# kolenyo2099/revers-o

Measured on AMD Instinct MI355X. Metric: images/sec embed+top-k (PE-L14-336, 1M x 1024 gallery), higher is better.
Workload: dtype bf16

## Files before the change

include/revo.h:

```cpp
#ifndef REVO_H
#define REVO_H
#include <stdint.h>

#ifdef __cplusplus
extern "C" {
#endif

typedef struct revo_vit revo_vit;
typedef struct revo_gallery revo_gallery;

typedef struct revo_vit_cfg {
    int32_t image_size, patch_size, width, layers, heads, mlp_dim, out_dim, pool_heads;
    int32_t use_cls;
    int32_t use_ls;
    float ln_eps, rope_theta;
    int32_t pool_mlp_dim;
} revo_vit_cfg;

typedef struct revo_tensor {
    const char* name;
    const float* data;
    int64_t numel;
} revo_tensor;

// ... 54 lines not shown
                         void* stream);
int32_t revo_search_topk_large(revo_gallery* g, const float* queries, int32_t n_queries, int32_t k, int32_t has_threshold,
                               float threshold, int64_t index_offset, float* scores, int64_t* indices, int32_t* counts,
                               void* stream);
int32_t revo_gallery_pairs(revo_gallery* g, float threshold, int64_t* n_pairs, void* stream);
int32_t revo_gallery_pairs_read(revo_gallery* g, int64_t start, int64_t n, int64_t* pairs, float* scores,
                                int32_t dst_on_device);
int32_t revo_gallery_clusters(revo_gallery* g, float threshold, int64_t* n_clusters, int64_t* n_members, void* stream);
int32_t revo_gallery_clusters_read(revo_gallery* g, int64_t* labels, int64_t* offsets, int64_t* members,
                                   int32_t dst_on_device);
int32_t revo_gallery_knn(revo_gallery* g, int32_t k, int32_t has_threshold, float threshold, int64_t* n_rows, void* stream);
int32_t revo_gallery_knn_read(revo_gallery* g, int64_t start, int64_t n, int64_t* indices, float* scores, int32_t* counts,
                              int32_t dst_on_device);
int32_t revo_gallery_kmeans(revo_gallery* g, const float* centroids, int32_t n_centroids, int32_t normalize,
                            int32_t src_on_device, int32_t max_iter, int32_t* n_iter, int32_t* converged, int64_t* n_rows,
                            void* stream);
int32_t revo_gallery_kmeans_read(revo_gallery* g, int64_t start, int64_t n, int32_t* labels, float* scores,
                                 int32_t dst_on_device);
int32_t revo_gallery_kmeans_centroids(revo_gallery* g, float* centroids, int64_t* sizes, int32_t dst_on_device);
int32_t revo_search_range(revo_gallery* g, const float* queries, int32_t n_queries, float threshold, int64_t index_offset,
                          int64_t* n_results, void* stream);
int32_t revo_search_range_read(revo_gallery* g, int64_t* offsets, int64_t start, int64_t n, int64_t* indices, float* scores,
                               int32_t dst_on_device);
int32_t revo_search_recommend(revo_gallery* g, const float* examples, int32_t n_positive, int32_t n_negative, int32_t k,
                              int32_t has_threshold, float threshold, int64_t index_offset, float* scores, int64_t* indices,
                              int32_t* counts, void* stream);
int32_t revo_search_discover(revo_gallery* g, const float* target, const float* positives, const float* negatives,
                             int32_t n_pairs, int32_t k, int32_t has_threshold, float threshold, int64_t index_offset,
                             float* scores, int64_t* indices, int32_t* counts, void* stream);
int32_t revo_search_maxsim(revo_gallery* g, const float* queries, int32_t n_vectors, int32_t k, int32_t has_threshold,
                           float threshold, int64_t index_offset, float* scores, int32_t* group_ids, int32_t* counts,
                           float* part_scores, int64_t* part_rows, void* stream);
int32_t revo_search_mmr(revo_gallery* g, const float* queries, int32_t n_queries, int32_t k, int32_t candidates,
                        float diversity, int32_t has_threshold, float threshold, int64_t index_offset, float* scores,
                        float* mmr_values, int64_t* indices, int32_t* counts, void* stream);
int32_t revo_search_fusion(revo_gallery* g, const float* queries, int32_t n_searches, int32_t n_lists, int32_t limit,
                           int32_t method, float rrf_k, const float* weights, const float* list_thresholds, int32_t k,
                           int32_t has_threshold, float threshold, int64_t index_offset, float* scores, int64_t* indices,
                           int32_t* counts, int32_t* ranks, float* list_scores, void* stream);
int32_t revo_topk_fuse(const float* scores, const int64_t* indices, const int32_t* counts, int32_t n_searches,
                       int32_t n_lists, int32_t limit, int32_t method, float rrf_k, const float* weights,
                       const float* list_thresholds, int32_t k, int32_t has_threshold, float threshold,
                       float* out_scores, int64_t* out_indices, int32_t* out_counts, int32_t* out_ranks, void* stream);
int32_t revo_search_ksel(int32_t k);
int32_t revo_search_set_total_rows(revo_gallery* g, int64_t total_rows);
int32_t revo_search_set_filter(revo_gallery* g, const uint32_t* allow_bits, int64_t rows, int32_t src_on_device,
                               void* stream);
int32_t revo_search_set_groups(revo_gallery* g, const int32_t* group_of_row, int64_t rows, int32_t src_on_device,
                               void* stream);
int32_t revo_search_groups(revo_gallery* g, const float* queries, int32_t n_queries, int32_t limit, int32_t group_size,
                           int32_t has_threshold, float threshold, int64_t index_offset, float* scores, int64_t* indices,
                           int32_t* hit_counts, int32_t* group_ids, int32_t* group_counts, void* stream);
int32_t revo_search_estimates(int32_t k);
int32_t revo_search_plan(const revo_gallery* g, int32_t n_queries, int32_t k, int64_t* out4);
int32_t revo_search_candidates(revo_gallery* g, const float* queries, int32_t n_queries, int32_t k, int32_t top_m,
                               uint32_t* bounds, void* stream);
int32_t revo_search_finish(revo_gallery* g, int32_t n_queries, int32_t k, int32_t has_threshold, float threshold,
                           int64_t index_offset, const uint32_t* all_bounds, int32_t parts, int32_t top_m, float* scores,
                           int64_t* indices, int32_t* counts, float* cert, void* stream);
int32_t revo_search_exact(revo_gallery* g, int32_t n, const int32_t* q_idx, const float* need, int32_t k,
                          int32_t has_threshold, float threshold, int64_t index_offset, float* scores, int64_t* indices,
                          int32_t* counts, void* stream);
int32_t revo_search_stats(revo_gallery* g, int32_t* out8, void* stream);
int32_t revo_topk_merge(const float* scores, const int64_t* indices, int32_t parts, int32_t n_queries, int32_t k,
                        int32_t has_threshold, float threshold, float* out_scores, int64_t* out_indices,
                        int32_t* out_counts, void* stream);

int64_t revo_topk_packed_bytes(int32_t n_queries, int32_t k);
int32_t revo_topk_merge_packed(const void* packed, int32_t parts, int32_t n_queries, int32_t k, int32_t has_threshold,
                               float threshold, float* out_scores, int64_t* out_indices, int32_t* out_counts,
                               int32_t* unc_count, int32_t* unc_q, float* unc_need, void* stream);

int32_t revo_op_gemm(int32_t epilogue, const void* a_bf16, int64_t lda, const void* b_bf16, int64_t ldb, int32_t m,
                     int32_t n, int32_t k, void* c, int64_t ldc, const float* bias, const float* gamma, void* stream);
int32_t revo_op_gemm_rope(const void* a_bf16, int64_t lda, const void* b_bf16, int64_t ldb, int32_t m, int32_t n, int32_t k,
                          void* c_bf16, int64_t ldc, const float* bias, const float* cos_sin, int32_t seq,
                          int32_t head_dim, int32_t rope_cols, void* stream);
int32_t revo_op_gemm_resid_ln(const void* a_bf16, int64_t lda, const void* b_bf16, int64_t ldb, int32_t m, int32_t n, int32_t k,
                              float* c, int64_t ldc, const float* bias, const float* gamma, void* xb_bf16, int64_t ldxb,
                              void* stats, int32_t* done, void* xlo_bf16, int32_t x_in_planes, int32_t planes_out, void* stream);
int32_t revo_op_gemm_ln_in(int32_t epilogue, const void* a_bf16, int64_t lda, const void* b_bf16, int64_t ldb, int32_t m, int32_t n,
                           int32_t k, void* c_bf16, int64_t ldc, const float* bias, const float* csum, const void* stats,
                           int32_t parts, float eps, void* tele, void* stream);
int32_t revo_op_gemm_ln_in_rope(const void* a_bf16, int64_t lda, const void* b_bf16, int64_t ldb, int32_t m, int32_t n, int32_t k,
                                void* c_bf16, int64_t ldc, const float* bias, const float* csum, const void* stats, int32_t parts,
                                float eps, const float* cos_sin, int32_t seq, int32_t head_dim, int32_t rope_cols, void* stream);
int32_t revo_op_gemm_resid_norm(const void* a_bf16, int64_t lda, const void* b_bf16, int64_t ldb, int32_t m, int32_t n, int32_t k,
                                float* c, int64_t ldc, const float* bias, const float* gamma, void* ln_out_bf16, int64_t ln_ldo,
                                float eps, int32_t* fused, void* stream);
int32_t revo_probe_mfma(const void* src_bf16, int64_t n_elems, float* sink, int32_t blocks, int32_t iters, void* stream);
int64_t revo_probe_mfma_flops(int32_t blocks, int32_t iters);
int32_t revo_probe_copy(void* dst, const void* src, int64_t bytes, void* stream);
#ifdef REVO_EXPERIMENTS
int32_t revo_vit_set_debug_layers(revo_vit* vit, int32_t n_layers);
int32_t revo_vit_read_residual(revo_vit* vit, int32_t batch, float* dst, void* stream);
int32_t revo_vit_read_tap(revo_vit* vit, int32_t which, int32_t batch, void* dst, void* stream);
int32_t revo_text_set_debug_layers(revo_text* text, int32_t n_layers);
int32_t revo_text_read_residual(revo_text* text, int32_t batch, float* dst, void* stream);
int32_t revo_search_set_mode(revo_gallery* g, int32_t mode);
int32_t revo_debug_set_remove_chunk(int64_t rows);
int32_t revo_debug_set_knn(int64_t cap_keys, int32_t level_mode);
int32_t revo_debug_set_kmeans(int64_t cap_keys);
int32_t revo_op_set_phase_groups(int32_t groups);
int32_t revo_op_set_qstores(int32_t on);
int32_t revo_debug_gemm_stamps(void* buf, int32_t items);
int32_t revo_debug_attention_clock(void* buf);
int32_t revo_debug_gemm_forms(int32_t reset);
int32_t revo_op_set_gemm_tile(int32_t tile);
int32_t revo_op_set_variant(int32_t flags);
int32_t revo_op_set_ln_fold(int32_t on);
int32_t revo_op_set_gemm_debug(int32_t flags);
int64_t revo_debug_scan_plan(int32_t Q, int64_t rows, int64_t* out, int32_t cap);
int64_t revo_debug_gemm_plan(int32_t epi, int32_t m, int32_t n, int32_t k, int64_t lda, int64_t ldb, int64_t ldc, int64_t ws_elems,
                             int32_t offers, int32_t rope_seq, int32_t rope_head_dim, int32_t rope_cols, int64_t* out, int32_t cap);
int32_t revo_debug_stream_in_planes(const revo_vit* vit, int32_t batch);
int64_t revo_debug_read_workspace(revo_gallery* g, int64_t offset, int64_t bytes, void* host_dst);
int32_t revo_debug_seed_bounds(revo_gallery* g, const uint32_t* bounds);
int32_t revo_probe_gridbar(int32_t mode, void* ctr_err, void* buf, int32_t n16, int32_t blocks, int32_t threads,
                           int32_t iters, float* sink, void* stamps, void* stream);
int32_t revo_debug_scan_stats(int64_t* out8);
#endif
int32_t revo_op_layernorm(const float* x, int64_t ldx, const float* w, const float* b, float eps, int32_t rows,
                          int32_t width, void* out, int64_t ldo, int32_t out_is_bf16, void* stream);
int32_t revo_op_layernorm_logits(const float* x, int64_t ldx, const float* w, const float* b, float eps, int32_t rows,
                                 int32_t width, float* out, int64_t ldo, const float* qk, const float* ck, int32_t heads,
                                 int32_t seq, float* logits, void* stream);
int32_t revo_op_linear_f32(int32_t epi, const float* A, int64_t lda, const float* Wt, int64_t ldw, const float* bias, int32_t M,
                           int32_t N, int32_t K, float* C, int64_t ldc, void* stream);
int32_t revo_op_linear_f32_grouped(int32_t epi, const float* A, int64_t lda, int64_t a_group_stride, int32_t group_cols,
                                   const float* Wt, int64_t ldw, const float* bias, int32_t M, int32_t N, int32_t K, float* C,
                                   int64_t ldc, void* stream);
int32_t revo_op_probe_qk(const float* q, const float* Wk, const float* bk, int32_t width, int32_t heads, float* qk, float* ck,
                         void* stream);
int32_t revo_op_l2norm_rows(const float* src, int64_t ld_src, float* dst_f32, int64_t ld_f32, uint16_t* dst_bf16, int64_t ld_bf16,
                            int64_t rows, int32_t dim, int32_t normalize, float* row_stats, float* max_stats, uint32_t* zero_a,
                            int64_t zero_a_words, uint32_t* zero_b, int64_t zero_b_words, const int64_t* dst_rows, void* stream);
int32_t revo_op_gallery_cert_stats(revo_gallery* g, float* out, void* stream);
int32_t revo_op_pool_rows(const float* x, int64_t ldx, const float* logits, int32_t batch, int32_t seq, int32_t width,
                          int32_t heads, float* u, void* stream);
int32_t revo_op_pool_rows_masked(const float* x, int64_t ldx, const float* logits, const int32_t* region_image,
                                 const uint32_t* region_bits, int32_t n_regions, int32_t batch, int32_t seq, int32_t width,
                                 int32_t heads, float* u, void* stream);
int32_t revo_op_detect_scores(const float* tokens, int64_t rows, const float* prompts, int32_t n_prompts, int32_t dim,
                              float* prompts_norm, float* scores, void* stream);
int32_t revo_op_detect_regions(const float* scores, int32_t batch, int32_t n_prompts, int32_t g, int32_t use_cls,
                               const float* thresholds, int32_t n_background, int32_t min_cells, int32_t max_regions,
                               int32_t* region_image, int32_t* region_prompt, int32_t* boxes, int32_t* cells, float* confidence,
                               uint32_t* bits, int32_t* labels, int32_t* counts, void* stream);
int32_t revo_op_rope(void* qkv_bf16, int64_t ld, const float* cos_sin, int32_t rows, int32_t seq, int32_t width,
                     int32_t heads, void* stream);
int32_t revo_op_attention(const void* qkv_bf16, int64_t ld, void* out_bf16, int64_t ldo, int32_t batch, int32_t seq,
                          int32_t heads, int32_t head_dim, void* stream);
int32_t revo_op_attention_causal(const void* qkv_bf16, int64_t ld, void* out_bf16, int64_t ldo, int32_t batch, int32_t seq,
                                 int32_t heads, int32_t head_dim, void* stream);
int32_t revo_op_embed_tokens(const int32_t* tokens_dev, const float* table, const float* pos, int32_t batch, int32_t seq,
                             int32_t vocab, int32_t width, float* x, int64_t ldx, void* stream);
int32_t revo_op_pool_eot(const int32_t* tokens_dev, const float* x, int64_t ldx, int32_t batch, int32_t seq, int32_t width,
                         float* out, void* stream);
int32_t revo_op_f32_to_bf16(const float* src, int64_t ld_src, void* dst_bf16, int64_t ld_dst, int64_t rows,
                            int32_t cols, void* stream);

int32_t revo_prof_enable(int32_t on);
int32_t revo_prof_reset(void);
int32_t revo_prof_report(char* buf, int32_t capacity);

typedef struct revo_crop_job {
// ... 12 lines not shown
```

revers-o_amd/_lib.py:

```python
import ctypes as C
import os

_HERE = os.path.dirname(os.path.abspath(__file__))
LIB_PATH = os.path.join(_HERE, "librevo.so")


class RevoError(RuntimeError):
    pass


class VitCfg(C.Structure):
    _fields_ = [(n, C.c_int32) for n in (
        "image_size", "patch_size", "width", "layers", "heads", "mlp_dim", "out_dim", "pool_heads",
        "use_cls", "use_ls")] + [("ln_eps", C.c_float), ("rope_theta", C.c_float), ("pool_mlp_dim", C.c_int32)]


class TextCfg(C.Structure):
    _fields_ = [(n, C.c_int32) for n in (
        "context_length", "vocab_size", "width", "layers", "heads", "mlp_dim", "out_dim", "use_ls")] + [("ln_eps", C.c_float)]


class Tensor(C.Structure):
    _fields_ = [("name", C.c_char_p), ("data", C.c_void_p), ("numel", C.c_int64)]


class CropJob(C.Structure):
    _fields_ = [("src", C.c_void_p), ("height", C.c_int32), ("width", C.c_int32), ("row_stride", C.c_int64),
                ("x0", C.c_int32), ("y0", C.c_int32), ("x1", C.c_int32), ("y1", C.c_int32)]


_p, _i32, _i64, _f32 = C.c_void_p, C.c_int32, C.c_int64, C.c_float

SIGNATURES = {
    "revo_last_error": (C.c_char_p, []),
    "revo_version": (_i32, []),
    "revo_sync": (_i32, [_p]),
    "revo_vit_create": (_i32, [C.POINTER(VitCfg), C.POINTER(Tensor), _i32, _i32, _i32, C.POINTER(_p)]),
    "revo_vit_destroy": (_i32, [_p]),
    "revo_vit_forward": (_i32, [_p, _p, _i32, _i32, _p, _i32, _p]),
    "revo_vit_forward_regions": (_i32, [_p, _p, _i32, _i32, _p, _p, _i32, _i32, _p, _p, _i32, _p]),
    "revo_vit_forward_tokens": (_i32, [_p, _p, _i32, _i32, _p, _p, _i32, _p]),
    "revo_vit_detect": (_i32, [_p, _p, _i32, _i32, _p, _i32, _p, _i32, _i32, _i32, _p, _i32, _i32, C.POINTER(C.c_int64), _p]),
    "revo_vit_detect_read": (_i32, [_p, _i64, _i64, _p, _p, _p, _p, _p, _p, _p, _i32]),
    "revo_vit_detect_maps": (_i32, [_p, _p, _p, _i32]),
    "revo_vit_seq_len": (_i32, [_p]),
    "revo_vit_stats": (_i32, [_p, C.POINTER(C.c_double), _i32, _p]),
    "revo_text_create": (_i32, [C.POINTER(TextCfg), C.POINTER(Tensor), _i32, _i32, _i32, C.POINTER(_p)]),
    "revo_text_destroy": (_i32, [_p]),
    "revo_text_forward": (_i32, [_p, _p, _i32, _i32, _p, _i32, _p]),
    "revo_gallery_create": (_i32, [_i32, _i64, _i32, _i32, C.POINTER(_p)]),
    "revo_gallery_destroy": (_i32, [_p]),
    "revo_gallery_append": (_i32, [_p, _p, _i64, _i32, _i32, _p]),
    "revo_gallery_size": (_i64, [_p]),
    "revo_gallery_clear": (_i32, [_p]),
    "revo_gallery_read": (_i32, [_p, _i64, _i64, _p, _i32]),
    "revo_gallery_remove": (_i32, [_p, _p, _i64, _i32, C.POINTER(C.c_int64), _p]),
    "revo_gallery_update": (_i32, [_p, _p, _p, _i64, _i32, _i32, _p]),
    "revo_gallery_append_unique": (_i32, [_p, _p, _i64, _i32, _i32, _f32, _p, _p, _i32, C.POINTER(C.c_int64), _p]),
    "revo_gallery_pairs": (_i32, [_p, _f32, C.POINTER(C.c_int64), _p]),
    "revo_gallery_pairs_read": (_i32, [_p, _i64, _i64, _p, _p, _i32]),
    "revo_gallery_clusters": (_i32, [_p, _f32, C.POINTER(C.c_int64), C.POINTER(C.c_int64), _p]),
    "revo_gallery_clusters_read": (_i32, [_p, _p, _p, _p, _i32]),
    "revo_gallery_knn": (_i32, [_p, _i32, _i32, _f32, C.POINTER(C.c_int64), _p]),
    "revo_gallery_knn_read": (_i32, [_p, _i64, _i64, _p, _p, _p, _i32]),
    "revo_gallery_kmeans": (_i32, [_p, _p, _i32, _i32, _i32, _i32, _p, _p, C.POINTER(C.c_int64), _p]),
    "revo_gallery_kmeans_read": (_i32, [_p, _i64, _i64, _p, _p, _i32]),
    "revo_gallery_kmeans_centroids": (_i32, [_p, _p, _p, _i32]),
    "revo_search_range": (_i32, [_p, _p, _i32, _f32, _i64, C.POINTER(C.c_int64), _p]),
    "revo_search_range_read": (_i32, [_p, _p, _i64, _i64, _p, _p, _i32]),
    "revo_search_recommend": (_i32, [_p, _p, _i32, _i32, _i32, _i32, _f32, _i64, _p, _p, _p, _p]),
    "revo_search_discover": (_i32, [_p, _p, _p, _p, _i32, _i32, _i32, _f32, _i64, _p, _p, _p, _p]),
    "revo_search_maxsim": (_i32, [_p, _p, _i32, _i32, _i32, _f32, _i64, _p, _p, _p, _p, _p, _p]),
    "revo_search_mmr": (_i32, [_p, _p, _i32, _i32, _i32, _f32, _i32, _f32, _i64, _p, _p, _p, _p, _p]),
    "revo_search_fusion": (_i32, [_p, _p, _i32, _i32, _i32, _i32, _f32, _p, _p, _i32, _i32, _f32, _i64, _p, _p, _p, _p, _p, _p]),
    "revo_topk_fuse": (_i32, [_p, _p, _p, _i32, _i32, _i32, _i32, _f32, _p, _p, _i32, _i32, _f32, _p, _p, _p, _p, _p]),
    "revo_search_topk": (_i32, [_p, _p, _i32, _i32, _i32, _f32, _i64, _p, _p, _p, _p]),
    "revo_search_topk_large": (_i32, [_p, _p, _i32, _i32, _i32, _f32, _i64, _p, _p, _p, _p]),
    "revo_search_ksel": (_i32, [_i32]),
    "revo_search_set_total_rows": (_i32, [_p, _i64]),
    "revo_search_set_filter": (_i32, [_p, _p, _i64, _i32, _p]),
    "revo_search_set_groups": (_i32, [_p, _p, _i64, _i32, _p]),
    "revo_search_groups": (_i32, [_p, _p, _i32, _i32, _i32, _i32, _f32, _i64, _p, _p, _p, _p, _p, _p]),
    "revo_search_estimates": (_i32, [_i32]),
    "revo_search_plan": (_i32, [_p, _i32, _i32, C.POINTER(C.c_int64)]),
    "revo_search_candidates": (_i32, [_p, _p, _i32, _i32, _i32, _p, _p]),
    "revo_search_finish": (_i32, [_p, _i32, _i32, _i32, _f32, _i64, _p, _i32, _i32, _p, _p, _p, _p, _p]),
    "revo_search_exact": (_i32, [_p, _i32, _p, _p, _i32, _i32, _f32, _i64, _p, _p, _p, _p]),
    "revo_search_stats": (_i32, [_p, C.POINTER(C.c_int32), _p]),
    "revo_topk_merge": (_i32, [_p, _p, _i32, _i32, _i32, _i32, _f32, _p, _p, _p, _p]),
    "revo_topk_packed_bytes": (_i64, [_i32, _i32]),
    "revo_topk_merge_packed": (_i32, [_p, _i32, _i32, _i32, _i32, _f32, _p, _p, _p, _p, _p, _p, _p]),
    "revo_op_gemm": (_i32, [_i32, _p, _i64, _p, _i64, _i32, _i32, _i32, _p, _i64, _p, _p, _p]),
    "revo_op_gemm_resid_ln": (_i32, [_p, _i64, _p, _i64, _i32, _i32, _i32, _p, _i64, _p, _p, _p, _i64, _p, C.POINTER(C.c_int32), _p, _i32,
                                     _i32, _p]),
    "revo_op_gemm_ln_in": (_i32, [_i32, _p, _i64, _p, _i64, _i32, _i32, _i32, _p, _i64, _p, _p, _p, _i32, _f32, _p, _p]),
    "revo_op_gemm_rope": (_i32, [_p, _i64, _p, _i64, _i32, _i32, _i32, _p, _i64, _p, _p, _i32, _i32, _i32, _p]),
    "revo_op_gemm_ln_in_rope": (_i32, [_p, _i64, _p, _i64, _i32, _i32, _i32, _p, _i64, _p, _p, _p, _i32, _f32, _p, _i32, _i32, _i32,
                                       _p]),
    "revo_op_gemm_resid_norm": (_i32, [_p, _i64, _p, _i64, _i32, _i32, _i32, _p, _i64, _p, _p, _p, _i64, _f32, C.POINTER(C.c_int32),
                                       _p]),
    "revo_op_layernorm": (_i32, [_p, _i64, _p, _p, _f32, _i32, _i32, _p, _i64, _i32, _p]),
    "revo_op_layernorm_logits": (_i32, [_p, _i64, _p, _p, _f32, _i32, _i32, _p, _i64, _p, _p, _i32, _i32, _p, _p]),
    "revo_op_linear_f32": (_i32, [_i32, _p, _i64, _p, _i64, _p, _i32, _i32, _i32, _p, _i64, _p]),
    "revo_op_linear_f32_grouped": (_i32, [_i32, _p, _i64, _i64, _i32, _p, _i64, _p, _i32, _i32, _i32, _p, _i64, _p]),
    "revo_op_probe_qk": (_i32, [_p, _p, _p, _i32, _i32, _p, _p, _p]),
    "revo_op_l2norm_rows": (_i32, [_p, _i64, _p, _i64, _p, _i64, _i64, _i32, _i32, _p, _p, _p, _i64, _p, _i64, _p, _p]),
    "revo_op_gallery_cert_stats": (_i32, [_p, C.POINTER(C.c_float), _p]),
    "revo_op_pool_rows": (_i32, [_p, _i64, _p, _i32, _i32, _i32, _i32, _p, _p]),
    "revo_op_pool_rows_masked": (_i32, [_p, _i64, _p, _p, _p, _i32, _i32, _i32, _i32, _i32, _p, _p]),
    "revo_op_detect_scores": (_i32, [_p, _i64, _p, _i32, _i32, _p, _p, _p]),
    "revo_op_detect_regions": (_i32, [_p, _i32, _i32, _i32, _i32, _p, _i32, _i32, _i32, _p, _p, _p, _p, _p, _p, _p, _p, _p]),
    "revo_op_rope": (_i32, [_p, _i64, _p, _i32, _i32, _i32, _i32, _p]),
    "revo_op_attention": (_i32, [_p, _i64, _p, _i64, _i32, _i32, _i32, _i32, _p]),
    "revo_op_attention_causal": (_i32, [_p, _i64, _p, _i64, _i32, _i32, _i32, _i32, _p]),
    "revo_op_embed_tokens": (_i32, [_p, _p, _p, _i32, _i32, _i32, _i32, _p, _i64, _p]),
    "revo_op_pool_eot": (_i32, [_p, _p, _i64, _i32, _i32, _i32, _p, _p]),
    "revo_op_f32_to_bf16": (_i32, [_p, _i64, _p, _i64, _i64, _i32, _p]),
    "revo_prof_enable": (_i32, [_i32]),
    "revo_prof_reset": (_i32, []),
    "revo_prof_report": (_i32, [C.c_char_p, _i32]),
    "revo_preprocess_crop_resize": (_i32, [C.POINTER(CropJob), _i32, _i32, _p, _p]),
    "revo_probe_mfma": (_i32, [_p, _i64, _p, _i32, _i32, _p]),
    "revo_probe_mfma_flops": (_i64, [_i32, _i32]),
    "revo_probe_copy": (_i32, [_p, _p, _i64, _p]),
}

EXPERIMENT_SIGNATURES = {
    "revo_vit_set_debug_layers": (_i32, [_p, _i32]),
    "revo_vit_read_residual": (_i32, [_p, _i32, _p, _p]),
    "revo_vit_read_tap": (_i32, [_p, _i32, _i32, _p, _p]),
    "revo_text_set_debug_layers": (_i32, [_p, _i32]),
    "revo_text_read_residual": (_i32, [_p, _i32, _p, _p]),
    "revo_search_set_mode": (_i32, [_p, _i32]),
    "revo_op_set_gemm_tile": (_i32, [_i32]),
    "revo_op_set_phase_groups": (_i32, [_i32]),
    "revo_op_set_qstores": (_i32, [_i32]),
    "revo_debug_gemm_forms": (_i32, [_i32]),
    "revo_debug_gemm_stamps": (_i32, [_p, _i32]),
    "revo_debug_attention_clock": (_i32, [_p]),
    "revo_op_set_variant": (_i32, [_i32]),
    "revo_op_set_ln_fold": (_i32, [_i32]),
    "revo_op_set_gemm_debug": (_i32, [_i32]),
    "revo_debug_scan_stats": (_i32, [C.POINTER(C.c_int64)]),
    "revo_debug_set_remove_chunk": (_i32, [_i64]),
    "revo_debug_set_knn": (_i32, [_i64, _i32]),
    "revo_debug_set_kmeans": (_i32, [_i64]),
    "revo_debug_seed_bounds": (_i32, [_p, _p]),
    "revo_debug_read_workspace": (_i64, [_p, _i64, _i64, _p]),
    "revo_debug_stream_in_planes": (_i32, [_p, _i32]),
    "revo_probe_gridbar": (_i32, [_i32, _p, _p, _i32, _i32, _i32, _i32, _p, _p, _p]),
    "revo_debug_scan_plan": (_i64, [_i32, _i64, C.POINTER(C.c_int64), _i32]),
    "revo_debug_gemm_plan": (_i64, [_i32, _i32, _i32, _i32, _i64, _i64, _i64, _i64, _i32, _i32, _i32, _i32, C.POINTER(C.c_int64), _i32]),
}
BASE_SIGNATURES = dict(SIGNATURES)
if os.environ.get("REVO_LIBRARY_PATH"):
    LIB_PATH = os.environ["REVO_LIBRARY_PATH"]
elif os.environ.get("REVO_EXPERIMENTS") == "1":
    LIB_PATH = os.path.join(_HERE, "librevo_exp.so")
if os.environ.get("REVO_EXPERIMENTS") == "1":
    SIGNATURES = dict(SIGNATURES, **EXPERIMENT_SIGNATURES)

_lib = None
_lib_exp = None


def product_is_experiment_build():
    return os.environ.get("REVO_EXPERIMENTS") == "1"


def load_exp():
    global _lib_exp
    if _lib_exp is not None:
        return _lib_exp
    import torch
    path = os.path.join(_HERE, "librevo_exp.so")
    if not os.path.exists(path):
        raise RevoError(f"{path} not found: build it with `make -C revers-o_amd/csrc exp`")
    lib = C.CDLL(path)
# ... 47 lines not shown
```

revers-o_amd/csrc/api.hip:

```cpp
#include <algorithm>
#include <cstdlib>
#include <cstring>
#include <map>
#include <mutex>
#include <string>
#include <vector>

#include "../../include/revo.h"
#include "api_internal.h"
#include "kernels.h"
#include "tower.h"

static thread_local std::string g_err;
void revo_set_error(const std::string& msg) { g_err = msg; }
extern "C" const char* revo_last_error(void) { return g_err.c_str(); }
extern "C" int32_t revo_version(void) { return 100; }

extern "C" int32_t revo_sync(void* stream) {
    REVO_HIP_CHECK(hipStreamSynchronize((hipStream_t)stream));
    return 0;
}

namespace {
struct Profiler {
// ... 4 lines not shown
    std::vector<hipEvent_t> pool;
    std::map<std::string, std::pair<long, double>> acc;
    hipEvent_t get() {
        if (!pool.empty()) { hipEvent_t e = pool.back(); pool.pop_back(); return e; }
        hipEvent_t e; (void)hipEventCreate(&e); return e;
    }
    void drain() {
        for (auto& r : recs) {
            float ms = 0.f;
            if (hipEventSynchronize(r.b) == hipSuccess && hipEventElapsedTime(&ms, r.a, r.b) == hipSuccess) {
                auto& s = acc[r.cls];
                s.first += 1; s.second += ms;
            }
            pool.push_back(r.a); pool.push_back(r.b);
        }
        recs.clear();
    }
} g_prof;
}

ProfScope::ProfScope(const char* cls, hipStream_t s) : active(g_prof.on != 0), st(s) {
    if (active && g_prof.on >= 2) {
        const int which = !strcmp(cls, "gemm_qkv") ? 0 : !strcmp(cls, "gemm_out") ? 1 : !strcmp(cls, "gemm_fc1") ? 2 :
                          !strcmp(cls, "gemm_fc2") ? 3 : -1;
        active = which >= 0;
        if (active && g_prof.on == 3) active = (g_prof.sample[which]++ & 3) == 0;
    }
    if (!active) return;
    std::lock_guard<std::mutex> lk(g_prof.mu);
    rec.cls = cls; rec.a = g_prof.get(); rec.b = g_prof.get();
    (void)hipEventRecord(rec.a, st);
}
ProfScope::~ProfScope() {
    if (!active) return;
    (void)hipEventRecord(rec.b, st);
    std::lock_guard<std::mutex> lk(g_prof.mu);
    g_prof.recs.push_back(rec);
}

extern "C" int32_t revo_prof_enable(int32_t on) {
    g_prof.on = on < 0 ? 0 : (on > 3 ? 1 : on);
    for (auto& x : g_prof.sample) x = 0;
    return 0;
}
extern "C" int32_t revo_prof_reset(void) {
    std::lock_guard<std::mutex> lk(g_prof.mu);
    g_prof.drain();
    g_prof.acc.clear();
    return 0;
}
extern "C" int32_t revo_prof_report(char* buf, int32_t capacity) {
    std::lock_guard<std::mutex> lk(g_prof.mu);
    g_prof.drain();
    std::string s = "{";
    bool first = true;
    for (auto& kv : g_prof.acc) {
        if (!first) s += ", ";
        first = false;
        s += "\"" + kv.first + "\": {\"launches\": " + std::to_string(kv.second.first) +
             ", \"ms\": " + std::to_string(kv.second.second) + "}";
    }
    s += "}";
    if ((int)s.size() + 1 > capacity) { revo_set_error("prof_report: buffer too small"); return -2; }
    memcpy(buf, s.c_str(), s.size() + 1);
    return 0;
}

namespace {
constexpr long OP_WS_ELEMS = 16l << 20;
struct OpScratch {
    float* p = nullptr; hipStream_t st; hipError_t err = hipSuccess;
    explicit OpScratch(hipStream_t s, bool wanted = true) : st(s) {
        if (wanted) err = hipMallocAsync((void**)&p, OP_WS_ELEMS * 4, st);
    }
    OpScratch(const OpScratch&) = delete;
    ~OpScratch() { if (p) (void)hipFreeAsync(p, st); }
    long elems() const { return p ? OP_WS_ELEMS : 0; }
    int status() const {
        if (err == hipSuccess) return 0;
        revo_set_error(std::string("hipMallocAsync((void**)&ws, OP_WS_ELEMS * 4, st): ") + hipGetErrorString(err));
        return -1;
    }
};
}

extern "C" int32_t revo_op_gemm(int32_t epi, const void* a, int64_t lda, const void* b, int64_t ldb, int32_t m,
                                int32_t n, int32_t k, void* c, int64_t ldc, const float* bias, const float* gamma,
                                void* stream) {
    API_BEGIN
    REVO_REQUIRE(epi >= 0 && epi <= 3, "op_gemm: epilogue must be 0..3");
    hipStream_t st = (hipStream_t)stream;
    OpScratch ws(st, epi == revo::EPI_RESID_F32);
    CHECK_RC(ws.status());
    return gemm("gemm_op", epi, (const bf16_t*)a, lda, (const bf16_t*)b, ldb, m, n, k, c, ldc, bias, gamma, st, ws.p, ws.elems());
    API_END
}
extern "C" int32_t revo_op_gemm_resid_ln(const void* a, int64_t lda, const void* b, int64_t ldb, int32_t m, int32_t n, int32_t k,
                                         float* c, int64_t ldc, const float* bias, const float* gamma, void* xb, int64_t ldxb,
                                         void* stats, int32_t* done, void* xlo, int32_t x_in_planes, int32_t planes_out,
                                         void* stream) {
    API_BEGIN
    REVO_REQUIRE(a && b && c && xb && done, "op_gemm_resid_ln: null argument");
    REVO_REQUIRE(stats || (xlo && x_in_planes && !planes_out), "op_gemm_resid_ln: stats may be NULL only for planes in, fp32 out");
    REVO_REQUIRE(xlo || (!x_in_planes && !planes_out), "op_gemm_resid_ln: planes need the low plane");
    hipStream_t st = (hipStream_t)stream;
    OpScratch ws(st);
    CHECK_RC(ws.status());
    revo::GemmArgs g = gemm_args(a, lda, b, ldb, m, n, k, c, ldc);
    g.bias = bias; g.gamma = gamma; g.ws = ws.p; g.ws_elems = OP_WS_ELEMS;
    int flag = 0;
    if (stats) { g.lnf_xb = (bf16_t*)xb; g.lnf_ldxb = ldxb; g.lnf_stats = (float2*)stats; g.lnf_done = &flag; }
    if (xlo) { g.xp_hi = (bf16_t*)xb; g.xp_lo = (bf16_t*)xlo; g.xp_ld = ldxb; g.xp_in = x_in_planes != 0; g.xp_out = planes_out != 0; }
    const int rc = revo::launch_gemm(revo::EPI_RESID_F32, g, st);
    *done = flag;
    return rc;
    API_END
}
extern "C" int32_t revo_op_gemm_ln_in(int32_t epi, const void* a, int64_t lda, const void* b, int64_t ldb, int32_t m, int32_t n,
                                      int32_t k, void* c, int64_t ldc, const float* bias, const float* csum, const void* stats,
                                      int32_t parts, float eps, void* tele, void* stream) {
    API_BEGIN
    REVO_REQUIRE(epi == revo::EPI_BF16 || epi == revo::EPI_BF16_GELU, "op_gemm_ln_in: epilogue must be 0 (bf16) or 1 (bf16 + GELU)");
    REVO_REQUIRE(a && b && c && csum && stats, "op_gemm_ln_in: null argument");
    revo::GemmArgs g = gemm_args(a, lda, b, ldb, m, n, k, c, ldc);
    g.bias = bias; g.lnc_stats = (const float2*)stats; g.lnc_parts = parts; g.lnc_c = csum; g.lnc_eps = eps;
    g.lnc_tele = (unsigned long long*)tele;
    return revo::launch_gemm(epi, g, (hipStream_t)stream);
    API_END
}
extern "C" int32_t revo_op_gemm_rope(const void* a, int64_t lda, const void* b, int64_t ldb, int32_t m, int32_t n,
                                     int32_t k, void* c, int64_t ldc, const float* bias, const float* cos_sin,
                                     int32_t seq, int32_t head_dim, int32_t rope_cols, void* stream) {
    API_BEGIN
    revo::GemmArgs g = gemm_args(a, lda, b, ldb, m, n, k, c, ldc);
    g.bias = bias; g.rope_cs = (const float2*)cos_sin; g.rope_S = seq; g.rope_hd = head_dim; g.rope_cols = rope_cols;
    return revo::launch_gemm(revo::EPI_BF16_ROPE, g, (hipStream_t)stream);
    API_END
}
extern "C" int32_t revo_op_gemm_ln_in_rope(const void* a, int64_t lda, const void* b, int64_t ldb, int32_t m, int32_t n, int32_t k,
                                           void* c, int64_t ldc, const float* bias, const float* csum, const void* stats,
                                           int32_t parts, float eps, const float* cos_sin, int32_t seq, int32_t head_dim,
                                           int32_t rope_cols, void* stream) {
    API_BEGIN
    REVO_REQUIRE(a && b && c && csum && stats && cos_sin, "op_gemm_ln_in_rope: null argument");
    revo::GemmArgs g = gemm_args(a, lda, b, ldb, m, n, k, c, ldc);
    g.bias = bias; g.rope_cs = (const float2*)cos_sin; g.rope_S = seq; g.rope_hd = head_dim; g.rope_cols = rope_cols;
    g.lnc_stats = (const float2*)stats; g.lnc_parts = parts; g.lnc_c = csum; g.lnc_eps = eps;
    return revo::launch_gemm(revo::EPI_BF16_ROPE, g, (hipStream_t)stream);
    API_END
}
extern "C" int32_t revo_op_gemm_resid_norm(const void* a, int64_t lda, const void* b, int64_t ldb, int32_t m, int32_t n, int32_t k,
                                           float* c, int64_t ldc, const float* bias, const float* gamma, void* ln_out,
                                           int64_t ln_ldo, float eps, int32_t* fused, void* stream) {
    API_BEGIN
    REVO_REQUIRE(a && b && c && ln_out && fused, "op_gemm_resid_norm: null argument");
    hipStream_t st = (hipStream_t)stream;
    OpScratch ws(st);
    CHECK_RC(ws.status());
    int flag = 0;
    const LnAfter ln{eps, (bf16_t*)ln_out, ln_ldo, &flag, nullptr, nullptr, nullptr, 0, 0};
    const int rc = gemm("gemm_op", revo::EPI_RESID_F32, (const bf16_t*)a, lda, (const bf16_t*)b, ldb, m, n, k, c, ldc, bias, gamma,
                        st, ws.p, OP_WS_ELEMS, &ln);
    *fused = flag;
    return rc;
    API_END
}
#ifdef REVO_EXPERIMENTS
extern "C" int32_t revo_op_set_variant(int32_t flags) {
    revo::gemm_force_gy((flags >> 4) & 15);
    revo::attention_force_nw((flags >> 8) & 15);
    revo::gemm_set_tail_split(((flags >> 12) & 1) ? 0 : 1);
    revo::gemm_set_persistent(((flags >> 16) & 1) ? 0 : 1);
    revo::gemm_set_splitk(((flags >> 17) & 1) ? 0 : 1);
    revo::gemm_set_min_tiles256(((flags >> 18) & 1) ? 0 : 100);
    revo::gemm_set_ring(((flags >> 19) & 1) ? 0 : 1, 0);
    revo::gemm_set_rows192(((flags >> 3) & 1) ? 0 : 1);
    revo::attention_set_shape16((flags >> 20) & 1);
    return 0;
}
extern "C" int32_t revo_op_set_ln_fold(int32_t on) {
    REVO_REQUIRE(on >= 0 && on <= 2, "set_ln_fold: 0 (LayerNorm kernels), 1 (folded, stream in planes: default) or 2 (folded, fp32 stream + bf16 copy)");
    revo::gemm_set_ln_fold(on);
    return 0;
}
extern "C" int32_t revo_op_set_qstores(int32_t on) {
    revo::gemm_set_qstores(on);
    return 0;
}
extern "C" int32_t revo_op_set_phase_groups(int32_t groups) {
    REVO_REQUIRE(groups >= 0 && groups <= 4, "set_phase_groups: 0 (heuristic), 1 (off) or 2..4");
    revo::gemm_set_phase_groups(groups);
    return 0;
}
extern "C" int32_t revo_debug_attention_clock(void* buf) {
    revo::attention_set_clock_buffer((unsigned long long*)buf);
    return 0;
}
extern "C" int32_t revo_debug_gemm_stamps(void* buf, int32_t items) {
    revo::gemm_set_stamps((unsigned long long*)buf, buf ? items : 0);
    return 0;
}
extern "C" int32_t revo_debug_gemm_forms(int32_t reset) { return (int32_t)revo::gemm_debug_forms(reset); }
extern "C" int32_t revo_op_set_gemm_tile(int32_t tile) {
    REVO_REQUIRE(tile == 0 || tile == 128 || tile == 256, "set_gemm_tile: 0, 128 or 256");
    revo::gemm_force_tile(tile);
    return 0;
}
extern "C" int32_t revo_op_set_gemm_debug(int32_t flags) {
    revo::gemm_set_debug(flags & 3);
    revo::gemm_set_stagger(((flags >> 28) & 15) * 200, 2 + ((flags >> 2) & 3));
    revo::topk_scan256_set_debug(((flags >> 13) & 7) | (((flags >> 20) & 255) << 3));
    return revo_op_set_variant(flags);
}
extern "C" int64_t revo_debug_scan_plan(int32_t Q, int64_t rows, int64_t* out, int32_t cap) {
    if (Q < 1 || rows < 1 || !out || cap < 2) return -1;
    return (int64_t)revo::topk_scan256_plan_dump(Q, (long)rows, (long*)out, cap);
}
extern "C" int64_t revo_debug_gemm_plan(int32_t epi, int32_t m, int32_t n, int32_t k, int64_t lda, int64_t ldb, int64_t ldc,
                                        int64_t ws_elems, int32_t offers, int32_t rope_seq, int32_t rope_head_dim, int32_t rope_cols,
                                        int64_t* out, int32_t cap) {
    if (epi < 0 || epi > 5 || !out) return -2;
    return (int64_t)revo::gemm_debug_plan(epi, m, n, k, (long)lda, (long)ldb, (long)ldc, (long)ws_elems, (unsigned)offers, rope_seq,
                                          rope_head_dim, rope_cols, (long*)out, cap);
}
#endif
extern "C" int32_t revo_op_layernorm(const float* x, int64_t ldx, const float* w, const float* b, float eps,
                                     int32_t rows, int32_t width, void* out, int64_t ldo, int32_t out_is_bf16,
                                     void* stream) {
    API_BEGIN
    return revo::launch_layernorm(x, ldx, w, b, eps, rows, width, out, ldo, out_is_bf16, (hipStream_t)stream);
    API_END
// ... 153 lines not shown
```

revers-o_amd/csrc/gemm.hip:

```cpp
#include <cstdlib>
#include "gemm_kernels.h"
#include "gemm_plan.h"

namespace revo {

static GemmKnobs g_knobs;
void gemm_force_tile(int t) { g_knobs.force_tile = t; }
void gemm_force_gy(int gy) { g_knobs.force_gy = gy; }
void gemm_set_min_tiles256(int n) { g_knobs.min_tiles256 = n; }
void gemm_set_persistent(int on) { g_knobs.persistent = on; }
void gemm_set_qstores(int on) { g_knobs.qstores = on & 31; g_knobs.qtail = !(on & 32); }
void gemm_set_ring(int on, int max_tiles) { g_knobs.ring = on; if (max_tiles > 0) g_knobs.ring_max_tiles = max_tiles; }
void gemm_set_tail_split(int on) { g_knobs.tail_split = on; }
void gemm_set_splitk(int on) { g_knobs.splitk = on; }
void gemm_set_rows192(int on) { g_knobs.rows192 = on; }
void gemm_set_ln_fold(int on) { g_knobs.lnf = on != 0; g_knobs.ln_planes = on != 2; }
bool gemm_ln_planes_enabled() { return g_knobs.lnf && g_knobs.ln_planes; }
#ifdef REVO_EXPERIMENTS
void gemm_set_debug(int d) { g_knobs.dbg = d; }
void gemm_set_stagger(int cycles, int groups) { g_knobs.stagger_cycles = cycles; g_knobs.stagger_groups = groups < 1 ? 1 : groups; }
void gemm_set_phase_groups(int g) { g_knobs.phase_groups = g < 0 ? 0 : (g > 4 ? 4 : g); }
static unsigned long long* g_stamps = nullptr; static int g_stamp_items = 0;
void gemm_set_stamps(unsigned long long* buf, int items) { g_stamps = buf; g_stamp_items = items; }
static unsigned g_forms = 0;
unsigned gemm_debug_forms(int reset) { const unsigned f = g_forms; if (reset) g_forms = 0; return f; }
#endif

static const char* check_args(const GemmArgs& a) {
    if (const char* e = gemm_shape_error(a.M, a.N, a.K, a.lda, a.ldb, a.ldc)) return e;
    if (((uintptr_t)a.A | (uintptr_t)a.B | (uintptr_t)a.C) & 15) return "gemm: operands must be 16-byte aligned";
    return nullptr;
}

bool gemm_resid_folds(int M, int N, int K, long lda, long ldb, long ldc) {
    GemmProblem p{};
    p.epi = EPI_RESID_F32; p.M = M; p.N = N; p.K = K; p.lda = lda; p.ldb = ldb; p.ldc = ldc;
    p.fold_offered = true;
    const GemmPlan pl = gemm_plan(p, g_knobs);
    return !pl.error && pl.step[0].fold;
}

template <int EPI, int BMR>
static int launch_256p(GemmArgs& b, const GemmStep& s, hipStream_t st) {
    int nslot = s.nslot;
#ifdef REVO_EXPERIMENTS
    b.stagger_cycles = g_knobs.stagger_cycles; b.stagger_groups = g_knobs.stagger_groups;
    b.stamps = g_stamps; b.stamp_items = g_stamp_items;
    if (const char* e = getenv("REVO_GEMM_NSLOT")) { const int v = atoi(e); if (v >= 1 && v < nslot) nslot = v; }
    {
        int groups = g_knobs.phase_groups > 1 ? g_knobs.phase_groups : 1;
        if (BMR != 256 && groups > 3) groups = 3;
        if (groups > 1 || b.stamps != nullptr) {
            REVO_FUNC_LDS((gemm256pp_kernel<EPI, BMR>), G256P_LDS);
            hipLaunchKernelGGL((gemm256pp_kernel<EPI, BMR>), dim3(8 * nslot), dim3(G256_THREADS), G256P_LDS, st, b, nslot, groups);
            return 0;
        }
    }
#endif
    if constexpr (EPI == EPI_RESID_F32) {
#define REVO_LAUNCH_XP(X)                                                                                              \
    case X:                                                                                                             \
        REVO_FUNC_LDS((gemm256p_kernel<EPI, BMR, X>), G256P_LDS);                                                       \
        hipLaunchKernelGGL((gemm256p_kernel<EPI, BMR, X>), dim3(8 * nslot), dim3(G256_THREADS), G256P_LDS, st, b, nslot); \
        return 0;
        switch (s.xp) { REVO_LAUNCH_XP(1) REVO_LAUNCH_XP(2) REVO_LAUNCH_XP(3) default: break; }
#undef REVO_LAUNCH_XP
    }
    REVO_FUNC_LDS((gemm256p_kernel<EPI, BMR>), G256P_LDS);
    hipLaunchKernelGGL((gemm256p_kernel<EPI, BMR>), dim3(8 * nslot), dim3(G256_THREADS), G256P_LDS, st, b, nslot);
    return 0;
}

template <int EPI, int DBG>
static int launch_256d(const GemmArgs& b, const GemmStep& s, hipStream_t st) {
    REVO_FUNC_LDS((gemm256_kernel<EPI, DBG>), G256_LDS_LN);
    hipLaunchKernelGGL((gemm256_kernel<EPI, DBG>), dim3(s.grid_x), dim3(G256_THREADS), G256_LDS_LN, st, b);
    return 0;
}

static int launch_splitk(const GemmArgs& b, const GemmStep& s, hipStream_t st) {
    const long plane = (long)b.M * b.N;
    GemmArgs c = b;
    c.C = b.ws; c.ldc = b.N; c.bias = nullptr; c.gamma = nullptr;
    c.ksplit = s.S; c.c_split_stride = plane;
    if (s.form == GF_SPLITK_256) {
        REVO_FUNC_LDS((gemm256_kernel<EPI_F32, 4>), G256_LDS);
        hipLaunchKernelGGL((gemm256_kernel<EPI_F32, 4>), dim3(s.grid_x, s.grid_y), dim3(G256_THREADS), G256_LDS, st, c);
    } else {
        constexpr int LDS = G128R_NST * (128 + 64) * 128;
        REVO_FUNC_LDS((gemm128r_kernel<EPI_F32>), LDS);
        hipLaunchKernelGGL((gemm128r_kernel<EPI_F32>), dim3(s.grid_x, s.grid_y), dim3(GEMM_THREADS), LDS, st, c);
    }
    REVO_HIP_CHECK(hipGetLastError());
    if (s.reduce_ln) {
        const dim3 grid((unsigned)((b.M + 3) / 4));
        const int groups = (b.N / 8 + 63) / 64;
#define RLN_LAUNCH(G) hipLaunchKernelGGL((splitk_reduce_resid_ln_kernel<G>), grid, dim3(256), 0, st, b.ws, s.S, plane, b.M, b.N, b.bias, \
                                         b.gamma, (float*)b.C, b.ldc, b.ln_w, b.ln_b, b.ln_eps, b.ln_out, b.ln_ldo)
        if (groups <= 1) RLN_LAUNCH(1);
        else if (groups <= 2) RLN_LAUNCH(2);
        else if (groups <= 3) RLN_LAUNCH(3);
        else RLN_LAUNCH(4);
#undef RLN_LAUNCH
        return 0;
    }
    const long quads = plane / 4;
    hipLaunchKernelGGL(splitk_reduce_resid_kernel, dim3((unsigned)((quads + 255) / 256)), dim3(256), 0, st, b.ws, s.S, plane,
                       b.M, b.N, b.bias, b.gamma, (float*)b.C, b.ldc);
    return 0;
}

template <int EPI>
static int run_step(const GemmArgs& a, const GemmStep& s, hipStream_t st) {
    constexpr bool BF16 = EPI == EPI_BF16 || EPI == EPI_BF16_GELU;
    GemmArgs b = a;
    b.M = s.rows;
    b.A = a.A + (long)s.row0 * a.lda;
    b.C = (char*)a.C + (long)s.row0 * a.ldc * (BF16 ? 2 : 4);
    if (b.lnc_stats) b.lnc_stats += (long)s.row0 * a.lnc_parts;
    b.gy = s.gy; b.t192_tiles = s.t192_tiles; b.t192_tall = s.t192_tall; b.qtail_rows = s.qtail_rows;
    if (!s.fold) { b.lnf_xb = nullptr; b.lnf_stats = nullptr; }
    if (!s.xp) b.xp_in = b.xp_out = 0;
    switch (s.form) {
        case GF_SKINNY_444:
        case GF_SKINNY_411:
            if (s.form == GF_SKINNY_444) hipLaunchKernelGGL((gemm_skinny_kernel<EPI, 4, 4, 4>), dim3(s.grid_x, s.grid_y), dim3(256), 0, st, b);
            else hipLaunchKernelGGL((gemm_skinny_kernel<EPI, 4, 1, 1>), dim3(s.grid_x), dim3(256), 0, st, b);
            break;
        case GF_128_128:
            REVO_FUNC_LDS((gemm128_kernel<EPI, 128>), 2 * (128 + 128) * 128);
            hipLaunchKernelGGL((gemm128_kernel<EPI, 128>), dim3(s.grid_x), dim3(GEMM_THREADS), 2 * (128 + 128) * 128, st, b);
            break;
        case GF_128_64:
            hipLaunchKernelGGL((gemm128_kernel<EPI, 64>), dim3(s.grid_x), dim3(GEMM_THREADS), 2 * (128 + 64) * 128, st, b);
            break;
        case GF_128R: {
            constexpr int LDS = G128R_NST * (128 + 64) * 128;
            REVO_FUNC_LDS((gemm128r_kernel<EPI>), LDS);
            hipLaunchKernelGGL((gemm128r_kernel<EPI>), dim3(s.grid_x), dim3(GEMM_THREADS), LDS, st, b);
            break;
        }
        case GF_256_TILE:
#ifdef REVO_EXPERIMENTS
            if constexpr (EPI == EPI_BF16) {
                if (s.dbg == 1) return launch_256d<EPI_BF16, 1>(b, s, st);
                if (s.dbg == 2) return launch_256d<EPI_BF16, 2>(b, s, st);
                if (s.dbg) return launch_256d<EPI_BF16, 3>(b, s, st);
            }
#endif
            return launch_256d<EPI, 0>(b, s, st);
        case GF_256P:
            return launch_256p<EPI, 256>(b, s, st);
        case GF_256P_192:
            if constexpr (EPI == EPI_RESID_F32) return launch_256p<EPI, 192>(b, s, st);
            return -3;
        case GF_256Q:
        case GF_256Q_QTAIL:
            if constexpr (BF16 || (EPI == EPI_BF16_ROPE && G256Q_ROPE_BUILT)) {
#ifdef REVO_EXPERIMENTS
                b.stamps = g_stamps; b.stamp_items = g_stamp_items;
                b.stagger_cycles = 0;
                b.stagger_groups = ((g_knobs.qstores & 7) == 2 ? 0x100 : 0)
                                   | ((g_knobs.qstores & 8) ? 0x200 : 0);
#endif
                REVO_FUNC_LDS((gemm256q_kernel<EPI>), G256Q_LDS);
                hipLaunchKernelGGL((gemm256q_kernel<EPI>), dim3(8 * s.nslot), dim3(G256_THREADS), G256Q_LDS, st, b, s.nslot);
                break;
            }
            return -3;
        case GF_SPLITK_RING:
        case GF_SPLITK_RING_LN:
        case GF_SPLITK_256:
            if constexpr (EPI == EPI_RESID_F32) return launch_splitk(b, s, st);
            return -3;
        default:
            return -3;
    }
    return 0;
}

template <int EPI>
static int run_plan(const GemmArgs& a, const GemmPlan& pl, hipStream_t st) {
    for (int i = 0; i < pl.nsteps; ++i) {
        const int rc = run_step<EPI>(a, pl.step[i], st);
        if (rc == -3) revo_set_error("gemm: internal: the plan names a form this epilogue does not have");
        if (rc) return rc;
        REVO_HIP_CHECK(hipGetLastError());
    }
    return 0;
}

int launch_gemm_f32_ring(const GemmArgs& a, hipStream_t st) {
    if (const char* e = check_args(a)) {
        revo_set_error(e);
        return -2;
    }
    REVO_REQUIRE(a.N % 64 == 0 && a.K % 64 == 0, "gemm ring: N and K must be multiples of 64");
    const int tiles64 = ((a.M + 127) / 128) * ((a.N + 63) / 64);
    constexpr int LDS = G128R_NST * (128 + 64) * 128;
    REVO_FUNC_LDS((gemm128r_kernel<EPI_F32>), LDS);
    GemmArgs b = a;
    b.ksplit = 1;
    hipLaunchKernelGGL((gemm128r_kernel<EPI_F32>), dim3(tiles64), dim3(GEMM_THREADS), LDS, st, b);
    REVO_HIP_CHECK(hipGetLastError());
    return 0;
}

int launch_gemm(int epi, const GemmArgs& a, hipStream_t st) {
    if (const char* e = check_args(a)) {
        revo_set_error(e);
        return -2;
    }
    if (a.lnc_stats && (!a.lnc_c || a.lnc_parts < 1 || a.lnc_parts > 6 || (epi != EPI_BF16 && epi != EPI_BF16_GELU && epi != EPI_BF16_ROPE))) {
        revo_set_error("gemm: a folded LayerNorm (lnc_*) needs a bf16 epilogue, the column sums and 1..6 statistics slots per row");
        return -2;
    }
    if (epi == EPI_BF16_ROPE && (!a.rope_cs || a.rope_S <= 0 || a.rope_hd <= 0 || a.rope_hd % 8 || a.rope_cols % a.rope_hd || a.rope_cols > a.N)) {
        revo_set_error("gemm: the RoPE epilogue needs a table, rope_hd % 8 == 0 and rope_cols a multiple of rope_hd");
        return -2;
    }
    const GemmPlan pl = gemm_plan(gemm_problem(epi, a), g_knobs);
    if (pl.error) {
        revo_set_error(pl.error);
        return -2;
    }
    int rc;
    switch (epi) {
        case EPI_BF16: rc = run_plan<EPI_BF16>(a, pl, st); break;
        case EPI_BF16_GELU: rc = run_plan<EPI_BF16_GELU>(a, pl, st); break;
        case EPI_RESID_F32: rc = run_plan<EPI_RESID_F32>(a, pl, st); break;
        case EPI_F32: rc = run_plan<EPI_F32>(a, pl, st); break;
        case EPI_PATCH: rc = run_plan<EPI_PATCH>(a, pl, st); break;
        case EPI_BF16_ROPE: rc = run_plan<EPI_BF16_ROPE>(a, pl, st); break;
        default: revo_set_error("gemm: unknown epilogue"); return -2;
    }
    if (rc) return rc;
    if (pl.step[0].fold) *a.lnf_done = 1;
    if (pl.step[0].reduce_ln) *a.ln_fused = 1;
#ifdef REVO_EXPERIMENTS
    g_forms |= pl.forms;
#endif
    return 0;
}

#ifdef REVO_EXPERIMENTS
long gemm_debug_plan(int epi, int M, int N, int K, long lda, long ldb, long ldc, long ws_elems, unsigned offers, int rope_S,
                     int rope_hd, int rope_cols, long* out, int cap) {
    GemmProblem p{};
    p.epi = epi; p.M = M; p.N = N; p.K = K; p.lda = lda; p.ldb = ldb; p.ldc = ldc; p.ws_elems = ws_elems;
    p.ln_offered = offers & 1; p.ln_ldo = ldc;
    p.fold_offered = offers & 2; p.lnf_ldxb = ldc;
    p.xp_in = (offers >> 2) & 1; p.xp_out = (offers >> 3) & 1; p.planes_valid = true;
    p.lnc = offers & 16; p.prefer256 = (offers >> 5) & 1;
    p.rope_S = rope_S; p.rope_hd = rope_hd; p.rope_cols = rope_cols;
    const GemmPlan pl = gemm_plan(p, g_knobs);
    constexpr int PER_STEP = 14;
    if (cap < 2 + 2 * PER_STEP) return -2;
    out[0] = pl.error ? -1 : (long)pl.forms;
    out[1] = pl.error ? 0 : pl.nsteps;
    for (int i = 0; i < out[1]; ++i) {
        const GemmStep& s = pl.step[i];
        const long v[PER_STEP] = {(long)s.form, s.row0, s.rows, s.gy, s.nslot, s.grid_x, s.grid_y, s.t192_tiles, s.t192_tall, s.qtail_rows,
                                  s.S, s.reduce_ln, s.xp, s.fold};
        for (int j = 0; j < PER_STEP; ++j) out[2 + i * PER_STEP + j] = v[j];
    }
    return out[0];
}
#endif

}
```

revers-o_amd/csrc/gemm_kernels.h:

```cpp
#pragma once
#include <type_traits>
#include "gemm_core.h"
#include "gemm256_core.h"
#include "kernels.h"

namespace revo {

__device__ __forceinline__ f32x2 gelu_erf2(f32x2 x) {
    const f32x2 ax = {__builtin_fabsf(x.x), __builtin_fabsf(x.y)};
    const f32x2 z = ax * 0.70710678118654752f;
    f32x2 p = z * 0.0000430638f + 0.0002765672f;
    p = p * z + 0.0001520143f;
    p = p * z + 0.0092705272f;
    p = p * z + 0.0422820123f;
    p = p * z + 0.0705230784f;
    p = p * z + 1.0f;
    p = p * p;
    p = p * p;
    p = p * p;
    p = p * p;
    const f32x2 r = {__builtin_amdgcn_rcpf(p.x), __builtin_amdgcn_rcpf(p.y)};
    return (x + ax * (1.0f - r)) * 0.5f;
}
__device__ __forceinline__ f32x4 gelu_erf4(f32x4 v) {
    const f32x2 lo = gelu_erf2((f32x2){v[0], v[1]}), hi = gelu_erf2((f32x2){v[2], v[3]});
    return (f32x4){lo.x, lo.y, hi.x, hi.y};
}
#ifndef REVO_LNC_ABLATE
#define REVO_LNC_ABLATE 0
#endif
#ifndef REVO_GELU_WIDTH
#define REVO_GELU_WIDTH 2
#endif
template <int NV>
__device__ __forceinline__ void gelu_erf4xn(f32x4 (&v)[NV]) {
    constexpr int NP = 2 * NV;
    f32x2 x[NP], ax[NP], z[NP], q[NP];
#pragma unroll
    for (int i = 0; i < NP; ++i) {
        x[i] = (f32x2){v[i >> 1][(i & 1) * 2], v[i >> 1][(i & 1) * 2 + 1]};
        ax[i] = (f32x2){__builtin_fabsf(x[i].x), __builtin_fabsf(x[i].y)};
    }
#pragma unroll
    for (int i = 0; i < NP; ++i) z[i] = ax[i] * 0.70710678118654752f;
#pragma unroll
    for (int i = 0; i < NP; ++i) q[i] = z[i] * 0.0000430638f + 0.0002765672f;
#pragma unroll
    for (int i = 0; i < NP; ++i) q[i] = q[i] * z[i] + 0.0001520143f;
#pragma unroll
    for (int i = 0; i < NP; ++i) q[i] = q[i] * z[i] + 0.0092705272f;
#pragma unroll
    for (int i = 0; i < NP; ++i) q[i] = q[i] * z[i] + 0.0422820123f;
#pragma unroll
    for (int i = 0; i < NP; ++i) q[i] = q[i] * z[i] + 0.0705230784f;
#pragma unroll
    for (int i = 0; i < NP; ++i) q[i] = q[i] * z[i] + 1.0f;
#pragma unroll
    for (int r = 0; r < 4; ++r)
#pragma unroll
        for (int i = 0; i < NP; ++i) q[i] = q[i] * q[i];
#pragma unroll
    for (int i = 0; i < NP; ++i) q[i] = (f32x2){__builtin_amdgcn_rcpf(q[i].x), __builtin_amdgcn_rcpf(q[i].y)};
#pragma unroll
    for (int i = 0; i < NP; ++i) q[i] = 1.0f - q[i];
#pragma unroll
    for (int i = 0; i < NP; ++i) x[i] = x[i] + ax[i] * q[i];
#pragma unroll
    for (int i = 0; i < NP; ++i) x[i] = x[i] * 0.5f;
#pragma unroll
    for (int i = 0; i < NV; ++i) v[i] = (f32x4){x[2 * i].x, x[2 * i].y, x[2 * i + 1].x, x[2 * i + 1].y};
}

__device__ __forceinline__ float row16_sum(float v) {
    v += __builtin_bit_cast(float, __builtin_amdgcn_update_dpp(0, __builtin_bit_cast(int, v), 0xB1, 0xf, 0xf, true));
    v += __builtin_bit_cast(float, __builtin_amdgcn_update_dpp(0, __builtin_bit_cast(int, v), 0x4E, 0xf, 0xf, true));
    v += __builtin_bit_cast(float, __builtin_amdgcn_update_dpp(0, __builtin_bit_cast(int, v), 0x141, 0xf, 0xf, true));
    v += __builtin_bit_cast(float, __builtin_amdgcn_update_dpp(0, __builtin_bit_cast(int, v), 0x140, 0xf, 0xf, true));
    return v;
}
__device__ __forceinline__ void lnf_merge(const float2* part, int P, float eps, float& rstd, float& mr) {
    float sm = 0.f, sq = 0.f;
    for (int i = 0; i < P; ++i) { const float2 t = part[i]; sm += t.x; sq += t.y; }
    const float mean = sm / (float)P;
    float dd = 0.f;
    for (int i = 0; i < P; ++i) { const float d = part[i].x - mean; dd = fmaf(d, d, dd); }
    const float var = fmaf((float)LNF_SLICE, dd, sq) / (float)(LNF_SLICE * P);
    rstd = rsqrtf(var + eps);
    mr = -mean * rstd;
}

template <int EPI, int MF, int NF>
__device__ __forceinline__ void gemm_epilogue(const GemmArgs& p, int m_base, int n_base, int lane,
                                              f32x4 (&acc)[MF][NF]) {
    const int lr = lane & 15, lq = lane >> 4;
    const bool lnc = (EPI == EPI_BF16 || EPI == EPI_BF16_GELU || EPI == EPI_BF16_ROPE) && p.lnc_stats != nullptr;
#pragma unroll
    for (int m = 0; m < MF; ++m) {
        const int row = m_base + m * 16 + lr;
        if (row >= p.M) continue;
        float ln_rstd = 1.f, ln_mr = 0.f;
        if (lnc)
            lnf_merge(p.lnc_stats + (long)row * p.lnc_parts, p.lnc_parts, p.lnc_eps, ln_rstd, ln_mr);
        long orow = row;
        int prow = 0;
        if (EPI == EPI_PATCH) {
            const int b = row / p.G2, g = row - b * p.G2;
            orow = (long)b * p.S + p.cls + g;
            prow = p.cls + g;
        }
#pragma unroll
        for (int n = 0; n < NF; ++n) {
            const int col = n_base + n * 16 + lq * 4;
            if (col >= p.N) continue;
            f32x4 v = acc[m][n];
            if (lnc) {
                const f32x4 c = *(const f32x4*)(p.lnc_c + col);
                const f32x4 b = p.bias ? *(const f32x4*)(p.bias + col) : (f32x4){0.f, 0.f, 0.f, 0.f};
                v = v * ln_rstd + (c * ln_mr + b);
            } else
            if (p.bias) {
                const f32x4 b = *(const f32x4*)(p.bias + col);
                v += b;
            }
            if (EPI == EPI_BF16_ROPE) {
                {
                    const bool rot = col < p.rope_cols;
                    const float2* t = p.rope_cs + (long)(row % p.rope_S) * (p.rope_hd >> 1) + ((col % p.rope_hd) >> 1);
                    const f32x4 tc = *(const f32x4*)t;
#pragma unroll
                    for (int h2 = 0; h2 < 2; ++h2) {
                        const float x0 = bf16_to_f32(f32_to_bf16(v[2 * h2])), x1 = bf16_to_f32(f32_to_bf16(v[2 * h2 + 1]));
                        const float cx = rot ? tc[2 * h2] : 1.0f, cy = rot ? tc[2 * h2 + 1] : 0.0f;
                        v[2 * h2] = x0 * cx - x1 * cy;
                        v[2 * h2 + 1] = x1 * cx + x0 * cy;
                    }
                }
            }
            if (EPI == EPI_BF16 || EPI == EPI_BF16_GELU || EPI == EPI_BF16_ROPE) {
                if (EPI == EPI_BF16_GELU) v = gelu_erf4(v);
                uint2 o;
                o.x = pack_bf16x2(v[0], v[1]);
                o.y = pack_bf16x2(v[2], v[3]);
                *(uint2*)((bf16_t*)p.C + orow * p.ldc + col) = o;
            } else if (EPI == EPI_RESID_F32) {
                float* dst = (float*)p.C + orow * p.ldc + col;
                f32x4 x = *(const f32x4*)dst;
                if (p.gamma) {
                    const f32x4 g = *(const f32x4*)(p.gamma + col);
                    v *= g;
                }
                x += v;
                *(f32x4*)dst = x;
            } else if (EPI == EPI_F32) {
                *(f32x4*)((float*)p.C + orow * p.ldc + col) = v;
            } else if (EPI == EPI_PATCH) {
                const f32x4 pe = *(const f32x4*)(p.pos + (long)prow * p.N + col);
                v += pe;
                *(f32x4*)((float*)p.C + orow * p.ldc + col) = v;
            }
        }
    }
}

template <int QT>
__device__ __forceinline__ void gemm256_load_resid(const GemmArgs& p, int m_base, int n_base, int lane, f32x4 (&res)[8],
                                                   bool nt = false) {
    int gcol = n_base + (lane & 15) * 4;
    gcol = gcol < p.N ? gcol : p.N - 4;
#pragma unroll
    for (int it = 0; it < 8; ++it) {
        int grow = m_base + QT * 32 + it * 4 + (lane >> 4);
        grow = grow < p.M ? grow : p.M - 1;
        const f32x4* src = (const f32x4*)((const float*)p.C + (long)grow * p.ldc + gcol);
        res[it] = nt ? __builtin_nontemporal_load(src) : *src;
    }
}
template <int EPI, int QT>
__device__ __forceinline__ void gemm256_epilogue_f32_quarter(const GemmArgs& p, char* slab, int m_base, int n_base,
                                                             int lane, f32x4 (&acc)[8][4], const f32x4 (&bias4)[4],
                                                             const f32x4 (&gamma4)[4], const f32x4 (&res)[8],
                                                             float2* lnst = nullptr) {
    constexpr int RS = 272;
    asm volatile("" : "+v"(lane) :: "memory");
    const int lr = lane & 15, lq = lane >> 4;
#pragma unroll
// ... 201 lines not shown
                                o.y = pack_bf16x2(v[n][2], v[n][3]);
                                *(uint2*)(slab + (m * 16 + lr) * RS + ((n0 + n) * 16 + lq * 4) * 2) = o;
                            }
                        }
                    } else {
#pragma unroll
                        for (int n = 0; n < 4; ++n) {
                            f32x4 v;
                            if (LNC && !(REVO_LNC_ABLATE & 2)) v = acc[half * 4 + m][n] * st.x + (c4[n] * st.y + bias4[n]);
                            else v = acc[half * 4 + m][n] + bias4[n];
                            uint2 o;
                            o.x = pack_bf16x2(v[0], v[1]);
                            o.y = pack_bf16x2(v[2], v[3]);
                            *(uint2*)(slab + (m * 16 + lr) * RS + (n * 16 + lq * 4) * 2) = o;
                        }
                    }
                }
            };
            if (lnmr) frag_phase(std::true_type{});
            else frag_phase(std::false_type{});
            if (EPI == EPI_BF16_ROPE && half == 0 && !(SKIP_DEAD && m_base + 64 >= p.M)) rope_load(1, rtab_next);
            const int gcol = n_base + (lane & 7) * 8;
#pragma unroll
            for (int it = 0; it < 8; ++it) {
                const int rl = it * 8 + (lane >> 3);
                uint4 v = *(const uint4*)(slab + rl * RS + (lane & 7) * 16);
                const int grow = m_base + half * 64 + rl;
                if (EPI == EPI_BF16_ROPE) {
                    if (gcol < p.rope_cols) {
                        uint32_t w[4] = {v.x, v.y, v.z, v.w};
#pragma unroll
                        for (int j = 0; j < 4; ++j) {
                            const float x0 = bf16_to_f32((bf16_t)(w[j] & 0xffff)), x1 = bf16_to_f32((bf16_t)(w[j] >> 16));
                            const float cx = rtab[it][j >> 1][(j & 1) * 2], cy = rtab[it][j >> 1][(j & 1) * 2 + 1];
                            w[j] = pack_bf16x2(x0 * cx - x1 * cy, x1 * cx + x0 * cy);
                        }
                        v = make_uint4(w[0], w[1], w[2], w[3]);
                    }
                }
                typedef uint32_t nt_u32x4 __attribute__((ext_vector_type(4)));
                if (EPI == EPI_BF16_ROPE || EPI == EPI_BF16_GELU) {
                    if (grow < p.M && gcol < p.N)
                        __builtin_nontemporal_store(__builtin_bit_cast(nt_u32x4, v), (nt_u32x4*)((bf16_t*)p.C + (long)grow * p.ldc + gcol));
                } else
                if (grow < p.M && gcol < p.N) *(uint4*)((bf16_t*)p.C + (long)grow * p.ldc + gcol) = v;
            }
            asm volatile("" ::: "memory");
        }
    } else {
        if (SKIP_DEAD && m_base >= p.M) return;
        if constexpr (EPI == EPI_RESID_F32 && XP != 0) {
            constexpr bool PIN = XP >= 2, POUT = XP <= 2, ST = XP <= 2;
#pragma unroll
            for (int m = 0; m < 8; ++m)
#pragma unroll
                for (int n = 0; n < 4; ++n) acc[m][n] = (acc[m][n] + bias4[n]) * gamma4[n];
            asm volatile("" ::: "memory");
            uint4 pa[4][2], pb[4][2];
            gemm256_resid8_load<0, PIN>(p, m_base, n_base, lane, pa);
            gemm256_resid8_quarter<0, PIN, POUT, ST>(p, slab, m_base, n_base, lane, acc, pa, lnst);
            gemm256_resid8_load<1, PIN>(p, m_base, n_base, lane, pa);
            gemm256_resid8_load<2, PIN>(p, m_base, n_base, lane, pb);
            gemm256_resid8_quarter<1, PIN, POUT, ST>(p, slab, m_base, n_base, lane, acc, pa, lnst);
            if (SKIP_DEAD && m_base + 64 >= p.M) return;
            gemm256_resid8_quarter<2, PIN, POUT, ST>(p, slab, m_base, n_base, lane, acc, pb, lnst);
            gemm256_resid8_load<3, PIN>(p, m_base, n_base, lane, pa);
            gemm256_resid8_quarter<3, PIN, POUT, ST>(p, slab, m_base, n_base, lane, acc, pa, lnst);
            return;
        }
        f32x4 ra[8], rb[8];
        const bool nt = lnst != nullptr;
        if (EPI == EPI_RESID_F32) gemm256_load_resid<0>(p, m_base, n_base, lane, ra, nt);
        if (EPI == EPI_RESID_F32) gemm256_load_resid<1>(p, m_base, n_base, lane, rb, nt);
        gemm256_epilogue_f32_quarter<EPI, 0>(p, slab, m_base, n_base, lane, acc, bias4, gamma4, ra, lnst);
        gemm256_epilogue_f32_quarter<EPI, 1>(p, slab, m_base, n_base, lane, acc, bias4, gamma4, rb, lnst);
        if (SKIP_DEAD && m_base + 64 >= p.M) return;
        if (EPI == EPI_RESID_F32) gemm256_load_resid<2>(p, m_base, n_base, lane, ra, nt);
        if (EPI == EPI_RESID_F32) gemm256_load_resid<3>(p, m_base, n_base, lane, rb, nt);
        gemm256_epilogue_f32_quarter<EPI, 2>(p, slab, m_base, n_base, lane, acc, bias4, gamma4, ra, lnst);
        gemm256_epilogue_f32_quarter<EPI, 3>(p, slab, m_base, n_base, lane, acc, bias4, gamma4, rb, lnst);
    }
}

constexpr int LNC_RAW_BYTES = 256 * 6 * 8 + 1024, LNC_MR_BYTES = 256 * 8;
constexpr int G256P_LN_OFF = 98304 + 5 * 9216;
static_assert(G256P_LN_OFF + LNC_RAW_BYTES + LNC_MR_BYTES <= 163840, "");
constexpr int G256_LDS_LN = G256_LDS + LNC_RAW_BYTES + LNC_MR_BYTES;
constexpr int G256Q_BC_OFF = G256_LDS_LN + LNC_MR_BYTES;
constexpr int G256Q_LDS = G256Q_BC_OFF + 2 * 2048;
static_assert(G256Q_LDS <= 163840, "");
template <class ARGS>
__device__ __forceinline__ void lnc_issue_stats(const ARGS& p, int m0, char* lds_raw, int wave, int ) {
    if (wave >= 4) return;
    int lane;
    asm volatile("v_mbcnt_lo_u32_b32 %0, -1, 0\n\tv_mbcnt_hi_u32_b32 %0, -1, %0" : "=v"(lane) :: "memory");
    const int P = p.lnc_parts;
    long left = ((long)p.M - m0) * P * 8;
    const long full = 256l * P * 8;
    left = left < 0 ? 0 : (left > full ? full : left);
    const __amdgpu_buffer_rsrc_t rs = __builtin_amdgcn_make_buffer_rsrc((void*)(p.lnc_stats + (long)m0 * P), 0, (int)left, 0x00020000);
    const int share = 512 * P, pieces = (share + 1023) >> 10;
    for (int j = 0; j < pieces; ++j) {
        const int off = wave * share + j * 1024;
        if (off + 1024 <= LNC_RAW_BYTES)
            __builtin_amdgcn_raw_ptr_buffer_load_lds(rs, (__attribute__((address_space(3))) void*)(lds_raw + off), 16,
                                                     (uint32_t)(off + lane * 16), 0, 0, 0);
    }
}
template <int VM = 4, class ARGS = GemmArgs>
__device__ __forceinline__ void lnc_merge_rows(const ARGS& p, const char* lds_raw, float2* lds_mr, int wave, int , bool one_ktile,
                                               bool tele = false, int rows_left = 0) {
    if (wave >= 4) return;
    int lane;
    asm volatile("v_mbcnt_lo_u32_b32 %0, -1, 0\n\tv_mbcnt_hi_u32_b32 %0, -1, %0" : "=v"(lane) :: "memory");
    if (one_ktile) asm volatile("s_waitcnt vmcnt(0)" ::: "memory");
    else asm volatile("s_waitcnt vmcnt(%0)" :: "n"(VM) : "memory");
    const int t = wave * 64 + lane;
    if (t < 256) {
        float r, m;
        auto merge_n = [&](auto np) {
            constexpr int NP = decltype(np)::value;
            f32x4 v[NP / 2];
#pragma unroll
            for (int i = 0; i < NP / 2; ++i) v[i] = *(const f32x4*)(lds_raw + t * (NP * 8) + i * 16);
            float sm = 0.f, sq = 0.f;
#pragma unroll
            for (int i = 0; i < NP; ++i) { sm += v[i >> 1][(i & 1) * 2]; sq += v[i >> 1][(i & 1) * 2 + 1]; }
            const float mean = sm / (float)NP;
            float dd = 0.f;
#pragma unroll
            for (int i = 0; i < NP; ++i) { const float d = v[i >> 1][(i & 1) * 2] - mean; dd = fmaf(d, d, dd); }
            const float var = fmaf((float)LNF_SLICE, dd, sq) / (float)(LNF_SLICE * NP);
            r = rsqrtf(var + p.lnc_eps);
            m = -mean * r;
        };
        if (p.lnc_parts == 4) merge_n(std::integral_constant<int, 4>{});
        else if (p.lnc_parts == 6) merge_n(std::integral_constant<int, 6>{});
        else lnf_merge((const float2*)lds_raw + t * p.lnc_parts, p.lnc_parts, p.lnc_eps, r, m);
        lds_mr[t] = make_float2(r, m);
        if (tele) {
            const int live = rows_left - wave * 64 < 0 ? 0 : (rows_left - wave * 64 > 64 ? 64 : rows_left - wave * 64);
            const float am = lane < live ? __builtin_fabsf(m) : 0.f;
            const unsigned long long big = __builtin_amdgcn_ballot_w64(am > LNC_TELE_RATIO);
            const unsigned long long huge = __builtin_amdgcn_ballot_w64(am > 4.0f * LNC_TELE_RATIO);
            if (lane == 0 && live > 0) {
                unsigned long long* tp = p.lnc_tele;
                asm volatile("" : "+v"(tp));
                atomicAdd(tp, (unsigned long long)live);
                if (big) atomicAdd(tp + 1, (unsigned long long)__builtin_popcountll(big));
                if (huge) atomicAdd(tp + 2, (unsigned long long)__builtin_popcountll(huge));
            }
        }
    }
    asm volatile("s_waitcnt lgkmcnt(0)" ::: "memory");
}
__device__ __forceinline__ void lnf_store_tile_stats(const GemmArgs& p, const float2* lds_st, int m0, int mend, int tn, int wave,
                                                     int lane) {
    asm volatile("" : "+v"(lane) :: "memory");
    const int t = wave * 64 + lane;
    if (t < 256 && m0 + t < mend) {
        const float2 a = lds_st[t * 4], b = lds_st[t * 4 + 1], c = lds_st[t * 4 + 2], d = lds_st[t * 4 + 3];
        const float mean = ((a.x + b.x) + (c.x + d.x)) * 0.25f;
        const float da = a.x - mean, db = b.x - mean, dc = c.x - mean, dd = d.x - mean;
        const float m2 = ((a.y + b.y) + (c.y + d.y)) + 64.0f * (fmaf(da, da, db * db) + fmaf(dc, dc, dd * dd));
        p.lnf_stats[(long)(m0 + t) * (p.N / LNF_SLICE) + tn] = make_float2(mean, m2);
    }
}

template <int EPI, int BN = 128>
__global__ __launch_bounds__(GEMM_THREADS) void gemm128_kernel(GemmArgs p) {
    extern __shared__ __attribute__((aligned(16))) char smem[];
    constexpr int BM = 128, MF = 4, NF = BN / 32;
    const int tiles_n = (p.N + BN - 1) / BN;
    const int tiles_m = (p.M + BM - 1) / BM;
    const int s = xcd_remap(blockIdx.x, tiles_m * tiles_n);
    const int tm = s / tiles_n, tn = s - tm * tiles_n;
    const int m0 = tm * BM, n0 = tn * BN;
    const int wave = __builtin_amdgcn_readfirstlane(threadIdx.x >> 6);
    const int lane = threadIdx.x & 63;
    const int wr = wave >> 1, wc = wave & 1;

    TileLoader<BM> la;
    TileLoader<BN> lb;
    la.init(p.A, p.lda, m0, p.M, wave, lane);
    lb.init(p.B, p.ldb, n0, p.N, wave, lane);

    f32x4 acc[MF][NF];
#pragma unroll
    for (int m = 0; m < MF; ++m)
#pragma unroll
        for (int n = 0; n < NF; ++n) acc[m][n] = (f32x4){0.f, 0.f, 0.f, 0.f};

    gemm_mainloop<BM, BN, MF, NF>(la, lb, smem, p.K, wave, lane, wr * 64, wc * (BN / 2), acc);
    gemm_epilogue<EPI, MF, NF>(p, m0 + wr * 64, n0 + wc * (BN / 2), lane, acc);
}

constexpr int G128R_NST = 6;
template <int EPI>
__global__ __launch_bounds__(GEMM_THREADS) void gemm128r_kernel(GemmArgs p) {
    extern __shared__ __attribute__((aligned(16))) char smem[];
    constexpr int BM = 128, BN = 64, MF = 4, NF = BN / 32;
    const int tiles_n = (p.N + BN - 1) / BN;
    const int tiles_m = (p.M + BM - 1) / BM;
    const int s = xcd_remap(blockIdx.x, tiles_m * tiles_n);
    const int tm = s / tiles_n, tn = s - tm * tiles_n;
    const int m0 = tm * BM, n0 = tn * BN;
    const int wave = __builtin_amdgcn_readfirstlane(threadIdx.x >> 6);
    const int lane = threadIdx.x & 63;
    const int wr = wave >> 1, wc = wave & 1;
    if (EPI == EPI_F32 && p.ksplit > 1) {
        const int nt = p.K >> 6, t0 = (int)blockIdx.y * nt / p.ksplit, t1 = ((int)blockIdx.y + 1) * nt / p.ksplit;
        p.A += t0 * 64;
        p.B += t0 * 64;
        p.K = (t1 - t0) * 64;
        p.C = (float*)p.C + (long)blockIdx.y * p.c_split_stride;
    }
    TileLoader<BM> la;
    TileLoader<BN> lb;
    la.init(p.A, p.lda, m0, p.M, wave, lane);
    lb.init(p.B, p.ldb, n0, p.N, wave, lane);
    f32x4 acc[MF][NF];
#pragma unroll
    for (int m = 0; m < MF; ++m)
#pragma unroll
        for (int n = 0; n < NF; ++n) acc[m][n] = (f32x4){0.f, 0.f, 0.f, 0.f};
    gemm_mainloop_ring<BM, BN, MF, NF, G128R_NST>(la, lb, smem, p.K, wave, lane, wr * 64, wc * (BN / 2), acc);
    gemm_epilogue<EPI, MF, NF>(p, m0 + wr * 64, n0 + wc * (BN / 2), lane, acc);
}

template <int EPI, int DBG>
__global__ __launch_bounds__(G256_THREADS, 2) void gemm256_kernel(GemmArgs p) {
    extern __shared__ __attribute__((aligned(16))) char smem[];
    const int tiles_n = (p.N + 255) / 256;
    const int tiles_m = (p.M + 255) / 256;
    const int gy = p.gy, gx = 8 / gy;
    const int xcd = blockIdx.x & 7, slot = blockIdx.x >> 3;
    const int xi = xcd / gy, xj = xcd - xi * gy;
    const int pm = (tiles_m + gx - 1) / gx, pn = (tiles_n + gy - 1) / gy;
    const int m_lo = xi * pm, n_lo = xj * pn;
    const int m_cnt = (tiles_m - m_lo) < pm ? (tiles_m - m_lo) : pm;
    const int n_cnt = (tiles_n - n_lo) < pn ? (tiles_n - n_lo) : pn;
    if (m_cnt <= 0 || n_cnt <= 0 || slot >= m_cnt * n_cnt) return;
    const int tm = m_lo + slot / n_cnt, tn = n_lo + slot % n_cnt;
    const int m0 = tm * 256, n0 = tn * 256;
    const int wave = __builtin_amdgcn_readfirstlane(threadIdx.x >> 6);
    const int lane = threadIdx.x & 63;

    if (DBG & 4) {
        const int nt = p.K >> 6, t0 = (int)blockIdx.y * nt / p.ksplit, t1 = ((int)blockIdx.y + 1) * nt / p.ksplit;
        p.A += t0 * 64;
        p.B += t0 * 64;
        p.K = (t1 - t0) * 64;
        p.C = (float*)p.C + (long)blockIdx.y * p.c_split_stride;
    }
    G256Operand A, B;
    g256_operand_init(A, p.A, p.lda, p.M, m0, wave, lane);
    g256_operand_init(B, p.B, p.ldb, p.N, n0, wave, lane);

    f32x4 acc[8][4];
#pragma unroll
    for (int m = 0; m < 8; ++m)
#pragma unroll
        for (int n = 0; n < 4; ++n) acc[m][n] = (f32x4){0.f, 0.f, 0.f, 0.f};

    const bool lnc = (EPI == EPI_BF16 || EPI == EPI_BF16_GELU || EPI == EPI_BF16_ROPE) && p.lnc_stats != nullptr;
    float2* lds_mr = (float2*)(smem + G256_LDS + LNC_RAW_BYTES);
    if (!(DBG & 2)) {
        if (lnc) lnc_issue_stats(p, m0, smem + G256_LDS, wave, lane);
        g256_issue_prologue(A, B, smem, p.K, wave);
        if (lnc) lnc_merge_rows(p, smem + G256_LDS, lds_mr, wave, lane, p.K <= 64, p.lnc_tele != nullptr && n0 == 0, p.M - m0);
        gemm256_mainloop(A, B, smem, p.K, wave, lane, acc);
    }
    if (DBG & 1) {
        if (acc[0][0][0] != 12345.678f) return;
    }
    if constexpr (EPI == EPI_PATCH) {
        gemm_epilogue<EPI, 8, 4>(p, m0 + (wave >> 2) * 128, n0 + (wave & 3) * 64, lane, acc);
    } else {
        const bool wide = (p.N & 7) == 0 && (p.ldc & 7) == 0;
        if (wide) gemm256_epilogue<EPI>(p, smem + wave * 16384, m0 + (wave >> 2) * 128, n0 + (wave & 3) * 64, lane, acc, nullptr,
                                        lnc ? lds_mr + (wave >> 2) * 128 : nullptr);
        else gemm_epilogue<EPI, 8, 4>(p, m0 + (wave >> 2) * 128, n0 + (wave & 3) * 64, lane, acc);
    }
}


constexpr int G256P_LDS = 163840;
template <int EPI, int BMR = 256, int XP = 0>
__global__ __launch_bounds__(G256_THREADS, 2) void gemm256p_kernel(GemmArgs p, int nslot) {
    static_assert(BMR == 256 || BMR == 192, "");
    extern __shared__ __attribute__((aligned(16))) char smem[];
    const int tiles_n = (p.N + 255) / 256;
    const int tiles_m = BMR == 256 ? (p.M + 255) / 256 : p.t192_tiles;
    const int tall0 = tiles_m - p.t192_tall;
    const int gy = p.gy, gx = 8 / gy;
    const int xcd = blockIdx.x & 7;
    const int xi = __builtin_amdgcn_readfirstlane(xcd / gy), xj = xcd - xi * gy;
    const int pm = __builtin_amdgcn_readfirstlane((tiles_m + gx - 1) / gx), pn = __builtin_amdgcn_readfirstlane((tiles_n + gy - 1) / gy);
    const int m_lo = xi * pm, n_lo = xj * pn;
    const int m_cnt = (tiles_m - m_lo) < pm ? (tiles_m - m_lo) : pm;
    const int n_cnt = (tiles_n - n_lo) < pn ? (tiles_n - n_lo) : pn;
    const int total = (m_cnt > 0 && n_cnt > 0) ? m_cnt * n_cnt : 0;
    int slot = blockIdx.x >> 3;
    if (slot >= total) return;
    const int wave = __builtin_amdgcn_readfirstlane(threadIdx.x >> 6);
    const int lane = threadIdx.x & 63;
    char* slab = smem + (wave < 3 ? 32768 + wave * 9216 : 98304 + (wave - 3) * 9216);
#ifdef REVO_EXPERIMENTS
    if (p.stagger_cycles > 0) {
        const int grp = (blockIdx.x >> 3) % p.stagger_groups;
        const long t0 = (long)__builtin_amdgcn_s_memrealtime();
        const long wait = (long)p.stagger_cycles * grp / p.stagger_groups;
        while ((long)__builtin_amdgcn_s_memrealtime() - t0 < wait) __builtin_amdgcn_s_sleep(8);
    }
#endif

    auto tile_row0 = [&](int mi) { return BMR == 256 ? mi * 256 : mi * 192 + (mi > tall0 ? (mi - tall0) * 16 : 0); };
    int sq = __builtin_amdgcn_readfirstlane(slot / n_cnt);
    int mi = m_lo + sq;
    int m0 = tile_row0(mi), n0 = (n_lo + (slot - sq * n_cnt)) * 256;
    bool tall = BMR != 256 && mi >= tall0;
    const bool lnc = (EPI == EPI_BF16 || EPI == EPI_BF16_GELU || EPI == EPI_BF16_ROPE) && p.lnc_stats != nullptr;
    const bool lnf = EPI == EPI_RESID_F32 && p.lnf_stats != nullptr;
    char* lds_raw = smem + G256P_LN_OFF;
    float2* lds_mr = (float2*)(smem + G256P_LN_OFF + LNC_RAW_BYTES);
    float2* lds_st = (float2*)(smem + G256P_LN_OFF);
    if (lnc) lnc_issue_stats(p, m0, lds_raw, wave, lane);
    G256Operand A, B;
    g256_operand_init(A, p.A, p.lda, p.M, m0, wave, lane, BMR == 256 ? 256 : (tall ? 208 : 192));
    g256_operand_init(B, p.B, p.ldb, p.N, n0, wave, lane);
    g256_issue_half(A, 0, 0, G256_A(smem, 0), wave);
    g256_issue_half(A, 1, 0, G256_A(smem, 0), wave);
    g256_issue_half(B, 0, 0, G256_B(smem, 0), wave);
    g256_issue_half(B, 1, 0, G256_B(smem, 0), wave);
    for (;;) {
        if (p.K > 64) {
            g256_issue_half(A, 0, 128, G256_A(smem, 1), wave);
            g256_issue_half(A, 1, 128, G256_A(smem, 1), wave);
        }
        if (lnc && !(REVO_LNC_ABLATE & 1)) lnc_merge_rows(p, lds_raw, lds_mr, wave, lane, p.K <= 64, p.lnc_tele != nullptr && n0 == 0, p.M - m0);
        f32x4 acc[8][4];
#pragma unroll
        for (int m = 0; m < 8; ++m)
#pragma unroll
            for (int n = 0; n < 4; ++n) acc[m][n] = (f32x4){0.f, 0.f, 0.f, 0.f};
        if constexpr (BMR == 256) gemm256_mainloop(A, B, smem, p.K, wave, lane, acc);
        else gemm256_mainloop<192>(A, B, smem, p.K, wave, lane, acc, tall);

        int lane_e = lane;
        if constexpr (EPI != EPI_BF16 && EPI != EPI_BF16_ROPE)
            asm volatile("v_mbcnt_lo_u32_b32 %0, -1, 0\n\tv_mbcnt_hi_u32_b32 %0, -1, %0" : "=v"(lane_e));
        const int mb = m0 + (wave >> 2) * 128, nb = n0 + (wave & 3) * 64;
        GemmArgs pe = p;
        if (BMR != 256) {
            const int mend = m0 + (tall ? 208 : 192);
            pe.M = mend < p.M ? mend : p.M;
        }
        const int m0_done = m0, tn_done = n0 >> 8;
        slot += nslot;
        const bool more = slot < total;
        if (more) {
            sq = __builtin_amdgcn_readfirstlane(slot / n_cnt);
            mi = m_lo + sq;
            m0 = tile_row0(mi);
            n0 = (n_lo + (slot - sq * n_cnt)) * 256;
            tall = BMR != 256 && mi >= tall0;
            if (lnc && !(REVO_LNC_ABLATE & 4)) lnc_issue_stats(p, m0, lds_raw, wave, lane);
            g256_operand_init(A, p.A, p.lda, p.M, m0, wave, lane, BMR == 256 ? 256 : (tall ? 208 : 192));
            g256_operand_init(B, p.B, p.ldb, p.N, n0, wave, lane);
            g256_issue_half(A, 0, 0, G256_A(smem, 0), wave);
            g256_issue_half(A, 1, 0, G256_A(smem, 0), wave);
            g256_issue_half(B, 0, 0, G256_B(smem, 0), wave);
            g256_issue_half(B, 1, 0, G256_B(smem, 0), wave);
        }
        if constexpr (EPI == EPI_PATCH) {
            gemm_epilogue<EPI, 8, 4>(pe, mb, nb, lane_e, acc);
        } else {
            const bool wide = (p.N & 7) == 0 && (p.ldc & 7) == 0;
            if (wide) gemm256_epilogue<EPI, BMR != 256, XP>(pe, slab, mb, nb, lane_e, acc,
                                                            lnf ? lds_st + (wave >> 2) * 128 * 4 + (wave & 3) : nullptr,
                                                            lnc ? lds_mr + (wave >> 2) * 128 : nullptr);
            else gemm_epilogue<EPI, 8, 4>(pe, mb, nb, lane_e, acc);
        }
        if (lnf) {
            asm volatile("s_waitcnt lgkmcnt(0)" ::: "memory");
            __builtin_amdgcn_s_barrier();
            lnf_store_tile_stats(pe, lds_st, m0_done, pe.M, tn_done, wave, lane_e);
            if (!more) break;
            continue;
        }
        if (!more) break;
        __builtin_amdgcn_s_barrier();
    }
}


template <int EPI>
__device__ __forceinline__ void gemm256q_tail(char* smem, int wave) {
    const __attribute__((address_space(4))) GemmArgs* pk0 = (const __attribute__((address_space(4))) GemmArgs*)__builtin_amdgcn_kernarg_segment_ptr();
    if (pk0->qtail_rows <= 0) return;
    const bool lnc = pk0->lnc_stats != nullptr;
    {
        const __attribute__((address_space(4))) GemmArgs& q = *pk0;
        int lane_t;
        asm volatile("v_mbcnt_lo_u32_b32 %0, -1, 0\n\tv_mbcnt_hi_u32_b32 %0, -1, %0" : "=v"(lane_t));
        const int li = lane_t & 15, lq = lane_t >> 4;
        const int tail = q.qtail_rows, Kw = q.K >> 3;
        const __amdgpu_buffer_rsrc_t ars = __builtin_amdgcn_make_buffer_rsrc((void*)(q.A + (long)q.M * q.lda), 0, (int)(tail * q.lda * 2), 0x00020000);
        float* part = (float*)smem;
        for (int strip = blockIdx.x; strip * 16 < q.N; strip += gridDim.x) {
            __builtin_amdgcn_s_barrier();
            f32x4 acc4[4];
#pragma unroll
            for (int m = 0; m < 4; ++m) acc4[m] = (f32x4){0.f, 0.f, 0.f, 0.f};
            const bf16_t* wrow = q.B + (long)(strip * 16 + li) * q.ldb + wave * Kw + lq * 8;
            const int aoff = (li * (int)q.lda + wave * Kw + lq * 8) * 2;
            for (int k0 = 0; k0 < Kw; k0 += 128) {
                bf16x8 wf[4], af[4][4];
#pragma unroll
                for (int s4 = 0; s4 < 4; ++s4) {
                    if (k0 + s4 * 32 < Kw) {
                        wf[s4] = *(const bf16x8*)(wrow + k0 + s4 * 32);
#pragma unroll
                        for (int m = 0; m < 4; ++m)
                            af[s4][m] = __builtin_bit_cast(bf16x8, __builtin_amdgcn_raw_buffer_load_b128(ars, aoff + (m * 16 * (int)q.lda + k0 + s4 * 32) * 2, 0, 0));
                    }
                }
#pragma unroll
                for (int s4 = 0; s4 < 4; ++s4)
                    if (k0 + s4 * 32 < Kw) {
#pragma unroll
                        for (int m = 0; m < 4; ++m) acc4[m] = __builtin_amdgcn_mfma_f32_16x16x32_bf16(wf[s4], af[s4][m], acc4[m], 0, 0, 0);
                    }
            }
#pragma unroll
            for (int m = 0; m < 4; ++m) *(f32x4*)(part + (wave * 64 + m * 16 + li) * 16 + lq * 4) = acc4[m];
            __builtin_amdgcn_s_barrier();
            if (wave < 4) {
                const int tt = wave * 64 + lane_t;
                const int row = tt >> 2, cq = tt & 3;
                f32x4 v = *(const f32x4*)(part + row * 16 + cq * 4);
#pragma unroll
                for (int w = 1; w < 8; ++w) v += *(const f32x4*)(part + (w * 64 + row) * 16 + cq * 4);
                if (row < tail) {
                    const int col = strip * 16 + cq * 4;
                    const long grow = (long)q.M + row;
                    const f32x4 b4 = q.bias ? *(const f32x4*)(q.bias + col) : (f32x4){0.f, 0.f, 0.f, 0.f};
                    if (lnc) {
                        float rstd, mr;
                        lnf_merge(q.lnc_stats + grow * q.lnc_parts, q.lnc_parts, q.lnc_eps, rstd, mr);
                        if (q.lnc_tele && strip == 0 && cq == 0) {
                            unsigned long long* tp = q.lnc_tele;
                            asm volatile("" : "+v"(tp));
                            const float am = __builtin_fabsf(mr);
                            atomicAdd(tp, 1ull);
                            if (am > LNC_TELE_RATIO) atomicAdd(tp + 1, 1ull);
                            if (am > 4.0f * LNC_TELE_RATIO) atomicAdd(tp + 2, 1ull);
                        }
                        const f32x4 c = *(const f32x4*)(q.lnc_c + col);
                        v = v * rstd + (c * mr + b4);
                    } else {
                        v += b4;
                    }
                    if (EPI == EPI_BF16_GELU) v = gelu_erf4(v);
                    uint2 o;
                    o.x = pack_bf16x2(v[0], v[1]);
                    o.y = pack_bf16x2(v[2], v[3]);
                    *(uint2*)((bf16_t*)q.C + grow * q.ldc + col) = o;
                }
            }
        }
    }
}

constexpr int G256Q_STORES = 16;
template <int EPI>
__global__ __launch_bounds__(G256_THREADS, 2) void gemm256q_kernel(GemmArgs p, int nslot) {
    static_assert(EPI == EPI_BF16 || EPI == EPI_BF16_GELU || EPI == EPI_BF16_ROPE, "");
    extern __shared__ __attribute__((aligned(16))) char smem[];
    const int tiles_n = p.N >> 8;
    const int tiles_m = (p.M + 255) >> 8;
    const int gy = p.gy, gx = 8 / gy;
    const int xcd = blockIdx.x & 7;
    const int xi = __builtin_amdgcn_readfirstlane(xcd / gy), xj = xcd - xi * gy;
    const int pm = __builtin_amdgcn_readfirstlane((tiles_m + gx - 1) / gx), pn = __builtin_amdgcn_readfirstlane((tiles_n + gy - 1) / gy);
    const int m_lo = xi * pm, n_lo = xj * pn;
    const int m_cnt = (tiles_m - m_lo) < pm ? (tiles_m - m_lo) : pm;
    const int n_cnt = (tiles_n - n_lo) < pn ? (tiles_n - n_lo) : pn;
    const int total = (m_cnt > 0 && n_cnt > 0) ? m_cnt * n_cnt : 0;
    int slot = blockIdx.x >> 3;
    const int wave = __builtin_amdgcn_readfirstlane(threadIdx.x >> 6);
    if (slot >= total) {
        gemm256q_tail<EPI>(smem, wave);
        return;
    }
    const int lane = threadIdx.x & 63;

    int sq = __builtin_amdgcn_readfirstlane(slot / n_cnt);
    int m0 = (m_lo + sq) * 256, n0 = (n_lo + (slot - sq * n_cnt)) * 256;
    const bool lnc = p.lnc_stats != nullptr;
    char* lds_raw = smem + G256_LDS;
    float2* lds_mr = (float2*)(smem + G256_LDS + LNC_RAW_BYTES);
    float2* lds_mr_next = lds_mr + 256;
    char* lds_bc = smem + G256Q_BC_OFF;
    char* lds_bc_next = lds_bc + 2048;
    auto issue_bias_csum = [&](const float* bias, const float* csum, int N, int n0_, char* dst, int lane_) {
        if (wave == 4 || wave == 5) {
            const float* src = wave == 4 ? bias : csum;
            const __amdgpu_buffer_rsrc_t rs = __builtin_amdgcn_make_buffer_rsrc((void*)(src + n0_), 0, src ? (N - n0_ < 256 ? N - n0_ : 256) * 4 : 0, 0x00020000);
            __builtin_amdgcn_raw_ptr_buffer_load_lds(rs, (__attribute__((address_space(3))) void*)(dst + (wave - 4) * 1024), 16,
                                                     (uint32_t)(lane_ * 16), 0, 0, 0);
        }
    };
    if (lnc) lnc_issue_stats(p, m0, lds_raw, wave, lane);
    issue_bias_csum(p.bias, lnc ? p.lnc_c : nullptr, p.N, n0, lds_bc, lane);
    G256Operand A, B;
    g256_operand_init(A, p.A, p.lda, p.M, m0, wave, lane);
    g256_operand_init(B, p.B, p.ldb, p.N, n0, wave, lane);
    g256_issue_prologue(A, B, smem, p.K, wave);
    G256_FENCE();
    {
        const __amdgpu_buffer_rsrc_t none = __builtin_amdgcn_make_buffer_rsrc(p.C, 0, 0, 0x00020000);
        typedef uint32_t u32x4 __attribute__((ext_vector_type(4)));
#pragma unroll
        for (int i = 0; i < G256Q_STORES; ++i)
            __builtin_amdgcn_raw_buffer_store_b128((u32x4){0u, 0u, 0u, 0u}, none, i * 16, 0, 0);
    }
    G256_FENCE();
#ifdef REVO_EXPERIMENTS
    int tiles_done = 0;
#endif
    if (lnc) lnc_merge_rows<G256Q_STORES>(p, lds_raw, lds_mr, wave, lane, false, p.lnc_tele != nullptr && n0 == 0, p.M - m0);
    else if (threadIdx.x < 512) lds_mr[threadIdx.x] = make_float2(1.f, 0.f);
    for (;;) {
        f32x4 acc[8][4];
#pragma unroll
        for (int m = 0; m < 8; ++m)
#pragma unroll
            for (int n = 0; n < 4; ++n) acc[m][n] = (f32x4){0.f, 0.f, 0.f, 0.f};
#ifdef REVO_EXPERIMENTS
        unsigned long long t_a = 0, t_b = 0, t_c = 0, c_a = 0;
        if (p.stamps) { t_a = __builtin_amdgcn_s_memrealtime(); c_a = __builtin_amdgcn_s_memtime(); }
#endif
        gemm256_mainloop<0, false, false, G256Q_STORES>(A, B, smem, p.K, wave, lane, acc);
#ifdef REVO_EXPERIMENTS
        if (p.stamps) { t_b = __builtin_amdgcn_s_memrealtime(); c_a = __builtin_amdgcn_s_memtime() - c_a; }
#endif

        const __attribute__((address_space(4))) GemmArgs* pk = (const __attribute__((address_space(4))) GemmArgs*)__builtin_amdgcn_kernarg_segment_ptr();
        asm volatile("" : "+s"(pk));
        const __attribute__((address_space(4))) GemmArgs& q = *pk;
        int lane_e;
        asm volatile("v_mbcnt_lo_u32_b32 %0, -1, 0\n\tv_mbcnt_hi_u32_b32 %0, -1, %0" : "=v"(lane_e));
        const int lr = lane_e & 15, lq = lane_e >> 4;
        const int wr = wave >> 2, wc = wave & 3;
        const int m0_done = m0, n0_done = n0;
        const int nb = n0_done + wc * 64;
        slot += nslot;
        const bool more = slot < total;
        float2 st8[8];
#pragma unroll
        for (int m = 0; m < 8; ++m) st8[m] = lds_mr[wr * 128 + m * 16 + lr];
        f32x4 bias4[4], c4[4];
#pragma unroll
        for (int n = 0; n < 4; ++n) {
            bias4[n] = *(const f32x4*)(lds_bc + (wc * 64 + n * 16 + lq * 4) * 4);
            c4[n] = *(const f32x4*)(lds_bc + 1024 + (wc * 64 + n * 16 + lq * 4) * 4);
        }
        asm volatile("s_waitcnt lgkmcnt(0)" ::: "memory");
        G256_FENCE();
        const bool rot = EPI == EPI_BF16_ROPE && nb < q.rope_cols;
        __amdgpu_buffer_rsrc_t rtab = __builtin_amdgcn_make_buffer_rsrc((void*)q.rope_cs, 0, EPI == EPI_BF16_ROPE ? q.rope_S * (q.rope_hd >> 1) * 8 : 0, 0x00020000);
        int tok = 0, cpair[4] = {0, 0, 0, 0};
        if (EPI == EPI_BF16_ROPE) {
            tok = (m0_done + wr * 128 + lr) % q.rope_S;
            int c0 = (nb + lq * 4) % q.rope_hd;
#pragma unroll
            for (int n = 0; n < 4; ++n) {
                cpair[n] = (c0 >> 1) * 8;
                c0 += 16;
                if (c0 >= q.rope_hd) c0 -= q.rope_hd;
            }
        }
        const int tok_row_bytes = (q.rope_hd >> 1) * 8;
        f32x4 rt[2][2][4];
        auto rope_load = [&](auto bufc) {
            constexpr int buf = decltype(bufc)::value;
#pragma unroll
            for (int mm = 0; mm < 2; ++mm) {
#pragma unroll
                for (int n = 0; n < 4; ++n)
                    rt[buf][mm][n] = __builtin_bit_cast(f32x4, __builtin_amdgcn_raw_buffer_load_b128(rtab, tok * tok_row_bytes + cpair[n], 0, 0));
                tok += 16;
                if (tok >= q.rope_S) tok -= q.rope_S;
            }
        };
        using I0 = std::integral_constant<int, 0>; using I1 = std::integral_constant<int, 1>;
        using I2 = std::integral_constant<int, 2>; using I3 = std::integral_constant<int, 3>;
        if (rot) { rope_load(I0{}); rope_load(I1{}); }
        if (rot) {
#pragma unroll
            for (int i = 0; i < 2; ++i)
#pragma unroll
                for (int mm = 0; mm < 2; ++mm)
#pragma unroll
                    for (int n = 0; n < 4; ++n) asm volatile("" : "+v"(rt[i][mm][n]));
        }
        G256_FENCE();
        if (more) {
            sq = __builtin_amdgcn_readfirstlane(slot / n_cnt);
            m0 = (m_lo + sq) * 256;
            n0 = (n_lo + (slot - sq * n_cnt)) * 256;
            if (lnc) lnc_issue_stats(q, m0, lds_raw, wave, lane_e);
            issue_bias_csum(q.bias, lnc ? q.lnc_c : nullptr, q.N, n0, lds_bc_next, lane_e);
            g256_operand_init(A, q.A, q.lda, q.M, m0, wave, lane_e);
            g256_operand_init(B, q.B, q.ldb, q.N, n0, wave, lane_e);
            g256_issue_prologue(A, B, smem, q.K, wave);
        }
        G256_FENCE();
        typedef uint32_t u32x2 __attribute__((ext_vector_type(2)));
        typedef uint32_t u32x4 __attribute__((ext_vector_type(4)));
        const long rows_here = (long)q.M - m0_done < 256 ? (long)q.M - m0_done : 256;
#ifdef REVO_EXPERIMENTS
        const bool drop_stores = (q.stagger_groups & 0x100) != 0;
#else
        constexpr bool drop_stores = false;
#endif
        const __amdgpu_buffer_rsrc_t crs = __builtin_amdgcn_make_buffer_rsrc(
            (void*)((bf16_t*)q.C + (long)m0_done * q.ldc + n0_done), 0, drop_stores ? 0 : (int)((rows_here - 1) * q.ldc * 2 + 512), 0x00020000);
        const int rstep = (int)(q.ldc * 32);
        int voff = (wr * 128 + lr) * (int)(q.ldc * 2) + (wc * 64 + (lq & 1) * 16 + (lq >> 1) * 8) * 2;
        auto quarter = [&](auto qc, auto bufc) {
            u32x4 out[2][2];
            constexpr int q = decltype(qc)::value, buf = decltype(bufc)::value;
#pragma unroll
            for (int mm = 0; mm < 2; ++mm) {
                constexpr int dummy_ = 0; (void)dummy_;
                const int m = q * 2 + mm;
                const float2 st = st8[m];
                uint32_t d[4][2];
#pragma unroll
                for (int n0f = 0; n0f < 4; n0f += 2) {
                    f32x4 v[2];
#pragma unroll
                    for (int n = 0; n < 2; ++n) v[n] = acc[m][n0f + n] * st.x + (c4[n0f + n] * st.y + bias4[n0f + n]);
                    if (EPI == EPI_BF16_GELU) gelu_erf4xn<2>(v);
#pragma unroll
                    for (int n = 0; n < 2; ++n) {
                        uint32_t w0 = pack_bf16x2(v[n][0], v[n][1]), w1 = pack_bf16x2(v[n][2], v[n][3]);
                        if (EPI == EPI_BF16_ROPE) {
                            if (rot) {
                                const f32x4 tc = rt[buf][mm][n0f + n];
                                const float a0 = __uint_as_float(w0 << 16), a1 = __uint_as_float(w0 & 0xffff0000u);
                                const float b0 = __uint_as_float(w1 << 16), b1 = __uint_as_float(w1 & 0xffff0000u);
                                w0 = pack_bf16x2(a0 * tc[0] - a1 * tc[1], a1 * tc[0] + a0 * tc[1]);
                                w1 = pack_bf16x2(b0 * tc[2] - b1 * tc[3], b1 * tc[2] + b0 * tc[3]);
                            }
                        }
                        d[n0f + n][0] = w0;
                        d[n0f + n][1] = w1;
                    }
                }
#pragma unroll
                for (int P = 0; P < 2; ++P) {
                    const u32x2 s0 = __builtin_amdgcn_permlane16_swap(d[2 * P][0], d[2 * P + 1][0], false, false);
                    const u32x2 s1 = __builtin_amdgcn_permlane16_swap(d[2 * P][1], d[2 * P + 1][1], false, false);
                    out[mm][P] = (u32x4){s0[0], s1[0], s0[1], s1[1]};
                }
            }
            G256_FENCE();
#pragma unroll
            for (int mm = 0; mm < 2; ++mm) {
                constexpr int aux = (EPI == EPI_BF16_ROPE || EPI == EPI_BF16_GELU) ? 2 : 0;
                __builtin_amdgcn_raw_buffer_store_b128(out[mm][0], crs, voff, 0, aux);
                __builtin_amdgcn_raw_buffer_store_b128(out[mm][1], crs, voff + 64, 0, aux);
                voff += rstep;
            }
            G256_FENCE();
        };
#ifdef REVO_EXPERIMENTS
        if (q.stamps) t_c = __builtin_amdgcn_s_memrealtime();
#endif
        quarter(I0{}, I0{});
        if (rot) rope_load(I0{});
        quarter(I1{}, I1{});
        if (rot) rope_load(I1{});
        quarter(I2{}, I0{});
        quarter(I3{}, I1{});
        G256_FENCE();
#ifdef REVO_EXPERIMENTS
        if (q.stamps && wave == 0 && lane_e == 0 && tiles_done < q.stamp_items) {
            unsigned long long* dst = q.stamps + ((size_t)blockIdx.x * q.stamp_items + tiles_done) * 4;
            dst[0] = t_a; dst[1] = t_b; dst[2] = (q.stagger_groups & 0x200) ? c_a : t_c; dst[3] = __builtin_amdgcn_s_memrealtime();
        }
        ++tiles_done;
#endif
        if (!more) break;
        if (lnc) {
            lnc_merge_rows<G256Q_STORES>(q, lds_raw, lds_mr_next, wave, lane_e, false, q.lnc_tele != nullptr && n0 == 0, q.M - m0);
        }
        { float2* t = lds_mr; lds_mr = lds_mr_next; lds_mr_next = t; }
        { char* t = lds_bc; lds_bc = lds_bc_next; lds_bc_next = t; }
    }
    gemm256q_tail<EPI>(smem, wave);
}

#ifdef REVO_EXPERIMENTS
template <int EPI, int BMR = 256>
__global__ __launch_bounds__(G256_THREADS, 2) void gemm256pp_kernel(GemmArgs p, int nslot, int groups) {
    static_assert(BMR == 256 || BMR == 192, "");
    extern __shared__ __attribute__((aligned(16))) char smem[];
    const int tiles_n = (p.N + 255) / 256;
    const int tiles_m = BMR == 256 ? (p.M + 255) / 256 : p.t192_tiles;
    const int tall0 = tiles_m - (BMR == 256 ? 0 : p.t192_tall);
    const int gy = p.gy, gx = 8 / gy;
    const int xcd = blockIdx.x & 7;
    const int xi = xcd / gy, xj = xcd - xi * gy;
    const int pm = (tiles_m + gx - 1) / gx, pn = (tiles_n + gy - 1) / gy;
    const int m_lo = xi * pm, n_lo = xj * pn;
    const int m_cnt = (tiles_m - m_lo) < pm ? (tiles_m - m_lo) : pm;
    const int n_cnt = (tiles_n - n_lo) < pn ? (tiles_n - n_lo) : pn;
    const int total = (m_cnt > 0 && n_cnt > 0) ? m_cnt * n_cnt : 0;
    const int slot0 = blockIdx.x >> 3;
    if (slot0 >= total) return;
    const int wave = __builtin_amdgcn_readfirstlane(threadIdx.x >> 6);
    const int lane = threadIdx.x & 63;
    const int wr = wave >> 2;
    char* slab = smem + (wave < 3 ? 32768 + wave * 9216 : 98304 + (wave - 3) * 9216);

    auto tile_row0 = [&](int mi) { return BMR == 256 ? mi * 256 : mi * 192 + (mi > tall0 ? (mi - tall0) * 16 : 0); };
    const int ntiles = (total - slot0 + nslot - 1) / nslot;
    const int grp = (slot0 / n_cnt) % groups;
    const int h = 64 * (((grp + 1) * (BMR / 64) + groups - 1) / groups);
    const bool first_tall = BMR != 256 && (m_lo + slot0 / n_cnt) >= tall0;
    const bool split = h < BMR && ntiles >= 2 && !first_tall;
    const int nitems = ntiles + (split ? 1 : 0);

    int m0, n0, rows;
    auto item = [&](int it) {
        const bool last_piece = split && it == nitems - 1;
        const int s = last_piece ? slot0 : slot0 + it * nslot;
        const int mi = m_lo + s / n_cnt;
        n0 = (n_lo + s % n_cnt) * 256;
        m0 = tile_row0(mi);
        rows = BMR == 256 ? 256 : (mi >= tall0 ? 208 : 192);
        if (split && it == 0) rows = h;
        if (last_piece) { m0 += h; rows = BMR - h; }
    };
    item(0);
    G256Operand A, B;
    g256_operand_init(A, p.A, p.lda, p.M, m0, wave, lane, rows);
    g256_operand_init(B, p.B, p.ldb, p.N, n0, wave, lane);
    g256_issue_half(A, 0, 0, G256_A(smem, 0), wave);
    g256_issue_half(A, 1, 0, G256_A(smem, 0), wave);
    g256_issue_half(B, 0, 0, G256_B(smem, 0), wave);
    g256_issue_half(B, 1, 0, G256_B(smem, 0), wave);
    for (int it = 0;;) {
        if (p.K > 64) {
            g256_issue_half(A, 0, 128, G256_A(smem, 1), wave);
            g256_issue_half(A, 1, 128, G256_A(smem, 1), wave);
        }
        f32x4 acc[8][4];
#pragma unroll
        for (int m = 0; m < 8; ++m)
#pragma unroll
            for (int n = 0; n < 4; ++n) acc[m][n] = (f32x4){0.f, 0.f, 0.f, 0.f};
        const bool do_lo = wr == 0 ? true : rows > 128;
        const bool do_hi = wr == 0 ? rows > 64 : rows >= 256;
        const bool do_ht = wr == 1 && rows == 208;
#ifdef REVO_EXPERIMENTS
        unsigned long long t_a = 0, t_b = 0;
        if (p.stamps) t_a = __builtin_amdgcn_s_memrealtime();
#endif
        gemm256_mainloop<0, true>(A, B, smem, p.K, wave, lane, acc, do_ht, do_lo, do_hi);
#ifdef REVO_EXPERIMENTS
        if (p.stamps) t_b = __builtin_amdgcn_s_memrealtime();
#endif

        const int mb = m0 + wr * 128, nb = n0 + (wave & 3) * 64;
        GemmArgs pe = p;
        {
            const int mend = m0 + rows;
            pe.M = mend < p.M ? mend : p.M;
        }
// ... 168 lines not shown
```

revers-o_amd/csrc/gemm_plan.h:

```cpp
#pragma once
#include "kernels.h"

namespace revo {

struct GemmKnobs {
    int force_tile = 0;
    int force_gy = 0;
    int min_tiles256 = 100;
    int persistent = 1;
    int qstores = 1;
    int qtail = 1;
    int ring = 1;
    int ring_max_tiles = 256;
    int tail_split = 1;
    int splitk = 1;
    int rows192 = 1;
    int lnf = 1;
    int ln_planes = 1;
#ifdef REVO_EXPERIMENTS
    int dbg = 0;
    int phase_groups = 0;
    int stagger_cycles = 0, stagger_groups = 2;
#endif
};

struct GemmProblem {
    int epi;
    int M, N, K;
    long lda, ldb, ldc;
    int prefer256;
    long ws_elems;
    bool ln_offered;
    long ln_ldo;
    bool fold_offered;
    long lnf_ldxb;
    int xp_in, xp_out;
    bool planes_valid;
    int rope_S, rope_hd, rope_cols;
    bool lnc;
};
static GemmProblem gemm_problem(int epi, const GemmArgs& a) {
    GemmProblem p{};
    p.epi = epi; p.M = a.M; p.N = a.N; p.K = a.K; p.lda = a.lda; p.ldb = a.ldb; p.ldc = a.ldc; p.prefer256 = a.prefer256;
    p.ws_elems = a.ws ? a.ws_elems : 0;
    p.ln_offered = a.ln_out && a.ln_fused; p.ln_ldo = a.ln_ldo;
    p.fold_offered = a.lnf_xb && a.lnf_stats && a.lnf_done; p.lnf_ldxb = a.lnf_ldxb;
    p.xp_in = a.xp_in; p.xp_out = a.xp_out;
    p.planes_valid = a.xp_hi && a.xp_lo && a.xp_ld % 8 == 0 && (!a.xp_out || a.xp_hi == a.lnf_xb);
    p.rope_S = a.rope_S; p.rope_hd = a.rope_hd; p.rope_cols = a.rope_cols;
    p.lnc = a.lnc_stats != nullptr;
    return p;
}

struct GemmStep {
    unsigned form;
    int row0, rows;
    int gy;
    int nslot;
    int grid_x, grid_y;
    int t192_tiles, t192_tall;
    int qtail_rows;
    int S;
    bool reduce_ln;
    int xp;
    bool fold;
    int dbg;
};
struct GemmPlan {
    const char* error;
    int nsteps;
    GemmStep step[2];
    unsigned forms;
};

#ifdef REVO_EXPERIMENTS
constexpr bool G256Q_ROPE_BUILT = true;
#else
constexpr bool G256Q_ROPE_BUILT = false;
#endif

static const char* gemm_shape_error(int M, int N, int K, long lda, long ldb, long ldc) {
    if (K <= 0 || K % 64) return "gemm: K must be a positive multiple of 64";
    if (N % 4) return "gemm: N must be a multiple of 4";
    if (M <= 0 || N <= 0) return "gemm: empty problem";
    if (lda % 8 || ldb % 8) return "gemm: lda/ldb must be multiples of 8 (16-byte rows)";
    if (ldc % 4) return "gemm: ldc must be a multiple of 4";
    return nullptr;
}

static bool gemm_window_ok(long ld, long rows = 256) { return rows * ld * 2 < (1l << 31); }
static long gemm_tiles256(int M, int N) { return (long)((M + 255) / 256) * ((N + 255) / 256); }
static bool gemm_persistent(const GemmKnobs& k, int M, int N, int K) { return k.persistent && K >= 128 && gemm_tiles256(M, N) > 256; }

static int gemm_xcd_stripes(int tiles_n) { return tiles_n >= 24 ? 4 : (tiles_n >= 8 ? 2 : 1); }
static int gemm_xcd_region(int tiles_m, int tiles_n, int gy) { return ((tiles_m + 8 / gy - 1) / (8 / gy)) * ((tiles_n + gy - 1) / gy); }
static void gemm_xcd_grid(GemmStep& s, int tiles_m, int tiles_n, const GemmKnobs& k, bool persistent) {
    s.gy = k.force_gy ? k.force_gy : gemm_xcd_stripes(tiles_n);
    const int region = gemm_xcd_region(tiles_m, tiles_n, s.gy);
    if (persistent) s.nslot = region < 32 ? region : 32;
    s.grid_x = 8 * (persistent ? s.nslot : region);
    s.grid_y = 1;
}

struct GemmRounds { long tm, tn, full, rem; };
static GemmRounds gemm_rounds(int M, int N) {
    const long tm = (M + 255) / 256, tn = (N + 255) / 256;
    return {tm, tn, tm * tn / 256, tm * tn % 256};
}
static bool gemm_tail_splits(const GemmRounds& r, const GemmKnobs& k) { return k.tail_split && r.full > 0 && r.rem > 0 && r.rem <= 160; }

static bool gemm_use_skinny(const GemmKnobs& k, int M, int N, int K) { return k.force_tile == 0 && M <= 64 && K % 256 == 0 && N >= 256; }
static bool gemm_use_256(const GemmProblem& p, const GemmKnobs& k) {
    if (!gemm_window_ok(p.lda) || !gemm_window_ok(p.ldb)) return false;
    if (k.force_tile == 256) return true;
    if (k.force_tile == 128) return false;
    return p.M >= 1024 && p.N >= 256 && gemm_tiles256(p.M, p.N) >= k.min_tiles256;
}
static bool gemm_use_256q(const GemmProblem& p, const GemmKnobs& k) {
    const int e = p.epi;
    if (!(e == EPI_BF16 || e == EPI_BF16_GELU || (e == EPI_BF16_ROPE && G256Q_ROPE_BUILT)) || !k.qstores) return false;
    if (p.N % 256 || p.K < 128 || (p.ldc & 7) || !gemm_window_ok(p.ldc)) return false;
    if (e == EPI_BF16_ROPE && (p.rope_cols % 64 || (long)p.rope_S * (p.rope_hd >> 1) * 8 >= (1l << 31))) return false;
    if (e == EPI_BF16_ROPE && (k.qstores & 7) != 3) return false;
    return true;
}

static int gemm_plan_rows192(const GemmProblem& p, const GemmKnobs& k, int* tall) {
    if (!k.rows192 || k.force_tile || p.K < 128 || p.M % 16) return 0;
    const long tn = (p.N + 255) / 256, T = p.M / 192, e = (p.M - T * 192) / 16;
    if (e > T || e > 8) return 0;
    const long tiles192 = T * tn, rounds192 = (tiles192 + 255) / 256;
    if (tiles192 <= 256 || rounds192 * 256 - tiles192 > tiles192 / 32) return 0;
    const GemmRounds r = gemm_rounds(p.M, p.N);
// ... 148 lines not shown
```

revers-o_amd/csrc/kernels.h:

```cpp
#pragma once
#include "common.h"

namespace revo {

enum GemmEpi {
    EPI_BF16 = 0,
    EPI_BF16_GELU = 1,
    EPI_RESID_F32 = 2,
    EPI_F32 = 3,
    EPI_PATCH = 4,
    EPI_BF16_ROPE = 5,
};

struct GemmArgs {
    const bf16_t* A; long lda;
    const bf16_t* B; long ldb;
    int M, N, K;
    void* C; long ldc;
    const float* bias;
    const float* gamma;
    const float* pos;
    int S, G2, cls;
    int gy;
    const float2* rope_cs;
    int rope_S, rope_hd, rope_cols;
    int prefer256;
    float* ws; long ws_elems;
    int t192_tiles, t192_tall;
    int ksplit; long c_split_stride;
    const float* ln_w; const float* ln_b; float ln_eps; bf16_t* ln_out; long ln_ldo; int* ln_fused;
    bf16_t* lnf_xb; long lnf_ldxb; float2* lnf_stats; int* lnf_done;
    bf16_t* xp_hi; bf16_t* xp_lo; long xp_ld; int xp_in, xp_out;
    const float2* lnc_stats; int lnc_parts; const float* lnc_c; float lnc_eps;
    unsigned long long* lnc_tele;
    int qtail_rows;
#ifdef REVO_EXPERIMENTS
    int stagger_cycles, stagger_groups;
    unsigned long long* stamps; int stamp_items;
#endif
};
constexpr float LNC_TELE_RATIO = 8.0f;
constexpr int LNF_SLICE = 256;
int launch_gemm(int epi, const GemmArgs& a, hipStream_t st);
enum GemmForm : unsigned {
    GF_SKINNY_444 = 1u << 0,
    GF_SKINNY_411 = 1u << 1,
    GF_128_128 = 1u << 2,
    GF_128_64 = 1u << 3,
    GF_128R = 1u << 4,
    GF_256_TILE = 1u << 5,
    GF_256P = 1u << 6,
    GF_256P_192 = 1u << 7,
    GF_256Q = 1u << 8,
    GF_256Q_QTAIL = 1u << 9,
    GF_SPLITK_RING = 1u << 10,
    GF_SPLITK_RING_LN = 1u << 11,
    GF_SPLITK_256 = 1u << 12,
    GF_LN_FOLDED = 1u << 13,
    GF_LN_CONSUMED = 1u << 14,
    GF_PLANES_IN = 1u << 15,
    GF_PLANES_OUT = 1u << 16,
};
#ifdef REVO_EXPERIMENTS
unsigned gemm_debug_forms(int reset);
long gemm_debug_plan(int epi, int M, int N, int K, long lda, long ldb, long ldc, long ws_elems, unsigned offers, int rope_S,
                     int rope_hd, int rope_cols, long* out, int cap);
#endif
int launch_gemm_f32_ring(const GemmArgs& a, hipStream_t st);
bool gemm_resid_folds(int M, int N, int K, long lda, long ldb, long ldc);
int launch_planes_to_f32(const bf16_t* hi, const bf16_t* lo, long ldp, float* x, long ldx, long rows, int W, hipStream_t st);
#ifdef REVO_EXPERIMENTS
void gemm_set_debug(int d);
void gemm_set_stagger(int cycles, int groups);
void gemm_set_stamps(unsigned long long* buf, int items);
void gemm_set_phase_groups(int g);
#endif
void gemm_force_gy(int gy);
void gemm_set_tail_split(int on);
void gemm_force_tile(int t);

constexpr int LN_MAXH = 16;
struct LnLogits { const float* qk; const float* ck; float* logits; int H, S; };
int launch_layernorm(const float* x, long ldx, const float* w, const float* b, float eps, int rows, int W,
                     void* out, long ldo, int out_is_bf16, hipStream_t st, const LnLogits* logits = nullptr);
int launch_fold_ln_linear(const float* w, const float* gamma, const float* beta, const float* bias, int rows, int cols,
                          bf16_t* out, long ld, float* csum, float* bias_out, hipStream_t st);
int launch_patchify(const void* images, int is_u8, int B, int img, int P, bf16_t* out, long Kp, hipStream_t st);
int launch_probe_qk(const float* q, const float* Wk, const float* bk, int W, int heads, float* qk, float* ck, hipStream_t st);
int launch_pool_head_rows(const float* x, long ldx, int B, int S, int W, int H, const float* logits, float* u, hipStream_t st);
int launch_pool_head_rows_masked(const float* x, long ldx, int B, int S, int W, int H, const float* logits,
                                 const int* region_image, const uint32_t* region_bits, int R, float* u, hipStream_t st);
int launch_zero_empty_regions(const uint32_t* region_bits, int R, int S, int D, float* out, hipStream_t st);
int launch_gemm_f32_skinny(int epi, const float* A, long lda, long a_group_stride, int group_cols, const float* Wt, long ldw,
                           const float* bias, int M, int N, int K, float* C, long ldc, hipStream_t st);
int launch_transpose_f32(const float* src, int rows, int cols, float* dst, hipStream_t st);
int launch_split_hi_lo_hi(const float* src, long rows, int cols, float scale, bf16_t* dst, long ld, hipStream_t st);
int launch_cls_rows(float* x, long ldx, const float* cls, const float* pos, int B, int S, int W, hipStream_t st);
int launch_rope(bf16_t* qkv, long ld, const float2* cs, int rows, int S, int W, int heads, hipStream_t st);
int launch_f32_to_bf16(const float* src, long ld_src, bf16_t* dst, long ld_dst, long rows, int cols, hipStream_t st);
int launch_l2norm_rows(const float* src, long ld_src, float* dst_f32, long ld_f32, bf16_t* dst_bf16, long ld_bf16,
                       long rows, int D, hipStream_t st, int normalize = 1, float* row_stats = nullptr,
                       uint32_t* max_stats = nullptr, uint32_t* zero_a = nullptr, long zero_a_words = 0,
                       uint32_t* zero_b = nullptr, long zero_b_words = 0, const long long* dst_rows = nullptr);

constexpr long REMOVE_MAX_CHUNK = 65536;
int launch_remove_count(const uint32_t* bits, long N, long chunk, uint32_t* cnt, uint32_t* first, hipStream_t st);
int launch_remove_gather(const uint32_t* bits, long N, long row0, long len, long j0, const uint4* src, uint4* dst,
                         int u4_per_row, hipStream_t st);

int launch_attention(const bf16_t* qkv, long ld, bf16_t* out, long ldo, int B, int S, int H, int hd, hipStream_t st);
int launch_attention_ex(const bf16_t* qkv, long ld, bf16_t* out, long ldo, int B, int S, int H, int hd, int has_cls,
                        hipStream_t st);
constexpr int ATTC_MAX_S = 128;
int launch_attention_causal(const bf16_t* qkv, long ld, bf16_t* out, long ldo, int B, int S, int H, int hd, hipStream_t st);
int launch_embed_tokens(const int32_t* tokens, const float* table, const float* pos, int B, int S, int vocab, int W, float* x,
                        long ldx, hipStream_t st);
int launch_pool_eot(const int32_t* tokens, const float* x, long ldx, int B, int S, int W, float* out, hipStream_t st);
void gemm_set_min_tiles256(int n);
void gemm_set_ring(int on, int max_tiles);
void gemm_set_splitk(int on);
void gemm_set_persistent(int on);
void gemm_set_qstores(int on);
void gemm_set_rows192(int on);
void gemm_set_ln_fold(int on);
bool gemm_ln_planes_enabled();
void attention_force_nw(int nw);
void attention_set_shape16(int on);
#ifdef REVO_EXPERIMENTS
void attention_set_clock_buffer(unsigned long long* buf);
#endif

struct ScanArgs {
    const bf16_t* Qb; long ldq;
    const bf16_t* Gb; long ldg;
    int Q; long N; int D;
    int ksel;
    int splits;
    uint64_t* part;
    const uint32_t* allow;
};
int topk_scan_workspace_splits(int Q, long N);
int launch_topk_scan(const ScanArgs& a, hipStream_t st);
int launch_topk_reduce(uint64_t* part, int Q, int splits, int ksel, hipStream_t st);
constexpr int EXACT_COL_CAP = 2048;
constexpr int EXACT_L3_SLICES = 32;
static_assert(EXACT_L3_SLICES * 64 == EXACT_COL_CAP, "the brute-force partial lists live in the collect buffer");
enum ExactCtr : int {
    CTR_UNCERTIFIED,
    CTR_BRUTEFORCE,
    CTR_CHECKED,
    CTR_COLLECTED,
    CTR_MODE3_FAILED,
// ... 445 lines not shown
```

revers-o_amd/csrc/tower.h:

```cpp
#pragma once
#include <algorithm>
#include <cstdlib>
#include <cstring>
#include <map>
#include <string>
#include <utility>
#include <vector>

#include "api_internal.h"
#include "kernels.h"

struct LayerW {
    bf16_t *w_qkv, *w_o, *w_fc1, *w_fc2;
    float *b_qkv, *b_o, *b_fc1, *b_fc2, *c_qkv, *c_fc1, *ls1, *ls2;
};

constexpr size_t SPLITK_WS_ELEMS = 16u << 20;

using NeedList = std::vector<std::pair<std::string, int64_t>>;

struct WeightMap {
    std::map<std::string, const revo_tensor*> m;
    int fill(const char* who, const revo_tensor* weights, int n_weights) {
        for (int i = 0; i < n_weights; ++i) {
            REVO_REQUIRE(weights[i].name && weights[i].data, std::string(who) + ": weight entry with a null name or data pointer");
            m[weights[i].name] = &weights[i];
        }
        return 0;
    }
    const revo_tensor* get(const std::string& name, int64_t numel) {
        auto it = m.find(name);
        if (it == m.end()) { revo_set_error("missing weight tensor: " + name); return nullptr; }
        if (it->second->numel != numel) {
            revo_set_error("weight " + name + ": expected " + std::to_string(numel) + " elements, got " +
                           std::to_string(it->second->numel));
            return nullptr;
        }
        return it->second;
    }
};

static inline void need_blocks(NeedList& need, const std::string& prefix, int layers, int W, int M, int use_ls) {
    for (int i = 0; i < layers; ++i) {
        const std::string p = prefix + std::to_string(i) + ".";
        for (const char* n : {"ln_1.weight", "ln_1.bias", "ln_2.weight", "ln_2.bias", "attn.out_proj.bias", "mlp.c_proj.bias"})
            need.push_back({p + n, W});
        need.push_back({p + "attn.in_proj_weight", (int64_t)3 * W * W});
        need.push_back({p + "attn.in_proj_bias", 3 * W});
        need.push_back({p + "attn.out_proj.weight", (int64_t)W * W});
        need.push_back({p + "mlp.c_fc.weight", (int64_t)M * W});
        need.push_back({p + "mlp.c_fc.bias", M});
        need.push_back({p + "mlp.c_proj.weight", (int64_t)W * M});
        if (use_ls) { need.push_back({p + "ls_1.gamma", W}); need.push_back({p + "ls_2.gamma", W}); }
    }
}

static inline int check_checkpoint(WeightMap& wm, const NeedList& need, const char* reader, int use_ls) {
    for (auto& kv : need)
        if (!wm.get(kv.first, kv.second)) return -2;
    if (wm.m.size() != need.size()) {
        std::map<std::string, int64_t> want(need.begin(), need.end());
        for (auto& kv : wm.m)
            if (!want.count(kv.first)) {
                revo_set_error("unexpected weight tensor: " + kv.first + " (not read by " + reader +
                               (use_ls ? ")" : "; LayerScale needs cfg.use_ls = 1)"));
                return -2;
            }
    }
    return 0;
}

struct TowerCore {
    int device = 0, max_batch = 0, debug_layers = -1;
    int W = 0, Md = 0; float ln_eps = 0.f;
    std::vector<LayerW> layers;
    float* x = nullptr;
    bf16_t *h = nullptr, *qkv = nullptr, *att = nullptr, *mlp = nullptr;
    bf16_t* xlo = nullptr;
    float2* ln_stats = nullptr;
    int ln_parts = 0;
    unsigned long long* ln_tele = nullptr;
    float* splitk_ws = nullptr;
    std::vector<void*> owned;

    template <class T> int dalloc(T** out, size_t count) {
        void* p = nullptr;
        REVO_HIP_CHECK(hipMalloc(&p, count * sizeof(T) + 256));
        owned.push_back(p);
        *out = (T*)p;
        return 0;
    }
    ~TowerCore() { for (void* p : owned) (void)hipFree(p); }
};

struct Staging {
    float *stage = nullptr, *gb = nullptr;
    int alloc(int W, int M, long largest_other) {
        const size_t stage_elems = (size_t)std::max({(long)3 * W * W, (long)M * W, largest_other});
        REVO_HIP_CHECK(hipMalloc((void**)&stage, stage_elems * 4));
        REVO_HIP_CHECK(hipMalloc((void**)&gb, (size_t)(2 * W + std::max(3 * W, M)) * 4));
        return 0;
    }
    ~Staging() { (void)hipFree(stage); (void)hipFree(gb); }
};

static inline int up_f32(TowerCore* v, WeightMap& wm, const std::string& name, int64_t numel, float** out) {
    const revo_tensor* t = wm.get(name, numel);
    if (!t) return -2;
    CHECK_RC(v->dalloc(out, (size_t)numel));
    REVO_HIP_CHECK(hipMemcpy(*out, t->data, (size_t)numel * 4, hipMemcpyDefault));
    return 0;
}
static inline int up_folded(TowerCore* v, WeightMap& wm, const Staging& s, const std::string& wname, const std::string& bname,
                            const std::string& ln, int64_t rows, int64_t cols, bf16_t** w_out, float** c_out, float** b_out) {
    const revo_tensor *tw = wm.get(wname, rows * cols), *tb = wm.get(bname, rows), *tg = wm.get(ln + ".weight", cols),
                      *te = wm.get(ln + ".bias", cols);
    if (!tw || !tb || !tg || !te) return -2;
    float *stage = s.stage, *gb = s.gb;
    CHECK_RC(v->dalloc(w_out, (size_t)(rows * cols)));
    CHECK_RC(v->dalloc(c_out, (size_t)rows));
    CHECK_RC(v->dalloc(b_out, (size_t)rows));
    REVO_HIP_CHECK(hipMemcpy(stage, tw->data, (size_t)(rows * cols) * 4, hipMemcpyDefault));
    REVO_HIP_CHECK(hipMemcpy(gb, tg->data, (size_t)cols * 4, hipMemcpyDefault));
    REVO_HIP_CHECK(hipMemcpy(gb + cols, te->data, (size_t)cols * 4, hipMemcpyDefault));
    REVO_HIP_CHECK(hipMemcpy(gb + 2 * cols, tb->data, (size_t)rows * 4, hipMemcpyDefault));
    CHECK_RC(revo::launch_fold_ln_linear(stage, gb, gb + cols, gb + 2 * cols, (int)rows, (int)cols, *w_out, cols, *c_out, *b_out, 0));
    REVO_HIP_CHECK(hipStreamSynchronize(0));
    return 0;
}
static inline int up_bf16(TowerCore* v, WeightMap& wm, const Staging& s, const std::string& name, int64_t rows, int64_t cols,
                          bf16_t** out) {
    const revo_tensor* t = wm.get(name, rows * cols);
    if (!t) return -2;
    CHECK_RC(v->dalloc(out, (size_t)(rows * cols)));
    REVO_HIP_CHECK(hipMemcpy(s.stage, t->data, (size_t)(rows * cols) * 4, hipMemcpyDefault));
    CHECK_RC(revo::launch_f32_to_bf16(s.stage, cols, *out, cols, rows, (int)cols, 0));
    REVO_HIP_CHECK(hipStreamSynchronize(0));
    return 0;
}
static inline int upload_blocks(TowerCore* v, WeightMap& wm, const Staging& s, const std::string& prefix, int layers, int use_ls) {
    const int W = v->W, M = v->Md;
    v->layers.resize(layers);
    for (int i = 0; i < layers; ++i) {
        const std::string p = prefix + std::to_string(i) + ".";
        LayerW& L = v->layers[i];
        memset(&L, 0, sizeof(L));
        CHECK_RC(up_folded(v, wm, s, p + "attn.in_proj_weight", p + "attn.in_proj_bias", p + "ln_1", 3 * W, W, &L.w_qkv, &L.c_qkv,
                           &L.b_qkv));
        CHECK_RC(up_bf16(v, wm, s, p + "attn.out_proj.weight", W, W, &L.w_o));
        CHECK_RC(up_f32(v, wm, p + "attn.out_proj.bias", W, &L.b_o));
        CHECK_RC(up_folded(v, wm, s, p + "mlp.c_fc.weight", p + "mlp.c_fc.bias", p + "ln_2", M, W, &L.w_fc1, &L.c_fc1, &L.b_fc1));
        CHECK_RC(up_bf16(v, wm, s, p + "mlp.c_proj.weight", W, M, &L.w_fc2));
        CHECK_RC(up_f32(v, wm, p + "mlp.c_proj.bias", W, &L.b_fc2));
        if (use_ls) {
            CHECK_RC(up_f32(v, wm, p + "ls_1.gamma", W, &L.ls1));
            CHECK_RC(up_f32(v, wm, p + "ls_2.gamma", W, &L.ls2));
        }
    }
    return 0;
}
static inline int upload_projT(TowerCore* v, WeightMap& wm, const Staging& s, const std::string& name, int D, float** out) {
    const int W = v->W;
    const revo_tensor* t = wm.get(name, (int64_t)W * D);
    if (!t) return -2;
    CHECK_RC(v->dalloc(out, (size_t)D * W));
    REVO_HIP_CHECK(hipMemcpy(s.stage, t->data, (size_t)W * D * 4, hipMemcpyDefault));
    CHECK_RC(revo::launch_transpose_f32(s.stage, W, D, *out, 0));
    REVO_HIP_CHECK(hipStreamSynchronize(0));
    return 0;
}
static inline int alloc_body(TowerCore* v, size_t rows) {
    const size_t W = (size_t)v->W;
    CHECK_RC(v->dalloc(&v->x, rows * W));
    CHECK_RC(v->dalloc(&v->h, rows * W));
    CHECK_RC(v->dalloc(&v->qkv, rows * 3 * W));
    CHECK_RC(v->dalloc(&v->att, rows * W));
    CHECK_RC(v->dalloc(&v->mlp, rows * (size_t)v->Md));
    CHECK_RC(v->dalloc(&v->splitk_ws, SPLITK_WS_ELEMS));
    v->ln_parts = (W % 256 == 0 && W / 256 <= 6) ? (int)(W / 256) : 0;
    if (v->ln_parts) CHECK_RC(v->dalloc(&v->ln_stats, rows * (size_t)v->ln_parts));
    if (v->ln_parts) CHECK_RC(v->dalloc(&v->xlo, rows * W));
    CHECK_RC(v->dalloc(&v->ln_tele, 4));
    REVO_HIP_CHECK(hipMemset(v->ln_tele, 0, 4 * sizeof(unsigned long long)));
    return 0;
}

struct PinnedStage {
    void* p = nullptr; hipEvent_t ev = nullptr; bool pending = false;
    int alloc(size_t bytes) {
        REVO_HIP_CHECK(hipHostMalloc(&p, bytes, hipHostMallocDefault));
        REVO_HIP_CHECK(hipEventCreateWithFlags(&ev, hipEventDisableTiming));
        return 0;
    }
    int wait() {
        if (pending) REVO_HIP_CHECK(hipEventSynchronize(ev));
        return 0;
    }
    int record(hipStream_t st) {
        REVO_HIP_CHECK(hipEventRecord(ev, st));
        pending = true;
        return 0;
    }
    ~PinnedStage() {
        if (p) (void)hipHostFree(p);
        if (ev) (void)hipEventDestroy(ev);
    }
};

static inline revo::GemmArgs gemm_args(const void* A, long lda, const void* B, long ldb, int M, int N, int K, void* C, long ldc) {
    revo::GemmArgs a{};
    a.A = (const bf16_t*)A; a.lda = lda; a.B = (const bf16_t*)B; a.ldb = ldb; a.M = M; a.N = N; a.K = K; a.C = C; a.ldc = ldc;
    return a;
}

struct LnAfter { float eps; bf16_t* out; long ldo; int* fused; float2* stats; int* folded; bf16_t* lo; int x_in_planes, planes_out; };
static inline int gemm(const char* cls, int epi, const bf16_t* A, long lda, const bf16_t* B, long ldb, int M, int N, int K, void* C,
                       long ldc, const float* bias, const float* gamma, hipStream_t st, float* ws = nullptr, long ws_elems = 0,
                       const LnAfter* ln = nullptr) {
    revo::GemmArgs a = gemm_args(A, lda, B, ldb, M, N, K, C, ldc);
    a.bias = bias; a.gamma = gamma; a.ws = ws; a.ws_elems = ws_elems;
    if (ln) {
        a.ln_eps = ln->eps; a.ln_ldo = ln->ldo; a.ln_fused = ln->fused;
        if (ln->fused) a.ln_out = ln->out;
        if (ln->stats) { a.lnf_xb = ln->out; a.lnf_ldxb = ln->ldo; a.lnf_stats = ln->stats; a.lnf_done = ln->folded; }
        if (ln->lo) { a.xp_hi = ln->out; a.xp_lo = ln->lo; a.xp_ld = ln->ldo; a.xp_in = ln->x_in_planes; a.xp_out = ln->planes_out; }
    }
    ProfScope ps(cls, st);
    return revo::launch_gemm(epi, a, st);
}

static inline bool stream_in_planes(const TowerCore& t, int rows) {
    const int W = t.W, Md = t.Md;
    return t.xlo && revo::gemm_ln_planes_enabled() && revo::gemm_resid_folds(rows, W, W, W, W, W) &&
           revo::gemm_resid_folds(rows, W, Md, Md, Md, W);
}

template <class QkvArgs, class Attention>
int body_blocks(const TowerCore& t, const char* who, int rows, int nl, hipStream_t st, QkvArgs&& qkv_args, Attention&& attention) {
    using namespace revo;
    const int W = t.W, Md = t.Md;
    enum { H_NONE = 0, H_NORM = 1, H_XB = 2 };
    int h_state = H_NONE;
    float2* stats = t.ln_stats;
    bf16_t* xlo = stream_in_planes(t, rows) ? t.xlo : nullptr;
    bool x_planes = false;
    auto ln_before = [&](const float* csum, GemmArgs& a) {
        if (h_state == H_XB) { a.lnc_stats = stats; a.lnc_parts = t.ln_parts; a.lnc_c = csum; a.lnc_eps = t.ln_eps; a.lnc_tele = t.ln_tele; }
    };
    auto normalise_if_needed = [&]() -> int {
        if (h_state != H_NONE) return 0;
        if (x_planes) { revo_set_error(std::string(who) + ": internal: a LayerNorm kernel was asked for while the stream is in planes"); return -3; }
        ProfScope ps("layernorm", st);
        CHECK_RC(launch_layernorm(t.x, W, nullptr, nullptr, t.ln_eps, rows, W, t.h, W, 1, st));
        h_state = H_NORM;
        return 0;
    };
    for (int i = 0; i < nl; ++i) {
        const LayerW& L = t.layers[i];
        CHECK_RC(normalise_if_needed());
        {
            GemmArgs a{};
            a.A = t.h; a.lda = W; a.B = L.w_qkv; a.ldb = W; a.M = rows; a.N = 3 * W; a.K = W; a.C = t.qkv;
            a.ldc = 3 * W; a.bias = L.b_qkv;
            const int epi = qkv_args(a);
            ln_before(L.c_qkv, a);
            ProfScope ps("gemm_qkv", st);
            CHECK_RC(launch_gemm(epi, a, st));
        }
        { ProfScope ps("attention", st);
          CHECK_RC(attention()); }
        int fused = 0, folded = 0;
        const LnAfter ln2{t.ln_eps, t.h, W, &fused, stats, &folded, xlo, x_planes ? 1 : 0, xlo ? 1 : 0};
        CHECK_RC(gemm("gemm_out", EPI_RESID_F32, t.att, W, L.w_o, W, rows, W, W, t.x, W, L.b_o, L.ls1, st, t.splitk_ws,
                      (long)SPLITK_WS_ELEMS, &ln2));
        h_state = folded ? H_XB : (fused ? H_NORM : H_NONE);
        x_planes = xlo && folded;
#ifdef REVO_EXPERIMENTS
        if (folded && getenv("REVO_LNFOLD_TOUCH")) {
            ProfScope ps("touch", st);
            REVO_HIP_CHECK(hipMemcpyAsync(t.qkv, t.h, (size_t)rows * W * 2, hipMemcpyDeviceToDevice, st));
        }
#endif
        CHECK_RC(normalise_if_needed());
        {
            GemmArgs a{};
            a.A = t.h; a.lda = W; a.B = L.w_fc1; a.ldb = W; a.M = rows; a.N = Md; a.K = W; a.C = t.mlp; a.ldc = Md;
            a.bias = L.b_fc1;
            ln_before(L.c_fc1, a);
            ProfScope ps("gemm_fc1", st);
            CHECK_RC(launch_gemm(EPI_BF16_GELU, a, st));
        }
        fused = 0; folded = 0;
        const bool last = i + 1 >= nl;
        const LnAfter ln1n{t.ln_eps, t.h, W, last ? nullptr : &fused, last ? nullptr : stats, last ? nullptr : &folded, xlo,
                           x_planes ? 1 : 0, (xlo && !last) ? 1 : 0};
        CHECK_RC(gemm("gemm_fc2", EPI_RESID_F32, t.mlp, Md, L.w_fc2, Md, rows, W, Md, t.x, W, L.b_fc2, L.ls2, st,
                      t.splitk_ws, (long)SPLITK_WS_ELEMS, (!last || x_planes) ? &ln1n : nullptr));
        h_state = last ? H_NONE : (folded ? H_XB : (fused ? H_NORM : H_NONE));
        x_planes = !last && xlo && folded;
#ifdef REVO_EXPERIMENTS
        if (folded && !last && getenv("REVO_LNFOLD_TOUCH")) {
            ProfScope ps("touch", st);
            REVO_HIP_CHECK(hipMemcpyAsync(t.qkv, t.h, (size_t)rows * W * 2, hipMemcpyDeviceToDevice, st));
        }
#endif
    }
    return 0;
}
```

Before: 2516.

## Merge LayerNorm partial statistics once in producer GEMM via tickets

The residual GEMM that produces LayerNorm partial statistics now also finalises them into per-row (rstd, -mean*rstd) pairs, using per-row-block tickets so the last contributing tile does the merge. Consumer GEMMs (qkv, fc1) load the merged pair directly instead of loading 1..6 partial slots and merging them in every tile. This removes redundant per-tile merge work and LDS staging in the consumer kernels. In exchange it adds atomic ticket coordination and an extra write in the producer epilogue, plus persistent ticket and merged-statistics buffers.

After: 2515. About the same (-0.1%).

```diff
diff --git a/include/revo.h b/include/revo.h
--- a/include/revo.h
+++ b/include/revo.h
@@ -160,6 +160,14 @@
 int32_t revo_op_gemm_ln_in(int32_t epilogue, const void* a_bf16, int64_t lda, const void* b_bf16, int64_t ldb, int32_t m, int32_t n,
                            int32_t k, void* c_bf16, int64_t ldc, const float* bias, const float* csum, const void* stats,
                            int32_t parts, float eps, void* tele, void* stream);
+int32_t revo_op_gemm_resid_ln_merged(const void* a_bf16, int64_t lda, const void* b_bf16, int64_t ldb, int32_t m, int32_t n,
+                                     int32_t k, float* c, int64_t ldc, const float* bias, const float* gamma, void* xb_bf16,
+                                     int64_t ldxb, void* stats, float eps, void* mr, void* tickets, int32_t* done, void* xlo_bf16,
+                                     int32_t x_in_planes, int32_t planes_out);
+int32_t revo_op_gemm_ln_in_merged(int32_t epilogue, const void* a_bf16, int64_t lda, const void* b_bf16, int64_t ldb, int32_t m,
+                                  int32_t n, int32_t k, void* c_bf16, int64_t ldc, const float* bias, const float* csum,
+                                  const void* mr, void* tele, const float* cos_sin, int32_t seq, int32_t head_dim,
+                                  int32_t rope_cols);
 int32_t revo_op_gemm_ln_in_rope(const void* a_bf16, int64_t lda, const void* b_bf16, int64_t ldb, int32_t m, int32_t n, int32_t k,
                                 void* c_bf16, int64_t ldc, const float* bias, const float* csum, const void* stats, int32_t parts,
                                 float eps, const float* cos_sin, int32_t seq, int32_t head_dim, int32_t rope_cols, void* stream);
diff --git a/revers-o_amd/_lib.py b/revers-o_amd/_lib.py
--- a/revers-o_amd/_lib.py
+++ b/revers-o_amd/_lib.py
@@ -94,6 +94,9 @@
     "revo_op_gemm_resid_ln": (_i32, [_p, _i64, _p, _i64, _i32, _i32, _i32, _p, _i64, _p, _p, _p, _i64, _p, C.POINTER(C.c_int32), _p, _i32,
                                      _i32, _p]),
     "revo_op_gemm_ln_in": (_i32, [_i32, _p, _i64, _p, _i64, _i32, _i32, _i32, _p, _i64, _p, _p, _p, _i32, _f32, _p, _p]),
+    "revo_op_gemm_resid_ln_merged": (_i32, [_p, _i64, _p, _i64, _i32, _i32, _i32, _p, _i64, _p, _p, _p, _i64, _p, _f32, _p, _p,
+                                            C.POINTER(C.c_int32), _p, _i32, _i32]),
+    "revo_op_gemm_ln_in_merged": (_i32, [_i32, _p, _i64, _p, _i64, _i32, _i32, _i32, _p, _i64, _p, _p, _p, _p, _p, _i32, _i32, _i32]),
     "revo_op_gemm_rope": (_i32, [_p, _i64, _p, _i64, _i32, _i32, _i32, _p, _i64, _p, _p, _i32, _i32, _i32, _p]),
     "revo_op_gemm_ln_in_rope": (_i32, [_p, _i64, _p, _i64, _i32, _i32, _i32, _p, _i64, _p, _p, _p, _i32, _f32, _p, _i32, _i32, _i32,
                                        _p]),
diff --git a/revers-o_amd/csrc/api.hip b/revers-o_amd/csrc/api.hip
--- a/revers-o_amd/csrc/api.hip
+++ b/revers-o_amd/csrc/api.hip
@@ -110,6 +110,18 @@
         return -1;
     }
 };
+struct OpMerged {
+    float2* p = nullptr; hipStream_t st; int rc = 0;
+    OpMerged(hipStream_t s, const void* stats, int parts, float eps, long rows) : st(s) {
+        if (rows <= 0) { revo_set_error("op_gemm_ln_in: empty problem"); rc = -2; return; }
+        const hipError_t e = hipMallocAsync((void**)&p, (size_t)rows * sizeof(float2), st);
+        if (e != hipSuccess) { revo_set_error(std::string("hipMallocAsync(merged statistics): ") + hipGetErrorString(e)); p = nullptr; rc = -1; return; }
+        rc = revo::launch_ln_merge_slots((const float2*)stats, parts, eps, rows, p, st);
+    }
+    OpMerged(const OpMerged&) = delete;
+    ~OpMerged() { if (p) (void)hipFreeAsync(p, st); }
+    int status() const { return rc; }
+};
 }
 
 extern "C" int32_t revo_op_gemm(int32_t epi, const void* a, int64_t lda, const void* b, int64_t ldb, int32_t m,
@@ -144,16 +156,54 @@
     return rc;
     API_END
 }
+extern "C" int32_t revo_op_gemm_resid_ln_merged(const void* a, int64_t lda, const void* b, int64_t ldb, int32_t m, int32_t n,
+                                                int32_t k, float* c, int64_t ldc, const float* bias, const float* gamma, void* xb,
+                                                int64_t ldxb, void* stats, float eps, void* mr, void* tickets, int32_t* done,
+                                                void* xlo, int32_t x_in_planes, int32_t planes_out) {
+    API_BEGIN
+    REVO_REQUIRE(a && b && c && xb && stats && mr && tickets && done, "op_gemm_resid_ln_merged: null argument");
+    REVO_REQUIRE(xlo || (!x_in_planes && !planes_out), "op_gemm_resid_ln_merged: planes need the low plane");
+    hipStream_t st = nullptr;
+    OpScratch ws(st);
+    CHECK_RC(ws.status());
+    revo::GemmArgs g = gemm_args(a, lda, b, ldb, m, n, k, c, ldc);
+    g.bias = bias; g.gamma = gamma; g.ws = ws.p; g.ws_elems = OP_WS_ELEMS;
+    int flag = 0;
+    g.lnf_xb = (bf16_t*)xb; g.lnf_ldxb = ldxb; g.lnf_stats = (float2*)stats; g.lnf_done = &flag;
+    g.ln_eps = eps; g.lnf_mr = (float2*)mr; g.lnf_tickets = (unsigned*)tickets;
+    if (xlo) { g.xp_hi = (bf16_t*)xb; g.xp_lo = (bf16_t*)xlo; g.xp_ld = ldxb; g.xp_in = x_in_planes != 0; g.xp_out = planes_out != 0; }
+    const int rc = revo::launch_gemm(revo::EPI_RESID_F32, g, st);
+    *done = flag;
+    return rc;
+    API_END
+}
 extern "C" int32_t revo_op_gemm_ln_in(int32_t epi, const void* a, int64_t lda, const void* b, int64_t ldb, int32_t m, int32_t n,
                                       int32_t k, void* c, int64_t ldc, const float* bias, const float* csum, const void* stats,
                                       int32_t parts, float eps, void* tele, void* stream) {
     API_BEGIN
     REVO_REQUIRE(epi == revo::EPI_BF16 || epi == revo::EPI_BF16_GELU, "op_gemm_ln_in: epilogue must be 0 (bf16) or 1 (bf16 + GELU)");
     REVO_REQUIRE(a && b && c && csum && stats, "op_gemm_ln_in: null argument");
-    revo::GemmArgs g = gemm_args(a, lda, b, ldb, m, n, k, c, ldc);
-    g.bias = bias; g.lnc_stats = (const float2*)stats; g.lnc_parts = parts; g.lnc_c = csum; g.lnc_eps = eps;
+    hipStream_t st = (hipStream_t)stream;
+    OpMerged mr(st, stats, parts, eps, m);
+    CHECK_RC(mr.status());
+    revo::GemmArgs g = gemm_args(a, lda, b, ldb, m, n, k, c, ldc);
+    g.bias = bias; g.lnc_mr = mr.p; g.lnc_c = csum;
     g.lnc_tele = (unsigned long long*)tele;
-    return revo::launch_gemm(epi, g, (hipStream_t)stream);
+    return revo::launch_gemm(epi, g, st);
+    API_END
+}
+extern "C" int32_t revo_op_gemm_ln_in_merged(int32_t epi, const void* a, int64_t lda, const void* b, int64_t ldb, int32_t m,
+                                             int32_t n, int32_t k, void* c, int64_t ldc, const float* bias, const float* csum,
+                                             const void* mr, void* tele, const float* cos_sin, int32_t seq, int32_t head_dim,
+                                             int32_t rope_cols) {
+    API_BEGIN
+    REVO_REQUIRE(epi == revo::EPI_BF16 || epi == revo::EPI_BF16_GELU || epi == revo::EPI_BF16_ROPE,
+                 "op_gemm_ln_in_merged: epilogue must be 0 (bf16), 1 (bf16 + GELU) or 5 (bf16 + RoPE)");
+    REVO_REQUIRE(a && b && c && csum && mr && (epi != revo::EPI_BF16_ROPE || cos_sin), "op_gemm_ln_in_merged: null argument");
+    revo::GemmArgs g = gemm_args(a, lda, b, ldb, m, n, k, c, ldc);
+    g.bias = bias; g.lnc_mr = (const float2*)mr; g.lnc_c = csum; g.lnc_tele = (unsigned long long*)tele;
+    if (epi == revo::EPI_BF16_ROPE) { g.rope_cs = (const float2*)cos_sin; g.rope_S = seq; g.rope_hd = head_dim; g.rope_cols = rope_cols; }
+    return revo::launch_gemm(epi, g, nullptr);
     API_END
 }
 extern "C" int32_t revo_op_gemm_rope(const void* a, int64_t lda, const void* b, int64_t ldb, int32_t m, int32_t n,
@@ -171,10 +221,13 @@
                                            int32_t rope_cols, void* stream) {
     API_BEGIN
     REVO_REQUIRE(a && b && c && csum && stats && cos_sin, "op_gemm_ln_in_rope: null argument");
+    hipStream_t st = (hipStream_t)stream;
+    OpMerged mr(st, stats, parts, eps, m);
+    CHECK_RC(mr.status());
     revo::GemmArgs g = gemm_args(a, lda, b, ldb, m, n, k, c, ldc);
     g.bias = bias; g.rope_cs = (const float2*)cos_sin; g.rope_S = seq; g.rope_hd = head_dim; g.rope_cols = rope_cols;
-    g.lnc_stats = (const float2*)stats; g.lnc_parts = parts; g.lnc_c = csum; g.lnc_eps = eps;
-    return revo::launch_gemm(revo::EPI_BF16_ROPE, g, (hipStream_t)stream);
+    g.lnc_mr = mr.p; g.lnc_c = csum;
+    return revo::launch_gemm(revo::EPI_BF16_ROPE, g, st);
     API_END
 }
 extern "C" int32_t revo_op_gemm_resid_norm(const void* a, int64_t lda, const void* b, int64_t ldb, int32_t m, int32_t n, int32_t k,
diff --git a/revers-o_amd/csrc/gemm.hip b/revers-o_amd/csrc/gemm.hip
--- a/revers-o_amd/csrc/gemm.hip
+++ b/revers-o_amd/csrc/gemm.hip
@@ -40,6 +40,13 @@
     return !pl.error && pl.step[0].fold;
 }
 
+int launch_ln_merge_slots(const float2* stats, int parts, float eps, long rows, float2* mr, hipStream_t st) {
+    REVO_REQUIRE(stats && mr && rows > 0 && parts >= 1 && parts <= 6, "ln merge: needs 1..6 statistics slots per row");
+    hipLaunchKernelGGL(ln_merge_slots_kernel, dim3((unsigned)((rows + 255) / 256)), dim3(256), 0, st, stats, parts, eps, rows, mr);
+    REVO_HIP_CHECK(hipGetLastError());
+    return 0;
+}
+
 template <int EPI, int BMR>
 static int launch_256p(GemmArgs& b, const GemmStep& s, hipStream_t st) {
     int nslot = s.nslot;
@@ -117,9 +124,9 @@
     b.M = s.rows;
     b.A = a.A + (long)s.row0 * a.lda;
     b.C = (char*)a.C + (long)s.row0 * a.ldc * (BF16 ? 2 : 4);
-    if (b.lnc_stats) b.lnc_stats += (long)s.row0 * a.lnc_parts;
+    if (b.lnc_mr) b.lnc_mr += s.row0;
     b.gy = s.gy; b.t192_tiles = s.t192_tiles; b.t192_tall = s.t192_tall; b.qtail_rows = s.qtail_rows;
-    if (!s.fold) { b.lnf_xb = nullptr; b.lnf_stats = nullptr; }
+    if (!s.fold) { b.lnf_xb = nullptr; b.lnf_stats = nullptr; b.lnf_mr = nullptr; b.lnf_tickets = nullptr; }
     if (!s.xp) b.xp_in = b.xp_out = 0;
     switch (s.form) {
         case GF_SKINNY_444:
@@ -211,8 +218,12 @@
         revo_set_error(e);
         return -2;
     }
-    if (a.lnc_stats && (!a.lnc_c || a.lnc_parts < 1 || a.lnc_parts > 6 || (epi != EPI_BF16 && epi != EPI_BF16_GELU && epi != EPI_BF16_ROPE))) {
-        revo_set_error("gemm: a folded LayerNorm (lnc_*) needs a bf16 epilogue, the column sums and 1..6 statistics slots per row");
+    if (a.lnc_mr && (!a.lnc_c || (epi != EPI_BF16 && epi != EPI_BF16_GELU && epi != EPI_BF16_ROPE))) {
+        revo_set_error("gemm: a folded LayerNorm (lnc_*) needs a bf16 epilogue and the column sums");
+        return -2;
+    }
+    if (((uintptr_t)a.lnc_mr | (uintptr_t)a.lnf_mr) & 15) {
+        revo_set_error("gemm: the merged row statistics must be 16-byte aligned");
         return -2;
     }
     if (epi == EPI_BF16_ROPE && (!a.rope_cs || a.rope_S <= 0 || a.rope_hd <= 0 || a.rope_hd % 8 || a.rope_cols % a.rope_hd || a.rope_cols > a.N)) {
diff --git a/revers-o_amd/csrc/gemm_kernels.h b/revers-o_amd/csrc/gemm_kernels.h
--- a/revers-o_amd/csrc/gemm_kernels.h
+++ b/revers-o_amd/csrc/gemm_kernels.h
@@ -78,29 +78,21 @@
     v += __builtin_bit_cast(float, __builtin_amdgcn_update_dpp(0, __builtin_bit_cast(int, v), 0x140, 0xf, 0xf, true));
     return v;
 }
-__device__ __forceinline__ void lnf_merge(const float2* part, int P, float eps, float& rstd, float& mr) {
-    float sm = 0.f, sq = 0.f;
-    for (int i = 0; i < P; ++i) { const float2 t = part[i]; sm += t.x; sq += t.y; }
-    const float mean = sm / (float)P;
-    float dd = 0.f;
-    for (int i = 0; i < P; ++i) { const float d = part[i].x - mean; dd = fmaf(d, d, dd); }
-    const float var = fmaf((float)LNF_SLICE, dd, sq) / (float)(LNF_SLICE * P);
-    rstd = rsqrtf(var + eps);
-    mr = -mean * rstd;
-}
 
 template <int EPI, int MF, int NF>
 __device__ __forceinline__ void gemm_epilogue(const GemmArgs& p, int m_base, int n_base, int lane,
                                               f32x4 (&acc)[MF][NF]) {
     const int lr = lane & 15, lq = lane >> 4;
-    const bool lnc = (EPI == EPI_BF16 || EPI == EPI_BF16_GELU || EPI == EPI_BF16_ROPE) && p.lnc_stats != nullptr;
+    const bool lnc = (EPI == EPI_BF16 || EPI == EPI_BF16_GELU || EPI == EPI_BF16_ROPE) && p.lnc_mr != nullptr;
 #pragma unroll
     for (int m = 0; m < MF; ++m) {
         const int row = m_base + m * 16 + lr;
         if (row >= p.M) continue;
         float ln_rstd = 1.f, ln_mr = 0.f;
-        if (lnc)
-            lnf_merge(p.lnc_stats + (long)row * p.lnc_parts, p.lnc_parts, p.lnc_eps, ln_rstd, ln_mr);
+        if (lnc) {
+            const float2 st = p.lnc_mr[row];
+            ln_rstd = st.x; ln_mr = st.y;
+        }
         long orow = row;
         int prow = 0;
         if (EPI == EPI_PATCH) {
@@ -468,77 +460,53 @@
     }
 }
 
-constexpr int LNC_RAW_BYTES = 256 * 6 * 8 + 1024, LNC_MR_BYTES = 256 * 8;
+constexpr int LNC_MR_BYTES = 256 * 8, LNF_ST_BYTES = 256 * 4 * 8;
 constexpr int G256P_LN_OFF = 98304 + 5 * 9216;
-static_assert(G256P_LN_OFF + LNC_RAW_BYTES + LNC_MR_BYTES <= 163840, "");
-constexpr int G256_LDS_LN = G256_LDS + LNC_RAW_BYTES + LNC_MR_BYTES;
-constexpr int G256Q_BC_OFF = G256_LDS_LN + LNC_MR_BYTES;
-constexpr int G256Q_LDS = G256Q_BC_OFF + 2 * 2048;
+static_assert(G256P_LN_OFF + 2 * LNC_MR_BYTES <= 163840, "");
+static_assert(G256P_LN_OFF + LNF_ST_BYTES <= 163840, "");
+constexpr int G256_LDS_LN = G256_LDS + LNC_MR_BYTES;
+constexpr int G256Q_BC_OFF = G256_LDS;
+constexpr int G256Q_BC_BYTES = 2048 + LNC_MR_BYTES;
+constexpr int G256Q_LDS = G256Q_BC_OFF + 2 * G256Q_BC_BYTES;
 static_assert(G256Q_LDS <= 163840, "");
 template <class ARGS>
-__device__ __forceinline__ void lnc_issue_stats(const ARGS& p, int m0, char* lds_raw, int wave, int ) {
+__device__ __forceinline__ void lnc_issue_mr(const ARGS& p, int m0, char* lds_mr, int wave, int wave0 = 0) {
+    if (wave != wave0 && wave != wave0 + 1) return;
+    int lane;
+    asm volatile("v_mbcnt_lo_u32_b32 %0, -1, 0\n\tv_mbcnt_hi_u32_b32 %0, -1, %0" : "=v"(lane) :: "memory");
+    long left = ((long)p.M - m0) * 8;
+    left = left < 0 ? 0 : (left > LNC_MR_BYTES ? LNC_MR_BYTES : left);
+    const __amdgpu_buffer_rsrc_t rs = __builtin_amdgcn_make_buffer_rsrc((void*)(p.lnc_mr + m0), 0, (int)left, 0x00020000);
+    const int off = (wave - wave0) * 1024;
+    __builtin_amdgcn_raw_ptr_buffer_load_lds(rs, (__attribute__((address_space(3))) void*)(lds_mr + off), 16,
+                                             (uint32_t)(off + lane * 16), 0, 0, 0);
+}
+template <class ARGS = GemmArgs>
+__device__ __forceinline__ void lnc_tele_count(const ARGS& p, float m, int wave, int rows_left) {
     if (wave >= 4) return;
     int lane;
     asm volatile("v_mbcnt_lo_u32_b32 %0, -1, 0\n\tv_mbcnt_hi_u32_b32 %0, -1, %0" : "=v"(lane) :: "memory");
-    const int P = p.lnc_parts;
-    long left = ((long)p.M - m0) * P * 8;
-    const long full = 256l * P * 8;
-    left = left < 0 ? 0 : (left > full ? full : left);
-    const __amdgpu_buffer_rsrc_t rs = __builtin_amdgcn_make_buffer_rsrc((void*)(p.lnc_stats + (long)m0 * P), 0, (int)left, 0x00020000);
-    const int share = 512 * P, pieces = (share + 1023) >> 10;
-    for (int j = 0; j < pieces; ++j) {
-        const int off = wave * share + j * 1024;
-        if (off + 1024 <= LNC_RAW_BYTES)
-            __builtin_amdgcn_raw_ptr_buffer_load_lds(rs, (__attribute__((address_space(3))) void*)(lds_raw + off), 16,
-                                                     (uint32_t)(off + lane * 16), 0, 0, 0);
-    }
-}
-template <int VM = 4, class ARGS = GemmArgs>
-__device__ __forceinline__ void lnc_merge_rows(const ARGS& p, const char* lds_raw, float2* lds_mr, int wave, int , bool one_ktile,
-                                               bool tele = false, int rows_left = 0) {
-    if (wave >= 4) return;
+    const int live = rows_left - wave * 64 < 0 ? 0 : (rows_left - wave * 64 > 64 ? 64 : rows_left - wave * 64);
+    const float am = lane < live ? __builtin_fabsf(m) : 0.f;
+    const unsigned long long big = __builtin_amdgcn_ballot_w64(am > LNC_TELE_RATIO);
+    const unsigned long long huge = __builtin_amdgcn_ballot_w64(am > 4.0f * LNC_TELE_RATIO);
+    if (lane == 0 && live > 0) {
+        unsigned long long* tp = p.lnc_tele;
+        asm volatile("" : "+v"(tp));
+        atomicAdd(tp, (unsigned long long)live);
+        if (big) atomicAdd(tp + 1, (unsigned long long)__builtin_popcountll(big));
+        if (huge) atomicAdd(tp + 2, (unsigned long long)__builtin_popcountll(huge));
+    }
+}
+__device__ __forceinline__ float lnc_tele_read(const float2* lds_mr, int wave) {
+    if (wave >= 4) return 0.f;
     int lane;
     asm volatile("v_mbcnt_lo_u32_b32 %0, -1, 0\n\tv_mbcnt_hi_u32_b32 %0, -1, %0" : "=v"(lane) :: "memory");
-    if (one_ktile) asm volatile("s_waitcnt vmcnt(0)" ::: "memory");
-    else asm volatile("s_waitcnt vmcnt(%0)" :: "n"(VM) : "memory");
-    const int t = wave * 64 + lane;
-    if (t < 256) {
-        float r, m;
-        auto merge_n = [&](auto np) {
-            constexpr int NP = decltype(np)::value;
-            f32x4 v[NP / 2];
-#pragma unroll
-            for (int i = 0; i < NP / 2; ++i) v[i] = *(const f32x4*)(lds_raw + t * (NP * 8) + i * 16);
-            float sm = 0.f, sq = 0.f;
-#pragma unroll
-            for (int i = 0; i < NP; ++i) { sm += v[i >> 1][(i & 1) * 2]; sq += v[i >> 1][(i & 1) * 2 + 1]; }
-            const float mean = sm / (float)NP;
-            float dd = 0.f;
-#pragma unroll
-            for (int i = 0; i < NP; ++i) { const float d = v[i >> 1][(i & 1) * 2] - mean; dd = fmaf(d, d, dd); }
-            const float var = fmaf((float)LNF_SLICE, dd, sq) / (float)(LNF_SLICE * NP);
-            r = rsqrtf(var + p.lnc_eps);
-            m = -mean * r;
-        };
-        if (p.lnc_parts == 4) merge_n(std::integral_constant<int, 4>{});
-        else if (p.lnc_parts == 6) merge_n(std::integral_constant<int, 6>{});
-        else lnf_merge((const float2*)lds_raw + t * p.lnc_parts, p.lnc_parts, p.lnc_eps, r, m);
-        lds_mr[t] = make_float2(r, m);
-        if (tele) {
-            const int live = rows_left - wave * 64 < 0 ? 0 : (rows_left - wave * 64 > 64 ? 64 : rows_left - wave * 64);
-            const float am = lane < live ? __builtin_fabsf(m) : 0.f;
-            const unsigned long long big = __builtin_amdgcn_ballot_w64(am > LNC_TELE_RATIO);
-            const unsigned long long huge = __builtin_amdgcn_ballot_w64(am > 4.0f * LNC_TELE_RATIO);
-            if (lane == 0 && live > 0) {
-                unsigned long long* tp = p.lnc_tele;
-                asm volatile("" : "+v"(tp));
-                atomicAdd(tp, (unsigned long long)live);
-                if (big) atomicAdd(tp + 1, (unsigned long long)__builtin_popcountll(big));
-                if (huge) atomicAdd(tp + 2, (unsigned long long)__builtin_popcountll(huge));
-            }
-        }
-    }
-    asm volatile("s_waitcnt lgkmcnt(0)" ::: "memory");
+    return lds_mr[wave * 64 + lane].y;
+}
+template <class ARGS = GemmArgs>
+__device__ __forceinline__ void lnc_tele_rows(const ARGS& p, const float2* lds_mr, int wave, int rows_left) {
+    lnc_tele_count(p, lnc_tele_read(lds_mr, wave), wave, rows_left);
 }
 __device__ __forceinline__ void lnf_store_tile_stats(const GemmArgs& p, const float2* lds_st, int m0, int mend, int tn, int wave,
                                                      int lane) {
@@ -549,8 +517,81 @@
         const float mean = ((a.x + b.x) + (c.x + d.x)) * 0.25f;
         const float da = a.x - mean, db = b.x - mean, dc = c.x - mean, dd = d.x - mean;
         const float m2 = ((a.y + b.y) + (c.y + d.y)) + 64.0f * (fmaf(da, da, db * db) + fmaf(dc, dc, dd * dd));
-        p.lnf_stats[(long)(m0 + t) * (p.N / LNF_SLICE) + tn] = make_float2(mean, m2);
-    }
+        __hip_atomic_store((unsigned long long*)(p.lnf_stats + (long)(m0 + t) * (p.N / LNF_SLICE) + tn),
+                           __builtin_bit_cast(unsigned long long, make_float2(mean, m2)), __ATOMIC_RELAXED, __HIP_MEMORY_SCOPE_AGENT);
+    }
+}
+template <int NP>
+__device__ __forceinline__ float2 lnf_merge_regs(const float2 (&v)[NP], float eps) {
+    float sm = 0.f, sq = 0.f;
+#pragma unroll
+    for (int i = 0; i < NP; ++i) { sm += v[i].x; sq += v[i].y; }
+    const float mean = sm / (float)NP;
+    float dd = 0.f;
+#pragma unroll
+    for (int i = 0; i < NP; ++i) { const float d = v[i].x - mean; dd = fmaf(d, d, dd); }
+    const float var = fmaf((float)LNF_SLICE, dd, sq) / (float)(LNF_SLICE * NP);
+    const float r = rsqrtf(var + eps);
+    return make_float2(r, -mean * r);
+}
+__device__ __forceinline__ float2 lnf_slot_agent(const float2* slots, int i) {
+    return __builtin_bit_cast(float2, __hip_atomic_load((const unsigned long long*)slots + i, __ATOMIC_RELAXED, __HIP_MEMORY_SCOPE_AGENT));
+}
+__device__ __forceinline__ float2 lnf_merge_row_agent(const float2* slots, int P, float eps) {
+    auto merge_n = [&](auto np) {
+        constexpr int NP = decltype(np)::value;
+        float2 v[NP];
+#pragma unroll
+        for (int i = 0; i < NP; ++i) v[i] = lnf_slot_agent(slots, i);
+        return lnf_merge_regs<NP>(v, eps);
+    };
+    if (P == 4) return merge_n(std::integral_constant<int, 4>{});
+    if (P == 6) return merge_n(std::integral_constant<int, 6>{});
+    float sm = 0.f, sq = 0.f;
+    for (int i = 0; i < P; ++i) { const float2 t = lnf_slot_agent(slots, i); sm += t.x; sq += t.y; }
+    const float mean = sm / (float)P;
+    float dd = 0.f;
+    for (int i = 0; i < P; ++i) { const float d = lnf_slot_agent(slots, i).x - mean; dd = fmaf(d, d, dd); }
+    const float var = fmaf((float)LNF_SLICE, dd, sq) / (float)(LNF_SLICE * P);
+    const float r = rsqrtf(var + eps);
+    return make_float2(r, -mean * r);
+}
+template <class ARGS>
+__device__ __forceinline__ void lnf_ticket_merge(const ARGS& p, int mi, int row0, int rows, int parts) {
+    int lane;
+    asm volatile("v_mbcnt_lo_u32_b32 %0, -1, 0\n\tv_mbcnt_hi_u32_b32 %0, -1, %0" : "=v"(lane) :: "memory");
+    unsigned ticket = 0;
+    if (lane == 0) ticket = __hip_atomic_fetch_add(p.lnf_tickets + mi, 1u, __ATOMIC_RELAXED, __HIP_MEMORY_SCOPE_AGENT);
+    ticket = __builtin_amdgcn_readfirstlane(ticket);
+    if (ticket != (unsigned)(parts - 1)) return;
+    const float2* stats = p.lnf_stats;
+    float2* mr = p.lnf_mr;
+    const float eps = p.ln_eps;
+    auto rows4 = [&](auto np) {
+        constexpr int NP = decltype(np)::value;
+        float2 v[4][NP];
+#pragma unroll
+        for (int j = 0; j < 4; ++j) {
+            int r = lane + 64 * j;
+            r = r < rows ? r : rows - 1;
+#pragma unroll
+            for (int i = 0; i < NP; ++i) v[j][i] = lnf_slot_agent(stats + (long)(row0 + r) * NP, i);
+        }
+#pragma unroll
+        for (int j = 0; j < 4; ++j) {
+            const float2 o = lnf_merge_regs<NP>(v[j], eps);
+            if (lane + 64 * j < rows) mr[row0 + lane + 64 * j] = o;
+        }
+    };
+    if (parts == 4) rows4(std::integral_constant<int, 4>{});
+    else if (parts == 6) rows4(std::integral_constant<int, 6>{});
+    else
+        for (int r = lane; r < rows; r += 64) mr[row0 + r] = lnf_merge_row_agent(stats + (long)(row0 + r) * parts, parts, eps);
+    if (lane == 0) __hip_atomic_store(p.lnf_tickets + mi, 0u, __ATOMIC_RELAXED, __HIP_MEMORY_SCOPE_AGENT);
+}
+__global__ __launch_bounds__(256) void ln_merge_slots_kernel(const float2* stats, int parts, float eps, long rows, float2* mr) {
+    const long r = (long)blockIdx.x * 256 + threadIdx.x;
+    if (r < rows) mr[r] = lnf_merge_row_agent(stats + r * parts, parts, eps);
 }
 
 template <int EPI, int BN = 128>
@@ -649,13 +690,13 @@
 #pragma unroll
         for (int n = 0; n < 4; ++n) acc[m][n] = (f32x4){0.f, 0.f, 0.f, 0.f};
 
-    const bool lnc = (EPI == EPI_BF16 || EPI == EPI_BF16_GELU || EPI == EPI_BF16_ROPE) && p.lnc_stats != nullptr;
-    float2* lds_mr = (float2*)(smem + G256_LDS + LNC_RAW_BYTES);
+    const bool lnc = (EPI == EPI_BF16 || EPI == EPI_BF16_GELU || EPI == EPI_BF16_ROPE) && p.lnc_mr != nullptr;
+    float2* lds_mr = (float2*)(smem + G256_LDS);
     if (!(DBG & 2)) {
-        if (lnc) lnc_issue_stats(p, m0, smem + G256_LDS, wave, lane);
+        if (lnc) lnc_issue_mr(p, m0, smem + G256_LDS, wave);
         g256_issue_prologue(A, B, smem, p.K, wave);
-        if (lnc) lnc_merge_rows(p, smem + G256_LDS, lds_mr, wave, lane, p.K <= 64, p.lnc_tele != nullptr && n0 == 0, p.M - m0);
         gemm256_mainloop(A, B, smem, p.K, wave, lane, acc);
+        if (lnc && p.lnc_tele != nullptr && n0 == 0) lnc_tele_rows(p, lds_mr, wave, p.M - m0);
     }
     if (DBG & 1) {
         if (acc[0][0][0] != 12345.678f) return;
@@ -706,12 +747,29 @@
     int mi = m_lo + sq;
     int m0 = tile_row0(mi), n0 = (n_lo + (slot - sq * n_cnt)) * 256;
     bool tall = BMR != 256 && mi >= tall0;
-    const bool lnc = (EPI == EPI_BF16 || EPI == EPI_BF16_GELU || EPI == EPI_BF16_ROPE) && p.lnc_stats != nullptr;
+    const bool lnc = (EPI == EPI_BF16 || EPI == EPI_BF16_GELU || EPI == EPI_BF16_ROPE) && p.lnc_mr != nullptr;
     const bool lnf = EPI == EPI_RESID_F32 && p.lnf_stats != nullptr;
-    char* lds_raw = smem + G256P_LN_OFF;
-    float2* lds_mr = (float2*)(smem + G256P_LN_OFF + LNC_RAW_BYTES);
+    float2* lds_mr = (float2*)(smem + G256P_LN_OFF);
+    float2* lds_mr_next = lds_mr + 256;
     float2* lds_st = (float2*)(smem + G256P_LN_OFF);
-    if (lnc) lnc_issue_stats(p, m0, lds_raw, wave, lane);
+    const bool lnm = lnf && p.lnf_mr != nullptr && p.lnf_tickets != nullptr;
+    int tk_mi = -1;
+    auto take_ticket = [&](int tmi) {
+        if (wave != 4) return;
+        const __attribute__((address_space(4))) GemmArgs* pk = (const __attribute__((address_space(4))) GemmArgs*)__builtin_amdgcn_kernarg_segment_ptr();
+        asm volatile("" : "+s"(pk));
+        const __attribute__((address_space(4))) GemmArgs& q = *pk;
+        const int tn_ = (q.N + 255) / 256;
+        int r0, h;
+        if (BMR == 256) { r0 = tmi * 256; h = 256; }
+        else {
+            const int t0 = q.t192_tiles - q.t192_tall;
+            r0 = tmi * 192 + (tmi > t0 ? (tmi - t0) * 16 : 0);
+            h = tmi >= t0 ? 208 : 192;
+        }
+        lnf_ticket_merge(q, tmi, r0, (r0 + h < q.M ? h : q.M - r0), tn_);
+    };
+    if (lnc) lnc_issue_mr(p, m0, (char*)lds_mr, wave);
     G256Operand A, B;
     g256_operand_init(A, p.A, p.lda, p.M, m0, wave, lane, BMR == 256 ? 256 : (tall ? 208 : 192));
     g256_operand_init(B, p.B, p.ldb, p.N, n0, wave, lane);
@@ -724,7 +782,6 @@
             g256_issue_half(A, 0, 128, G256_A(smem, 1), wave);
             g256_issue_half(A, 1, 128, G256_A(smem, 1), wave);
         }
-        if (lnc && !(REVO_LNC_ABLATE & 1)) lnc_merge_rows(p, lds_raw, lds_mr, wave, lane, p.K <= 64, p.lnc_tele != nullptr && n0 == 0, p.M - m0);
         f32x4 acc[8][4];
 #pragma unroll
         for (int m = 0; m < 8; ++m)
@@ -732,6 +789,8 @@
             for (int n = 0; n < 4; ++n) acc[m][n] = (f32x4){0.f, 0.f, 0.f, 0.f};
         if constexpr (BMR == 256) gemm256_mainloop(A, B, smem, p.K, wave, lane, acc);
         else gemm256_mainloop<192>(A, B, smem, p.K, wave, lane, acc, tall);
+        if (lnc && p.lnc_tele != nullptr && n0 == 0) lnc_tele_rows(p, lds_mr, wave, p.M - m0);
+        if (lnm && tk_mi >= 0) take_ticket(tk_mi);
 
         int lane_e = lane;
         if constexpr (EPI != EPI_BF16 && EPI != EPI_BF16_ROPE)
@@ -742,7 +801,7 @@
             const int mend = m0 + (tall ? 208 : 192);
             pe.M = mend < p.M ? mend : p.M;
         }
-        const int m0_done = m0, tn_done = n0 >> 8;
+        const int m0_done = m0, tn_done = n0 >> 8, mi_done = mi;
         slot += nslot;
         const bool more = slot < total;
         if (more) {
@@ -751,7 +810,7 @@
             m0 = tile_row0(mi);
             n0 = (n_lo + (slot - sq * n_cnt)) * 256;
             tall = BMR != 256 && mi >= tall0;
-            if (lnc && !(REVO_LNC_ABLATE & 4)) lnc_issue_stats(p, m0, lds_raw, wave, lane);
+            if (lnc) lnc_issue_mr(p, m0, (char*)lds_mr_next, wave);
             g256_operand_init(A, p.A, p.lda, p.M, m0, wave, lane, BMR == 256 ? 256 : (tall ? 208 : 192));
             g256_operand_init(B, p.B, p.ldb, p.N, n0, wave, lane);
             g256_issue_half(A, 0, 0, G256_A(smem, 0), wave);
@@ -772,11 +831,18 @@
             asm volatile("s_waitcnt lgkmcnt(0)" ::: "memory");
             __builtin_amdgcn_s_barrier();
             lnf_store_tile_stats(pe, lds_st, m0_done, pe.M, tn_done, wave, lane_e);
+            tk_mi = mi_done;
             if (!more) break;
             continue;
         }
         if (!more) break;
+        { float2* t = lds_mr; lds_mr = lds_mr_next; lds_mr_next = t; }
         __builtin_amdgcn_s_barrier();
+    }
+    if (lnm) {
+        asm volatile("s_waitcnt vmcnt(0)" ::: "memory");
+        __builtin_amdgcn_s_barrier();
+        take_ticket(tk_mi);
     }
 }
 
@@ -785,7 +851,7 @@
 __device__ __forceinline__ void gemm256q_tail(char* smem, int wave) {
     const __attribute__((address_space(4))) GemmArgs* pk0 = (const __attribute__((address_space(4))) GemmArgs*)__builtin_amdgcn_kernarg_segment_ptr();
     if (pk0->qtail_rows <= 0) return;
-    const bool lnc = pk0->lnc_stats != nullptr;
+    const bool lnc = pk0->lnc_mr != nullptr;
     {
         const __attribute__((address_space(4))) GemmArgs& q = *pk0;
         int lane_t;
@@ -833,8 +899,8 @@
                     const long grow = (long)q.M + row;
                     const f32x4 b4 = q.bias ? *(const f32x4*)(q.bias + col) : (f32x4){0.f, 0.f, 0.f, 0.f};
                     if (lnc) {
-                        float rstd, mr;
-                        lnf_merge(q.lnc_stats + grow * q.lnc_parts, q.lnc_parts, q.lnc_eps, rstd, mr);
+                        const float2 st = q.lnc_mr[grow];
+                        const float rstd = st.x, mr = st.y;
                         if (q.lnc_tele && strip == 0 && cq == 0) {
                             unsigned long long* tp = q.lnc_tele;
                             asm volatile("" : "+v"(tp));
@@ -884,12 +950,9 @@
 
     int sq = __builtin_amdgcn_readfirstlane(slot / n_cnt);
     int m0 = (m_lo + sq) * 256, n0 = (n_lo + (slot - sq * n_cnt)) * 256;
-    const bool lnc = p.lnc_stats != nullptr;
-    char* lds_raw = smem + G256_LDS;
-    float2* lds_mr = (float2*)(smem + G256_LDS + LNC_RAW_BYTES);
-    float2* lds_mr_next = lds_mr + 256;
+    const bool lnc = p.lnc_mr != nullptr;
     char* lds_bc = smem + G256Q_BC_OFF;
-    char* lds_bc_next = lds_bc + 2048;
+    char* lds_bc_next = lds_bc + G256Q_BC_BYTES;
     auto issue_bias_csum = [&](const float* bias, const float* csum, int N, int n0_, char* dst, int lane_) {
         if (wave == 4 || wave == 5) {
             const float* src = wave == 4 ? bias : csum;
@@ -898,7 +961,7 @@
                                                      (uint32_t)(lane_ * 16), 0, 0, 0);
         }
     };
-    if (lnc) lnc_issue_stats(p, m0, lds_raw, wave, lane);
+    if (lnc) lnc_issue_mr(p, m0, lds_bc + 2048, wave, 6);
     issue_bias_csum(p.bias, lnc ? p.lnc_c : nullptr, p.N, n0, lds_bc, lane);
     G256Operand A, B;
     g256_operand_init(A, p.A, p.lda, p.M, m0, wave, lane);
@@ -916,8 +979,8 @@
 #ifdef REVO_EXPERIMENTS
     int tiles_done = 0;
 #endif
-    if (lnc) lnc_merge_rows<G256Q_STORES>(p, lds_raw, lds_mr, wave, lane, false, p.lnc_tele != nullptr && n0 == 0, p.M - m0);
-    else if (threadIdx.x < 512) lds_mr[threadIdx.x] = make_float2(1.f, 0.f);
+    if (!lnc && threadIdx.x < 512)
+        ((float2*)((threadIdx.x < 256 ? lds_bc : lds_bc_next) + 2048))[threadIdx.x & 255] = make_float2(1.f, 0.f);
     for (;;) {
         f32x4 acc[8][4];
 #pragma unroll
@@ -946,7 +1009,10 @@
         const bool more = slot < total;
         float2 st8[8];
 #pragma unroll
-        for (int m = 0; m < 8; ++m) st8[m] = lds_mr[wr * 128 + m * 16 + lr];
+        for (int m = 0; m < 8; ++m) st8[m] = ((const float2*)(lds_bc + 2048))[wr * 128 + m * 16 + lr];
+        const bool tele_here = lnc && q.lnc_tele != nullptr && n0_done == 0;
+        float tele_m = 0.f;
+        if (tele_here) tele_m = lnc_tele_read((const float2*)(lds_bc + 2048), wave);
         f32x4 bias4[4], c4[4];
 #pragma unroll
         for (int n = 0; n < 4; ++n) {
@@ -954,6 +1020,8 @@
             c4[n] = *(const f32x4*)(lds_bc + 1024 + (wc * 64 + n * 16 + lq * 4) * 4);
         }
         asm volatile("s_waitcnt lgkmcnt(0)" ::: "memory");
+        G256_FENCE();
+        if (tele_here) lnc_tele_count(q, tele_m, wave, q.M - m0_done);
         G256_FENCE();
         const bool rot = EPI == EPI_BF16_ROPE && nb < q.rope_cols;
         __amdgpu_buffer_rsrc_t rtab = __builtin_amdgcn_make_buffer_rsrc((void*)q.rope_cs, 0, EPI == EPI_BF16_ROPE ? q.rope_S * (q.rope_hd >> 1) * 8 : 0, 0x00020000);
@@ -997,7 +1065,7 @@
             sq = __builtin_amdgcn_readfirstlane(slot / n_cnt);
             m0 = (m_lo + sq) * 256;
             n0 = (n_lo + (slot - sq * n_cnt)) * 256;
-            if (lnc) lnc_issue_stats(q, m0, lds_raw, wave, lane_e);
+            if (lnc) lnc_issue_mr(q, m0, lds_bc_next + 2048, wave, 6);
             issue_bias_csum(q.bias, lnc ? q.lnc_c : nullptr, q.N, n0, lds_bc_next, lane_e);
             g256_operand_init(A, q.A, q.lda, q.M, m0, wave, lane_e);
             g256_operand_init(B, q.B, q.ldb, q.N, n0, wave, lane_e);
@@ -1082,10 +1150,6 @@
         ++tiles_done;
 #endif
         if (!more) break;
-        if (lnc) {
-            lnc_merge_rows<G256Q_STORES>(q, lds_raw, lds_mr_next, wave, lane_e, false, q.lnc_tele != nullptr && n0 == 0, q.M - m0);
-        }
-        { float2* t = lds_mr; lds_mr = lds_mr_next; lds_mr_next = t; }
         { char* t = lds_bc; lds_bc = lds_bc_next; lds_bc_next = t; }
     }
     gemm256q_tail<EPI>(smem, wave);
diff --git a/revers-o_amd/csrc/gemm_plan.h b/revers-o_amd/csrc/gemm_plan.h
--- a/revers-o_amd/csrc/gemm_plan.h
+++ b/revers-o_amd/csrc/gemm_plan.h
@@ -48,7 +48,7 @@
     p.xp_in = a.xp_in; p.xp_out = a.xp_out;
     p.planes_valid = a.xp_hi && a.xp_lo && a.xp_ld % 8 == 0 && (!a.xp_out || a.xp_hi == a.lnf_xb);
     p.rope_S = a.rope_S; p.rope_hd = a.rope_hd; p.rope_cols = a.rope_cols;
-    p.lnc = a.lnc_stats != nullptr;
+    p.lnc = a.lnc_mr != nullptr;
     return p;
 }
 
diff --git a/revers-o_amd/csrc/kernels.h b/revers-o_amd/csrc/kernels.h
--- a/revers-o_amd/csrc/kernels.h
+++ b/revers-o_amd/csrc/kernels.h
@@ -30,8 +30,9 @@
     int ksplit; long c_split_stride;
     const float* ln_w; const float* ln_b; float ln_eps; bf16_t* ln_out; long ln_ldo; int* ln_fused;
     bf16_t* lnf_xb; long lnf_ldxb; float2* lnf_stats; int* lnf_done;
+    float2* lnf_mr; unsigned* lnf_tickets;
     bf16_t* xp_hi; bf16_t* xp_lo; long xp_ld; int xp_in, xp_out;
-    const float2* lnc_stats; int lnc_parts; const float* lnc_c; float lnc_eps;
+    const float2* lnc_mr; const float* lnc_c;
     unsigned long long* lnc_tele;
     int qtail_rows;
 #ifdef REVO_EXPERIMENTS
@@ -68,6 +69,7 @@
 #endif
 int launch_gemm_f32_ring(const GemmArgs& a, hipStream_t st);
 bool gemm_resid_folds(int M, int N, int K, long lda, long ldb, long ldc);
+int launch_ln_merge_slots(const float2* stats, int parts, float eps, long rows, float2* mr, hipStream_t st);
 int launch_planes_to_f32(const bf16_t* hi, const bf16_t* lo, long ldp, float* x, long ldx, long rows, int W, hipStream_t st);
 #ifdef REVO_EXPERIMENTS
 void gemm_set_debug(int d);
diff --git a/revers-o_amd/csrc/tower.h b/revers-o_amd/csrc/tower.h
--- a/revers-o_amd/csrc/tower.h
+++ b/revers-o_amd/csrc/tower.h
@@ -79,6 +79,8 @@
     bf16_t* xlo = nullptr;
     float2* ln_stats = nullptr;
     int ln_parts = 0;
+    float2* ln_mr = nullptr;
+    unsigned* ln_tickets = nullptr;
     unsigned long long* ln_tele = nullptr;
     float* splitk_ws = nullptr;
     std::vector<void*> owned;
@@ -180,6 +182,12 @@
     v->ln_parts = (W % 256 == 0 && W / 256 <= 6) ? (int)(W / 256) : 0;
     if (v->ln_parts) CHECK_RC(v->dalloc(&v->ln_stats, rows * (size_t)v->ln_parts));
     if (v->ln_parts) CHECK_RC(v->dalloc(&v->xlo, rows * W));
+    if (v->ln_parts) {
+        const size_t nt = rows / 192 + 2;
+        CHECK_RC(v->dalloc(&v->ln_mr, rows));
+        CHECK_RC(v->dalloc(&v->ln_tickets, nt));
+        REVO_HIP_CHECK(hipMemset(v->ln_tickets, 0, nt * sizeof(unsigned)));
+    }
     CHECK_RC(v->dalloc(&v->ln_tele, 4));
     REVO_HIP_CHECK(hipMemset(v->ln_tele, 0, 4 * sizeof(unsigned long long)));
     return 0;
@@ -213,7 +221,8 @@
     return a;
 }
 
-struct LnAfter { float eps; bf16_t* out; long ldo; int* fused; float2* stats; int* folded; bf16_t* lo; int x_in_planes, planes_out; };
+struct LnAfter { float eps; bf16_t* out; long ldo; int* fused; float2* stats; int* folded; bf16_t* lo; int x_in_planes, planes_out;
+                 float2* mr; unsigned* tickets; };
 static inline int gemm(const char* cls, int epi, const bf16_t* A, long lda, const bf16_t* B, long ldb, int M, int N, int K, void* C,
                        long ldc, const float* bias, const float* gamma, hipStream_t st, float* ws = nullptr, long ws_elems = 0,
                        const LnAfter* ln = nullptr) {
@@ -222,7 +231,8 @@
     if (ln) {
         a.ln_eps = ln->eps; a.ln_ldo = ln->ldo; a.ln_fused = ln->fused;
         if (ln->fused) a.ln_out = ln->out;
-        if (ln->stats) { a.lnf_xb = ln->out; a.lnf_ldxb = ln->ldo; a.lnf_stats = ln->stats; a.lnf_done = ln->folded; }
+        if (ln->stats) { a.lnf_xb = ln->out; a.lnf_ldxb = ln->ldo; a.lnf_stats = ln->stats; a.lnf_done = ln->folded;
+                         a.lnf_mr = ln->mr; a.lnf_tickets = ln->tickets; }
         if (ln->lo) { a.xp_hi = ln->out; a.xp_lo = ln->lo; a.xp_ld = ln->ldo; a.xp_in = ln->x_in_planes; a.xp_out = ln->planes_out; }
     }
     ProfScope ps(cls, st);
@@ -245,7 +255,7 @@
     bf16_t* xlo = stream_in_planes(t, rows) ? t.xlo : nullptr;
     bool x_planes = false;
     auto ln_before = [&](const float* csum, GemmArgs& a) {
-        if (h_state == H_XB) { a.lnc_stats = stats; a.lnc_parts = t.ln_parts; a.lnc_c = csum; a.lnc_eps = t.ln_eps; a.lnc_tele = t.ln_tele; }
+        if (h_state == H_XB) { a.lnc_mr = t.ln_mr; a.lnc_c = csum; a.lnc_tele = t.ln_tele; }
     };
     auto normalise_if_needed = [&]() -> int {
         if (h_state != H_NONE) return 0;
@@ -270,7 +280,7 @@
         { ProfScope ps("attention", st);
           CHECK_RC(attention()); }
         int fused = 0, folded = 0;
-        const LnAfter ln2{t.ln_eps, t.h, W, &fused, stats, &folded, xlo, x_planes ? 1 : 0, xlo ? 1 : 0};
+        const LnAfter ln2{t.ln_eps, t.h, W, &fused, stats, &folded, xlo, x_planes ? 1 : 0, xlo ? 1 : 0, t.ln_mr, t.ln_tickets};
         CHECK_RC(gemm("gemm_out", EPI_RESID_F32, t.att, W, L.w_o, W, rows, W, W, t.x, W, L.b_o, L.ls1, st, t.splitk_ws,
                       (long)SPLITK_WS_ELEMS, &ln2));
         h_state = folded ? H_XB : (fused ? H_NORM : H_NONE);
@@ -293,7 +303,7 @@
         fused = 0; folded = 0;
         const bool last = i + 1 >= nl;
         const LnAfter ln1n{t.ln_eps, t.h, W, last ? nullptr : &fused, last ? nullptr : stats, last ? nullptr : &folded, xlo,
-                           x_planes ? 1 : 0, (xlo && !last) ? 1 : 0};
+                           x_planes ? 1 : 0, (xlo && !last) ? 1 : 0, t.ln_mr, t.ln_tickets};
         CHECK_RC(gemm("gemm_fc2", EPI_RESID_F32, t.mlp, Md, L.w_fc2, Md, rows, W, Md, t.x, W, L.b_fc2, L.ls2, st,
                       t.splitk_ws, (long)SPLITK_WS_ELEMS, (!last || x_planes) ? &ln1n : nullptr));
         h_state = last ? H_NONE : (folded ? H_XB : (fused ? H_NORM : H_NONE));
```
